# 16lemoing/ccvs

Hardware: AMD Instinct MI355X
Metric: synthesized frames/sec (BAIR 256x256, cond=1, pred=15), whole job (higher is better)
Workload: dtype f32 (convolutions as split-bf16 x3 on bf16 MFMA, fp32 accumulate)

## Files before the change

### ccvs_amd/csrc/gpt.hip

```cpp
#include "common.h"

__global__ __launch_bounds__(256) void gpt_embed_kernel(const int64_t* __restrict__ idx, long idx_sB, const int32_t* __restrict__ pos_off,
                                                        int pos0, const int32_t* __restrict__ pos_dev, int grp_rows, int Tq,
                                                        const float* __restrict__ tok, const float* __restrict__ pos,
                                                        float* __restrict__ x, long total, int C, int vocab) {
    for (long i = (long)blockIdx.x * 256 + threadIdx.x; i < total; i += (long)gridDim.x * 256) {
        const long r = i / C;
        const int c = (int)(i - r * C);
        const long b = r / Tq;
        const int tq = (int)(r - b * Tq);
        long t = idx[b * idx_sB + tq];
        t = t < 0 ? 0 : (t >= vocab ? vocab - 1 : t);
        const long prow = (pos_off ? pos_off[b] : 0) + pos0 + (pos_dev ? pos_dev[grp_rows > 0 ? b / grp_rows : 0] : 0) + tq;
        x[i] = tok[t * C + c] + pos[prow * C + c];
    }
}

extern "C" int ccvs_gpt_embed(const int64_t* idx, int64_t idx_sB, const int32_t* pos_off, int32_t pos0, const int32_t* pos_dev, int32_t Tq,
                              const float* tok_emb, const float* pos_table, float* x, int32_t B, int32_t C, int32_t vocab, void* stream) {
    CCVS_REQUIRE(idx && tok_emb && pos_table && x, "ccvs_gpt_embed: null pointer");
    CCVS_REQUIRE(B > 0 && Tq > 0 && C > 0 && vocab > 0 && (pos0 >= 0 || pos_dev), "ccvs_gpt_embed: empty tensor");
    const long total = (long)B * Tq * C;
    hipLaunchKernelGGL(gpt_embed_kernel, dim3((unsigned)cdiv64(total, 256)), dim3(256), 0, (hipStream_t)stream, idx, (long)idx_sB, pos_off,
                       pos0, pos_dev, 0, Tq, tok_emb, pos_table, x, total, C, vocab);
    CCVS_CHECK_LAUNCH("ccvs_gpt_embed");
    return CCVS_OK;
}

__global__ __launch_bounds__(256) void layernorm_kernel(const float* __restrict__ x, const float* __restrict__ g,
                                                        const float* __restrict__ b, float* __restrict__ y, int rows, int C) {
    const int row = blockIdx.x * 4 + (threadIdx.x >> 6);
    if (row >= rows) return;
    const int lane = threadIdx.x & 63;
    const float* xr = x + (long)row * C;
    float s = 0.f;
    for (int c = lane; c < C; c += 64) s += xr[c];
    const float mean = wave_sum(s) / C;
    float v = 0.f;
    for (int c = lane; c < C; c += 64) { const float d = xr[c] - mean; v += d * d; }
    const float rstd = rsqrtf(wave_sum(v) / C + 1e-5f);
    float* yr = y + (long)row * C;
    for (int c = lane; c < C; c += 64) yr[c] = (xr[c] - mean) * rstd * g[c] + b[c];
}

extern "C" int ccvs_layernorm(const float* x, const float* gamma, const float* beta, float* y, int32_t rows, int32_t C, void* stream) {
    CCVS_REQUIRE(x && gamma && beta && y, "ccvs_layernorm: null pointer");
    CCVS_REQUIRE(rows > 0 && C > 0, "ccvs_layernorm: empty tensor");
    hipLaunchKernelGGL(layernorm_kernel, dim3(cdiv(rows, 4)), dim3(256), 0, (hipStream_t)stream, x, gamma, beta, y, rows, C);
    CCVS_CHECK_LAUNCH("ccvs_layernorm");
    return CCVS_OK;
}

__device__ __forceinline__ float gelu_erf(float v) { return 0.5f * v * (1.f + erff(v * 0.70710678118654752440f)); }

__device__ __forceinline__ void ln_accum(const float4& v, float& sx, float& sxx) {
#pragma clang fp contract(off)
    sx += (v.x + v.y) + (v.z + v.w);
    sxx += (v.x * v.x + v.y * v.y) + (v.z * v.z + v.w * v.w);
}

__device__ __forceinline__ void ln_accum(const f32x4& v, float& sx, float& sxx) {
#pragma clang fp contract(off)
    sx += (v[0] + v[1]) + (v[2] + v[3]);
    sxx += (v[0] * v[0] + v[1] * v[1]) + (v[2] * v[2] + v[3] * v[3]);
}

typedef unsigned int u32x4 __attribute__((ext_vector_type(4)));
template <int AUX = 0>
__device__ __forceinline__ f32x4 buf_load4(__amdgpu_buffer_rsrc_t r, unsigned voff, int soff) {
    const u32x4 v = __builtin_amdgcn_raw_buffer_load_b128(r, voff, soff, AUX);
    return __builtin_bit_cast(f32x4, v);
}

template <bool COH>
__device__ __forceinline__ float ld_act(const float* p) {
    if constexpr (COH) return __hip_atomic_load(p, __ATOMIC_RELAXED, __HIP_MEMORY_SCOPE_AGENT);
    else return *p;
}
template <bool COH>
__device__ __forceinline__ void st_act(float* p, float v) {
    if constexpr (COH) __hip_atomic_store(p, v, __ATOMIC_RELAXED, __HIP_MEMORY_SCOPE_AGENT);
    else *p = v;
}
template <bool OPAQUE>
__device__ __forceinline__ int thread_id() {
    int t = threadIdx.x;
    if constexpr (OPAQUE) asm volatile("" : "+v"(t));
    return t;
}
template <bool COH, typename T>
__device__ __forceinline__ T* gp_(T* p) {
    if constexpr (COH) return (T*)(__attribute__((address_space(1))) T*)p;
    else return p;
}
__device__ __forceinline__ f32x4 ld_act4_sc1(const float* p) {
    const __amdgpu_buffer_rsrc_t r = __builtin_amdgcn_make_buffer_rsrc(const_cast<float*>(p), 0, 16, 0x00020000);
    typedef unsigned int u32x4_ __attribute__((ext_vector_type(4)));
    const u32x4_ v = __builtin_amdgcn_raw_buffer_load_b128(r, 0, 0, 16);
    return __builtin_bit_cast(f32x4, v);
}

struct Gemm16 {
    const float* x; long ldx;
    const float* w; const float* bias; const float* res; float* y; long ldy;
    int M, N, K, epi, ks;
    const float* ln_s; float ln_eps;
    float* kcache; float* vcache; int C, H, D, Tq, Tmax, pos0; const int32_t* pos_dev;
    int seq;
    int grp_rows;
    int kz;
    float* ws_slabs;
    int* ws_count;
};

#define GEMM_U 4
#define GEMM_U_RB 8
#define GEMM_WS_TILES 1024
#define GEMM_KZ_MAX 4
#define GEMM_KZ_MIN_K 2048
#define GEMM_DECODE_MAX_M 256

__device__ __forceinline__ void ln_finish(float a, float b, int K, float eps, float& mean, float& rstd) {
#pragma clang fp contract(off)
    mean = a / K;
    const float var = fmaxf(b / K - mean * mean, 0.f);
    rstd = rsqrtf(var + eps);
}
__device__ __forceinline__ float gemm_epilogue(float v, bool ln, float rstd, float mean, float sn, float bv, int epi, float rv) {
#pragma clang fp contract(off)
    if (ln) v = rstd * (v - mean * sn);
    v += bv;
    if (epi == 1) v = gelu_erf(v);
    if (epi == 2) v += rv;
    return v;
}

#define GEMM_WAVES 4
#define GEMM16_RED_WORDS(NB) (GEMM_WAVES * (NB) * 64 * 4)
#define GEMM16_STAT_WORDS(RB) (GEMM_WAVES * (RB) * 16 * 2)
#define GEMM16_FIN_WORDS(RB) ((RB) * 16 * 2)
template <int RB, int CB, int U, bool COH, typename PT>
__device__ __forceinline__ void gemm16_tile(const float* __restrict__ x_, const float* __restrict__ w_, long ldx_, int K_, int N_, int M_, int ks_,
                                            int kz_, const PT& p, int bx_, int by_, int bz_, float* __restrict__ red, float* __restrict__ stat,
                                            float* __restrict__ fin) {
#define GP(ptr) gp_<COH>(ptr)
    constexpr int NB = RB * CB;
    constexpr int XAUX = COH ? 16 : 0;
    const int tid = thread_id<COH>(), lane = tid & 63, wave = tid >> 6;
    const int li = lane & 15, g = lane >> 4;
    const int m0 = by_ * 16 * RB, ncol0 = bx_ * 16 * CB;
    const int kper = K_ / (ks_ * kz_);
    const int kbase = bz_ * (K_ / kz_);
    const bool active = wave < ks_;
    const unsigned koff = kbase + (active ? wave : 0) * kper + 4 * g;
    unsigned wofs[CB], xofs[RB];
#pragma unroll
    for (int cb = 0; cb < CB; ++cb) {
        const int nrow = min(ncol0 + 16 * cb + li, N_ - 1);
        wofs[cb] = ((unsigned)nrow * (unsigned)K_ + koff) * 4u;
    }
#pragma unroll
    for (int rb = 0; rb < RB; ++rb) {
        const int mrow = min(m0 + 16 * rb + li, M_ - 1);
        xofs[rb] = ((unsigned)mrow * (unsigned)ldx_ + koff) * 4u;
    }
    const __amdgpu_buffer_rsrc_t wr = __builtin_amdgcn_make_buffer_rsrc(const_cast<float*>(w_), 0, N_ * K_ * 4, 0x00020000);
    const __amdgpu_buffer_rsrc_t xr = __builtin_amdgcn_make_buffer_rsrc(const_cast<float*>(x_), 0, (int)(M_ * ldx_ * 4), 0x00020000);
    f32x4 acc[RB][CB];
    float sx[RB], sxx[RB];
#pragma unroll
    for (int rb = 0; rb < RB; ++rb) {
        sx[rb] = 0.f; sxx[rb] = 0.f;
#pragma unroll
        for (int cb = 0; cb < CB; ++cb) acc[rb][cb] = {0.f, 0.f, 0.f, 0.f};
    }
    if (active) {
        int k0 = 0;
        for (; k0 + 16 * U <= kper; k0 += 16 * U) {
            f32x4 wv[CB][U], xv[RB][U];
#pragma unroll
            for (int cb = 0; cb < CB; ++cb)
#pragma unroll
                for (int u = 0; u < U; ++u) wv[cb][u] = buf_load4(wr, wofs[cb], k0 * 4 + 64 * u);
#pragma unroll
            for (int rb = 0; rb < RB; ++rb)
#pragma unroll
                for (int u = 0; u < U; ++u) xv[rb][u] = buf_load4<XAUX>(xr, xofs[rb], k0 * 4 + 64 * u);
            __builtin_amdgcn_sched_barrier(0);
#pragma unroll
            for (int u = 0; u < U; ++u) {
#pragma unroll
                for (int rb = 0; rb < RB; ++rb) {
#pragma unroll
                    for (int cb = 0; cb < CB; ++cb)
#pragma unroll
                        for (int t = 0; t < 4; ++t) acc[rb][cb] = __builtin_amdgcn_mfma_f32_16x16x4f32(xv[rb][u][t], wv[cb][u][t], acc[rb][cb], 0, 0, 0);
                    if (p.ln_s) ln_accum(xv[rb][u], sx[rb], sxx[rb]);
                }
            }
        }
        for (; k0 < kper; k0 += 16) {
            f32x4 w1[CB], x1[RB];
#pragma unroll
            for (int cb = 0; cb < CB; ++cb) w1[cb] = buf_load4(wr, wofs[cb], k0 * 4);
#pragma unroll
            for (int rb = 0; rb < RB; ++rb) x1[rb] = buf_load4<XAUX>(xr, xofs[rb], k0 * 4);
#pragma unroll
            for (int rb = 0; rb < RB; ++rb) {
#pragma unroll
                for (int cb = 0; cb < CB; ++cb)
#pragma unroll
                    for (int t = 0; t < 4; ++t) acc[rb][cb] = __builtin_amdgcn_mfma_f32_16x16x4f32(x1[rb][t], w1[cb][t], acc[rb][cb], 0, 0, 0);
                if (p.ln_s) ln_accum(x1[rb], sx[rb], sxx[rb]);
            }
        }
    }
    if (p.ln_s) {
#pragma unroll
        for (int rb = 0; rb < RB; ++rb) {
            float a = sx[rb], b = sxx[rb];
            a += __shfl_xor(a, 16, 64); a += __shfl_xor(a, 32, 64);
            b += __shfl_xor(b, 16, 64); b += __shfl_xor(b, 32, 64);
            if (g == 0) { stat[((wave * RB + rb) * 16 + li) * 2] = a; stat[((wave * RB + rb) * 16 + li) * 2 + 1] = b; }
        }
    }
#pragma unroll
    for (int rb = 0; rb < RB; ++rb)
#pragma unroll
        for (int cb = 0; cb < CB; ++cb) *reinterpret_cast<f32x4*>(red + ((wave * NB + rb * CB + cb) * 64 + lane) * 4) = acc[rb][cb];
    __syncthreads();
    if (p.ln_s && tid < 16 * RB) {
        const int rb = tid >> 4, r = tid & 15;
        float a = 0.f, b = 0.f;
        for (int w = 0; w < GEMM_WAVES; ++w) { a += stat[((w * RB + rb) * 16 + r) * 2]; b += stat[((w * RB + rb) * 16 + r) * 2 + 1]; }
        float mean, rstd;
        ln_finish(a, b, p.K, p.ln_eps, mean, rstd);
        fin[tid * 2] = mean;
        fin[tid * 2 + 1] = rstd;
    }
    __syncthreads();
#pragma unroll 1
    for (int blk = wave; blk < NB; blk += GEMM_WAVES) {
        const int rb = blk / CB, cb = blk - rb * CB;
        f32x4 a4;
        if constexpr (NB == 1) a4 = acc[0][0];
        else a4 = *reinterpret_cast<const f32x4*>(red + (blk * 64 + lane) * 4);
#pragma unroll
        for (int s = 1; s < GEMM_WAVES; ++s) a4 += *reinterpret_cast<const f32x4*>(red + ((s * NB + blk) * 64 + lane) * 4);
        const int mb0 = m0 + 16 * rb, nb0 = ncol0 + 16 * cb;
        if (mb0 >= p.M || nb0 >= p.N) continue;

        bool finisher = true;
        if (p.kz > 1) {
            const int tile = (mb0 >> 4) * ((p.N + 15) >> 4) + (nb0 >> 4);
            float* slabs = GP(p.ws_slabs) + (long)tile * p.kz * 256;
            float* mine = slabs + (bz_ * 64 + lane) * 4;
#pragma unroll
            for (int c = 0; c < 4; ++c) __hip_atomic_store(mine + c, a4[c], __ATOMIC_RELAXED, __HIP_MEMORY_SCOPE_AGENT);
            asm volatile("s_waitcnt vmcnt(0)" ::: "memory");
            int ticket = 0;
            if (lane == 0) ticket = __hip_atomic_fetch_add(GP(p.ws_count) + tile, 1, __ATOMIC_RELAXED, __HIP_MEMORY_SCOPE_AGENT);
            ticket = __builtin_amdgcn_readfirstlane(ticket);
            finisher = ticket == p.kz - 1;
            if (finisher) {
#pragma unroll
                for (int c = 0; c < 4; ++c) a4[c] = __hip_atomic_load(slabs + lane * 4 + c, __ATOMIC_RELAXED, __HIP_MEMORY_SCOPE_AGENT);
                for (int z = 1; z < p.kz; ++z) {
#pragma unroll
                    for (int c = 0; c < 4; ++c) a4[c] += __hip_atomic_load(slabs + (z * 64 + lane) * 4 + c, __ATOMIC_RELAXED, __HIP_MEMORY_SCOPE_AGENT);
                }
                if (lane == 0) __hip_atomic_store(GP(p.ws_count) + tile, 0, __ATOMIC_RELAXED, __HIP_MEMORY_SCOPE_AGENT);
            }
        }

        const int col = nb0 + li;
        if (finisher && col < p.N) {
            const float bv = p.bias ? GP(p.bias)[col] : 0.f;
            const float sn = p.ln_s ? GP(p.ln_s)[col] : 0.f;
#pragma unroll
            for (int r = 0; r < 4; ++r) {
                const int row = mb0 + 4 * g + r;
                if (row >= p.M) continue;
                const float rv = p.epi == 2 ? ld_act<COH>(GP(p.res) + (long)row * p.ldy + col) : 0.f;
                const float v = gemm_epilogue(a4[r], p.ln_s != nullptr, fin[(rb * 16 + 4 * g + r) * 2 + 1], fin[(rb * 16 + 4 * g + r) * 2], sn, bv, p.epi, rv);
                if (p.kcache && col >= p.C) {
                    const int cc = col - p.C;
                    float* cache = cc >= p.C ? GP(p.vcache) : GP(p.kcache);
                    const int c2 = cc >= p.C ? cc - p.C : cc;
                    const int h = c2 / p.D, d = c2 - h * p.D;
                    const int b = row / p.Tq, t = row - b * p.Tq;
                    const int pos = p.pos0 + (p.pos_dev ? GP(p.pos_dev)[p.grp_rows > 0 ? b / p.grp_rows : 0] : 0);
                    if (pos + t < p.Tmax) st_act<COH>(cache + (((long)b * p.H + h) * p.Tmax + pos + t) * p.D + d, v);
                } else {
                    st_act<COH>(GP(p.y) + (long)row * p.ldy + col, v);
                }
            }
        }
    }
#undef GP
}

template <int RB, int CB, int U>
__global__ __launch_bounds__(64 * GEMM_WAVES) void gemm16_kernel(const float* __restrict__ x_, const float* __restrict__ w_, long ldx_, int K_, int N_,
                                                                int M_, int ks_, int kz_, Gemm16 p) {
    __shared__ __attribute__((aligned(16))) float red[GEMM16_RED_WORDS(RB * CB)];
    __shared__ float stat[GEMM16_STAT_WORDS(RB)];
    __shared__ float fin[GEMM16_FIN_WORDS(RB)];
    gemm16_tile<RB, CB, U, false>(x_, w_, ldx_, K_, N_, M_, ks_, kz_, p, blockIdx.x, blockIdx.y, blockIdx.z, red, stat, fin);
}

template <int RB>
__global__ __launch_bounds__(512) void gemm16_rb_kernel(Gemm16 p) {
    __shared__ __attribute__((aligned(16))) float red[RB * 8 * 64 * 4];
    __shared__ float stat[RB * 8 * 16 * 2];
    __shared__ float fin[RB * 16 * 2];
    const int tid = threadIdx.x, lane = tid & 63, wave = tid >> 6;
    const int li = lane & 15, g = lane >> 4;
    const int m0 = blockIdx.y * 16 * RB, ncol0 = blockIdx.x * 16;
    const int nrow = min(ncol0 + li, p.N - 1);
    const int kper = p.K / p.ks;
    const bool active = wave < p.ks;
    const float* wp = p.w + (long)nrow * p.K + (active ? wave : 0) * kper + 4 * g;
    const float* xp[RB];
#pragma unroll
    for (int rb = 0; rb < RB; ++rb) xp[rb] = p.x + (long)min(m0 + 16 * rb + li, p.M - 1) * p.ldx + (active ? wave : 0) * kper + 4 * g;
    f32x4 acc0[RB], acc1[RB];
    float sx[RB], sxx[RB];
#pragma unroll
    for (int rb = 0; rb < RB; ++rb) { acc0[rb] = {0.f, 0.f, 0.f, 0.f}; acc1[rb] = {0.f, 0.f, 0.f, 0.f}; sx[rb] = 0.f; sxx[rb] = 0.f; }
    if (active) {
        int k0 = 0;
        for (; k0 + 16 * GEMM_U_RB <= kper; k0 += 16 * GEMM_U_RB) {
            float4 wv[GEMM_U_RB];
#pragma unroll
            for (int u = 0; u < GEMM_U_RB; ++u) wv[u] = *reinterpret_cast<const float4*>(wp + k0 + 16 * u);
#pragma unroll
            for (int rb = 0; rb < RB; ++rb) {
                float4 xv[GEMM_U_RB];
#pragma unroll
                for (int u = 0; u < GEMM_U_RB; ++u) xv[u] = *reinterpret_cast<const float4*>(xp[rb] + k0 + 16 * u);
#pragma unroll
                for (int u = 0; u < GEMM_U_RB; ++u) {
                    acc0[rb] = __builtin_amdgcn_mfma_f32_16x16x4f32(xv[u].x, wv[u].x, acc0[rb], 0, 0, 0);
                    acc1[rb] = __builtin_amdgcn_mfma_f32_16x16x4f32(xv[u].y, wv[u].y, acc1[rb], 0, 0, 0);
                    acc0[rb] = __builtin_amdgcn_mfma_f32_16x16x4f32(xv[u].z, wv[u].z, acc0[rb], 0, 0, 0);
                    acc1[rb] = __builtin_amdgcn_mfma_f32_16x16x4f32(xv[u].w, wv[u].w, acc1[rb], 0, 0, 0);
                    if (p.ln_s) ln_accum(xv[u], sx[rb], sxx[rb]);
                }
            }
        }
        for (; k0 < kper; k0 += 16) {
            const float4 w1 = *reinterpret_cast<const float4*>(wp + k0);
#pragma unroll
            for (int rb = 0; rb < RB; ++rb) {
                const float4 x1 = *reinterpret_cast<const float4*>(xp[rb] + k0);
                acc0[rb] = __builtin_amdgcn_mfma_f32_16x16x4f32(x1.x, w1.x, acc0[rb], 0, 0, 0);
                acc1[rb] = __builtin_amdgcn_mfma_f32_16x16x4f32(x1.y, w1.y, acc1[rb], 0, 0, 0);
                acc0[rb] = __builtin_amdgcn_mfma_f32_16x16x4f32(x1.z, w1.z, acc0[rb], 0, 0, 0);
                acc1[rb] = __builtin_amdgcn_mfma_f32_16x16x4f32(x1.w, w1.w, acc1[rb], 0, 0, 0);
                if (p.ln_s) ln_accum(x1, sx[rb], sxx[rb]);
            }
        }
    }
#pragma unroll
    for (int rb = 0; rb < RB; ++rb) {
        const f32x4 acc = acc0[rb] + acc1[rb];
        if (p.ln_s) {
            float a = sx[rb], b = sxx[rb];
            a += __shfl_xor(a, 16, 64); a += __shfl_xor(a, 32, 64);
            b += __shfl_xor(b, 16, 64); b += __shfl_xor(b, 32, 64);
            if (g == 0) { stat[((rb * 8 + wave) * 16 + li) * 2] = a; stat[((rb * 8 + wave) * 16 + li) * 2 + 1] = b; }
        }
        *reinterpret_cast<f32x4*>(red + ((rb * 8 + wave) * 64 + lane) * 4) = acc;
    }
    __syncthreads();
    if (p.ln_s && tid < 16 * RB) {
        const int rb = tid >> 4, r = tid & 15;
        float a = 0.f, b = 0.f;
        for (int w = 0; w < 8; ++w) { a += stat[((rb * 8 + w) * 16 + r) * 2]; b += stat[((rb * 8 + w) * 16 + r) * 2 + 1]; }
        float mean, rstd;
        ln_finish(a, b, p.K, p.ln_eps, mean, rstd);
        fin[tid * 2] = mean;
        fin[tid * 2 + 1] = rstd;
    }
    __syncthreads();
    if (wave >= RB) return;
    const int rb = wave;
    f32x4 acc = *reinterpret_cast<const f32x4*>(red + ((rb * 8) * 64 + lane) * 4);
#pragma unroll
    for (int s2 = 1; s2 < 8; ++s2) acc += *reinterpret_cast<const f32x4*>(red + ((rb * 8 + s2) * 64 + lane) * 4);
    const int col = ncol0 + li;
    if (col >= p.N) return;
    const float bv = p.bias ? p.bias[col] : 0.f;
    const float sn = p.ln_s ? p.ln_s[col] : 0.f;
    int pos0 = p.pos0;
    if (p.kcache && p.pos_dev) pos0 += *p.pos_dev;
#pragma unroll
    for (int r = 0; r < 4; ++r) {
        const int row = m0 + 16 * rb + 4 * g + r;
        if (row >= p.M) continue;
        const float v = gemm_epilogue(acc[r], p.ln_s != nullptr, fin[(rb * 16 + 4 * g + r) * 2 + 1], fin[(rb * 16 + 4 * g + r) * 2], sn, bv, p.epi,
                                      p.epi == 2 ? p.res[(long)row * p.ldy + col] : 0.f);
        if (p.kcache && col >= p.C) {
            const int cc = col - p.C;
            float* cache = cc >= p.C ? p.vcache : p.kcache;
            const int c2 = cc >= p.C ? cc - p.C : cc;
            const int h = c2 / p.D, d = c2 - h * p.D;
            const int b = row / p.Tq, t = row - b * p.Tq;
            if (pos0 + t < p.Tmax) cache[(((long)b * p.H + h) * p.Tmax + pos0 + t) * p.D + d] = v;
        } else {
            p.y[(long)row * p.ldy + col] = v;
        }
    }
}

#define GS_BM 128
#define GS_QS (GS_BM + 1)
typedef __attribute__((address_space(3))) void gs_lds_void;
__global__ __launch_bounds__(256, 4) void gemm_seq_kernel(Gemm16 p, int row_tiles, int col_tiles) {
    __shared__ __attribute__((aligned(16))) f32x4 sm0[2 * 4 * GS_QS];
    __shared__ __attribute__((aligned(16))) f32x4 sm1[2 * 4 * GS_QS];
    __shared__ float fin[GS_BM * 2];
    const int tid = threadIdx.x, lane = tid & 63, wave = tid >> 6;
    int rt, ct;
    {
        const int w = blockIdx.x;
        if (row_tiles % 8 == 0) {
            const int i = w >> 3;
            rt = (w & 7) + 8 * (i / col_tiles);
            ct = i % col_tiles;
        } else {
            rt = w / col_tiles;
            ct = w - rt * col_tiles;
        }
    }
    const int m0 = rt * GS_BM, n0 = ct * GS_BM;
    const __amdgpu_buffer_rsrc_t xr = __builtin_amdgcn_make_buffer_rsrc(const_cast<float*>(p.x), 0, (int)((long)p.M * p.ldx * 4), 0x00020000);
    const __amdgpu_buffer_rsrc_t wrs = __builtin_amdgcn_make_buffer_rsrc(const_cast<float*>(p.w), 0, (int)((long)p.N * p.K * 4), 0x00020000);
    unsigned xoff[2], woff[2];
#pragma unroll
    for (int hf = 0; hf < 2; ++hf) {
        xoff[hf] = (unsigned)((long)min(m0 + 64 * hf + lane, p.M - 1) * p.ldx + 4 * wave) * 4u;
        woff[hf] = (unsigned)((long)min(n0 + 64 * hf + lane, p.N - 1) * p.K + 4 * wave) * 4u;
    }
    const int wr = wave >> 1, wc = wave & 1, l31 = lane & 31, h = lane >> 5;
    f32x16 acc[2][2];
#pragma unroll
    for (int bi = 0; bi < 2; ++bi)
#pragma unroll
        for (int bj = 0; bj < 2; ++bj)
#pragma unroll
            for (int r = 0; r < 16; ++r) acc[bi][bj][r] = 0.f;
    float sx = 0.f, sxx = 0.f;
    const int nst = p.K / 16;
#define GS_DMA(k0, SM)                                                                                             \
    _Pragma("unroll") for (int hf = 0; hf < 2; ++hf) {                                                             \
        __builtin_amdgcn_raw_ptr_buffer_load_lds(xr, (gs_lds_void*)((SM) + wave * GS_QS + 64 * hf), 16, xoff[hf], (k0) * 4, 0, 0);               \
        __builtin_amdgcn_raw_ptr_buffer_load_lds(wrs, (gs_lds_void*)((SM) + 4 * GS_QS + wave * GS_QS + 64 * hf), 16, woff[hf], (k0) * 4, 0, 0);  \
    }
#define GS_STAGE(SM, NEXT_DMA)                                                                                     \
    {                                                                                                              \
        const f32x4* xa = (SM);                                                                                    \
        const f32x4* wb = (SM) + 4 * GS_QS;                                                                        \
        f32x4 a[2][2], b[2][2], t0, t1;                                                                            \
        _Pragma("unroll") for (int s2 = 0; s2 < 2; ++s2) {                                                         \
            const int q = 2 * s2 + h;                                                                              \
            _Pragma("unroll") for (int bi = 0; bi < 2; ++bi) a[s2][bi] = xa[q * GS_QS + 64 * wr + 32 * bi + l31];  \
            _Pragma("unroll") for (int bj = 0; bj < 2; ++bj) b[s2][bj] = wb[q * GS_QS + 64 * wc + 32 * bj + l31];  \
        }                                                                                                          \
        if (p.ln_s) {                                                                                              \
            const int r = tid >> 1, q0 = 2 * (tid & 1);                                                            \
            t0 = xa[q0 * GS_QS + r];                                                                               \
            t1 = xa[(q0 + 1) * GS_QS + r];                                                                         \
        }                                                                                                          \
         \
         \
        NEXT_DMA                                                                                                   \
        _Pragma("unroll") for (int s2 = 0; s2 < 2; ++s2)                                                           \
            _Pragma("unroll") for (int j = 0; j < 4; ++j)                                                          \
                _Pragma("unroll") for (int bi = 0; bi < 2; ++bi)                                                   \
                    _Pragma("unroll") for (int bj = 0; bj < 2; ++bj)                                               \
                        acc[bi][bj] = __builtin_amdgcn_mfma_f32_32x32x2f32(a[s2][bi][j], b[s2][bj][j], acc[bi][bj], 0, 0, 0); \
        if (p.ln_s) {                                                                                              \
            ln_accum(t0, sx, sxx);                                                                                 \
            ln_accum(t1, sx, sxx);                                                                                 \
        }                                                                                                          \
    }
    GS_DMA(0, sm0)
    for (int st = 0; st < nst; st += 2) {
        __syncthreads();
        GS_STAGE(sm0, if (st + 1 < nst) { GS_DMA(16 * (st + 1), sm1) })
        if (st + 1 >= nst) break;
        __syncthreads();
        GS_STAGE(sm1, if (st + 2 < nst) { GS_DMA(16 * (st + 2), sm0) })
    }
#undef GS_DMA
#undef GS_STAGE
    if (p.ln_s) {
        sx += __shfl_xor(sx, 1, 64);
        sxx += __shfl_xor(sxx, 1, 64);
        if (!(tid & 1)) {
            float mean, rstd;
            ln_finish(sx, sxx, p.K, p.ln_eps, mean, rstd);
            fin[(tid >> 1) * 2] = mean;
            fin[(tid >> 1) * 2 + 1] = rstd;
        }
        __syncthreads();
    }
    int pos0 = p.pos0;
    if (p.kcache && p.pos_dev) pos0 += *p.pos_dev;
#pragma unroll
    for (int bj = 0; bj < 2; ++bj) {
        const int col = n0 + 64 * wc + 32 * bj + l31;
        if (col >= p.N) continue;
        const float bv = p.bias ? p.bias[col] : 0.f;
        const float sn = p.ln_s ? p.ln_s[col] : 0.f;
#pragma unroll
        for (int bi = 0; bi < 2; ++bi) {
#pragma unroll
            for (int r = 0; r < 16; ++r) {
                const int lr = 64 * wr + 32 * bi + (r & 3) + 8 * (r >> 2) + 4 * h;
                const int row = m0 + lr;
                if (row >= p.M) continue;
                const float v = gemm_epilogue(acc[bi][bj][r], p.ln_s != nullptr, p.ln_s ? fin[lr * 2 + 1] : 0.f, p.ln_s ? fin[lr * 2] : 0.f, sn, bv,
                                              p.epi, p.epi == 2 ? p.res[(long)row * p.ldy + col] : 0.f);
                if (p.kcache && col >= p.C) {
                    const int cc = col - p.C;
                    float* cache = cc >= p.C ? p.vcache : p.kcache;
                    const int c2 = cc >= p.C ? cc - p.C : cc;
                    const int hh = c2 / p.D, d = c2 - hh * p.D;
                    const int b = row / p.Tq, t = row - b * p.Tq;
                    if (pos0 + t < p.Tmax) cache[(((long)b * p.H + hh) * p.Tmax + pos0 + t) * p.D + d] = v;
                } else {
                    p.y[(long)row * p.ldy + col] = v;
                }
            }
        }
    }
}

static int gemm_kz(const Gemm16& g) {
    const int tiles = cdiv(g.N, 16);
    int kz = 1;
    if (g.ws_slabs && !g.ln_s && tiles * cdiv(GEMM_DECODE_MAX_M, 16) <= GEMM_WS_TILES)
        while (g.K >= GEMM_KZ_MIN_K && kz < GEMM_KZ_MAX && tiles * kz * 2 <= 256 && g.K % (16 * GEMM_WAVES * kz * 2) == 0) kz *= 2;
    return kz;
}

static bool gemm_tile2() {
    static const bool v = getenv_int("CCVS_GEMM_TILE2", 1) != 0;
    return v;
}

enum GemmForm { GEMM_FORM_TILE1, GEMM_FORM_TILE2, GEMM_FORM_RB, GEMM_FORM_SEQ };
static GemmForm gemm16_plan(Gemm16& g) {
    const bool decode_form = !g.seq && g.M <= GEMM_DECODE_MAX_M;
    g.kz = decode_form ? gemm_kz(g) : 1;
    g.ks = decode_form ? GEMM_WAVES : 8;
    while (g.ks > 1 && g.K % (16 * g.ks * g.kz) != 0) g.ks >>= 1;
    if (decode_form) return gemm_tile2() && g.M > 32 && g.N >= 32 ? GEMM_FORM_TILE2 : GEMM_FORM_TILE1;
    static const int seq_dense = getenv_int("CCVS_GEMM_SEQ_DENSE", 1);
    const bool fits = (long)g.M * g.ldx * 4 < (1L << 31) && (long)g.N * g.K * 4 < (1L << 31);
    return g.seq && seq_dense && fits ? GEMM_FORM_SEQ : GEMM_FORM_RB;
}

static bool gemm_ws_holds(const Gemm16& g) { return g.kz == 1 || cdiv(g.N, 16) * cdiv(g.M, 16) <= GEMM_WS_TILES; }

static int launch_gemm16(Gemm16& g, hipStream_t st, const char* name) {
    if (!(g.x && g.w && g.y)) { ccvs_set_error("%s: null pointer", name); return CCVS_ERR_ARG; }
    if (!(g.M > 0 && g.N > 0 && g.K > 0)) { ccvs_set_error("%s: empty tensor", name); return CCVS_ERR_ARG; }
    if (g.K % 16 != 0 || g.ldx % 4 != 0) { ccvs_set_error("%s: K=%d must be a multiple of 16 (ldx %% 4 == 0)", name, g.K); return CCVS_ERR_ARG; }
    if (g.epi < 0 || g.epi > 2 || (g.epi == 2 && !g.res)) { ccvs_set_error("%s: bad epilogue", name); return CCVS_ERR_ARG; }
    const GemmForm form = gemm16_plan(g);
    const bool decode_form = form == GEMM_FORM_TILE1 || form == GEMM_FORM_TILE2;
    if (!gemm_ws_holds(g)) { ccvs_set_error("%s: split-K over %d x %d blocks outgrows the workspace", name, cdiv(g.M, 16), cdiv(g.N, 16)); return CCVS_ERR_ARG; }
    if (decode_form && ((long)g.N * g.K * 4 >= (1L << 31) || (long)g.M * g.ldx * 4 >= (1L << 31))) {
        ccvs_set_error("%s: operand beyond 2^31 bytes (32-bit buffer offsets)", name);
        return CCVS_ERR_ARG;
    }
    if (!decode_form && g.grp_rows > 0) { ccvs_set_error("%s: row groups need M <= %d", name, GEMM_DECODE_MAX_M); return CCVS_ERR_ARG; }
    if (form == GEMM_FORM_SEQ) {
        const int rt = cdiv(g.M, GS_BM), ct = cdiv(g.N, GS_BM);
        hipLaunchKernelGGL(gemm_seq_kernel, dim3(rt * ct), dim3(256), 0, st, g, rt, ct);
    } else if (form == GEMM_FORM_RB)
        hipLaunchKernelGGL((gemm16_rb_kernel<4>), dim3(cdiv(g.N, 16), cdiv(g.M, 64), 1), dim3(512), 0, st, g);
    else {
#define GEMM16_LAUNCH(RBv, CBv, Uv)                                                                                                         \
    hipLaunchKernelGGL((gemm16_kernel<RBv, CBv, Uv>), dim3(cdiv(g.N, 16 * CBv), cdiv(g.M, 16 * RBv), g.kz), dim3(64 * GEMM_WAVES), 0, st, g.x, \
                       g.w, g.ldx, g.K, g.N, g.M, g.ks, g.kz, g)
        if (form == GEMM_FORM_TILE2) GEMM16_LAUNCH(2, 2, 1); else GEMM16_LAUNCH(1, 1, GEMM_U);
#undef GEMM16_LAUNCH
    }
    CCVS_CHECK_LAUNCH(name);
    return CCVS_OK;
}

#define GEMM_WS_SLAB_BYTES ((size_t)GEMM_WS_TILES * GEMM_KZ_MAX * 256 * sizeof(float))
#define GEMM_WS_BAR_OFFSET (GEMM_WS_SLAB_BYTES + (size_t)GEMM_WS_TILES * sizeof(int))
#define GEMM_WS_BAR_BYTES 2048
extern "C" int64_t ccvs_gemm_workspace_bytes(void) { return (int64_t)(GEMM_WS_BAR_OFFSET + GEMM_WS_BAR_BYTES); }

extern "C" int ccvs_gemm_nt(const float* x, int64_t ldx, const float* w, const float* bias, const float* res, float* y, int64_t ldy,
                            int32_t M, int32_t N, int32_t K, int32_t epilogue, void* workspace, void* stream) {
    Gemm16 g = {};
    g.x = x; g.ldx = ldx; g.w = w; g.bias = bias; g.res = res; g.y = y; g.ldy = ldy; g.M = M; g.N = N; g.K = K;
    g.epi = epilogue & 0xff; g.seq = (epilogue & CCVS_GEMM_SEQ) ? 1 : 0;
    if (workspace) {
        g.ws_slabs = (float*)workspace;
        g.ws_count = (int*)((char*)workspace + GEMM_WS_SLAB_BYTES);
    }
    return launch_gemm16(g, (hipStream_t)stream, "ccvs_gemm_nt");
}

extern "C" int ccvs_gemm_ln(const float* x, int64_t ldx, const float* w_gamma, const float* bias_beta, const float* w_rowsum, float eps,
                            float* y, int64_t ldy, int32_t M, int32_t N, int32_t K, int32_t epilogue, void* stream) {
    CCVS_REQUIRE(w_rowsum, "ccvs_gemm_ln: null pointer");
    CCVS_REQUIRE((epilogue & 0xff) == 0 || (epilogue & 0xff) == 1, "ccvs_gemm_ln: bad epilogue");
    Gemm16 g = {};
    g.x = x; g.ldx = ldx; g.w = w_gamma; g.bias = bias_beta; g.y = y; g.ldy = ldy; g.M = M; g.N = N; g.K = K;
    g.epi = epilogue & 0xff; g.seq = (epilogue & CCVS_GEMM_SEQ) ? 1 : 0;
    g.ln_s = w_rowsum; g.ln_eps = eps;
    return launch_gemm16(g, (hipStream_t)stream, "ccvs_gemm_ln");
}

extern "C" int ccvs_gemm_ln_qkv(const float* x, int64_t ldx, const float* w_gamma, const float* bias_beta, const float* w_rowsum, float eps,
                                float* q, float* kcache, float* vcache, int32_t B, int32_t Tq, int32_t C, int32_t H, int32_t pos0,
                                const int32_t* pos_dev, int32_t Tmax, void* stream) {
    CCVS_REQUIRE(w_rowsum && kcache && vcache, "ccvs_gemm_ln_qkv: null pointer");
    CCVS_REQUIRE(B > 0 && Tq > 0 && H > 0 && C % H == 0 && pos0 >= 0 && pos0 + Tq <= Tmax, "ccvs_gemm_ln_qkv: bad shape / positions");
    Gemm16 g = {};
    g.x = x; g.ldx = ldx; g.w = w_gamma; g.bias = bias_beta; g.y = q; g.ldy = C; g.M = B * Tq; g.N = 3 * C; g.K = C; g.epi = 0;
    g.ln_s = w_rowsum; g.ln_eps = eps;
    g.kcache = kcache; g.vcache = vcache; g.C = C; g.H = H; g.D = C / H; g.Tq = Tq; g.Tmax = Tmax; g.pos0 = pos0; g.pos_dev = pos_dev;
    g.seq = Tq > 1 ? 1 : 0;
    return launch_gemm16(g, (hipStream_t)stream, "ccvs_gemm_ln_qkv");
}

__global__ __launch_bounds__(256) void kv_append_kernel(const float* __restrict__ k, const float* __restrict__ v, long sB, long ld,
                                                        float* __restrict__ kc, float* __restrict__ vc, long total, int H, int Tq,
                                                        int pos0, const int32_t* __restrict__ pos_dev, int Tmax, int D) {
    if (pos_dev) pos0 += *pos_dev;
    for (long i = (long)blockIdx.x * 256 + threadIdx.x; i < total; i += (long)gridDim.x * 256) {
        const int d = (int)(i % D);
        long t = i / D;
        const int h = (int)(t % H);
        t /= H;
        const int tq = (int)(t % Tq);
        const long b = t / Tq;
        if (pos0 + tq >= Tmax) continue;
        const long src = b * sB + tq * ld + h * D + d;
        const long dst = ((b * H + h) * Tmax + pos0 + tq) * D + d;
        kc[dst] = k[src];
        vc[dst] = v[src];
    }
}

extern "C" int ccvs_kv_append(const float* k, const float* v, int64_t sB, int64_t ld, float* kcache, float* vcache, int32_t B, int32_t H,
                              int32_t Tq, int32_t pos0, const int32_t* pos_dev, int32_t Tmax, int32_t D, void* stream) {
    CCVS_REQUIRE(k && v && kcache && vcache, "ccvs_kv_append: null pointer");
    CCVS_REQUIRE(B > 0 && H > 0 && Tq > 0 && D > 0 && pos0 >= 0 && pos0 + Tq <= Tmax, "ccvs_kv_append: positions %d..%d exceed cache %d",
                 pos0, pos0 + Tq, Tmax);
    const long total = (long)B * Tq * H * D;
    hipLaunchKernelGGL(kv_append_kernel, dim3((unsigned)cdiv64(total, 256)), dim3(256), 0, (hipStream_t)stream, k, v, (long)sB, (long)ld, kcache,
                       vcache, total, H, Tq, pos0, pos_dev, Tmax, D);
    CCVS_CHECK_LAUNCH("ccvs_kv_append");
    return CCVS_OK;
}

template <int D>
__global__ __launch_bounds__(256) void attention_prefill_kernel(const float* __restrict__ q, long q_sB, long ldq, const float* __restrict__ kc,
                                                                const float* __restrict__ vc, float* __restrict__ out, int H, int Tq, int pos0,
                                                                const int32_t* __restrict__ pos_dev, int Tmax, float scale) {
    constexpr int MT = (D + 31) / 32;
    constexpr int DP = MT * 32;
    constexpr int DK = D / 2;
    constexpr int KS = 33;
    constexpr int F4 = D / 4;
    constexpr int NLD = (32 * F4 + 255) / 256;
    constexpr int TILE_WORDS = D * KS + 32 * DP;
    constexpr int OUT_WORDS = 128 * (D + 1);
    constexpr int SMEM_WORDS = 2 * TILE_WORDS > OUT_WORDS ? 2 * TILE_WORDS : OUT_WORDS;
    __shared__ __attribute__((aligned(16))) float smem[SMEM_WORDS];
    const int tid = threadIdx.x, lane = tid & 63, wave = tid >> 6;
    const int qi = lane & 31, half = lane >> 5;
    const int bh = blockIdx.x, b = bh / H, h = bh - b * H;
    if (pos_dev) pos0 += *pos_dev;
    const int q0 = (gridDim.y - 1 - blockIdx.y) * 128;
    const int qw = q0 + wave * 32;
    const int qidx = qw + qi;
    const int q_last_wg = min(q0 + 127, Tq - 1), q_last_w = min(qw + 31, Tq - 1);
    const int ntiles = (min(pos0 + q_last_wg + 1, Tmax) + 31) >> 5;
    const float* kbase = kc + (long)bh * Tmax * D;
    const float* vbase = vc + (long)bh * Tmax * D;

    float qreg[DK];
    {
        const float* qp = q + (long)b * q_sB + (long)min(qidx, Tq - 1) * ldq + h * D + half;
#pragma unroll
        for (int i = 0; i < DK; ++i) qreg[i] = (qidx < Tq) ? qp[2 * i] * (scale * 1.44269504088896340736f) : 0.f;
    }
    if (MT * 32 > D) {
        for (int e = tid; e < 2 * 32 * (DP - D); e += 256) {
            const int bsel = e / (32 * (DP - D)), r = e - bsel * 32 * (DP - D);
            smem[bsel * TILE_WORDS + D * KS + (r / (DP - D)) * DP + D + r % (DP - D)] = 0.f;
        }
    }

    float4 kreg[NLD], vreg[NLD];
    auto fetch = [&](int kt) {
#pragma unroll
        for (int r = 0; r < NLD; ++r) {
            const int e = min(tid + 256 * r, 32 * F4 - 1);
            const int key = e / F4, d4 = e - key * F4;
            const bool written = kt * 32 + key < pos0 + Tq;
            const long row = min(kt * 32 + key, pos0 + Tq - 1);
            const float4 kv = *reinterpret_cast<const float4*>(kbase + row * D + 4 * d4);
            const float4 vv = *reinterpret_cast<const float4*>(vbase + row * D + 4 * d4);
            kreg[r] = written ? kv : make_float4(0.f, 0.f, 0.f, 0.f);
            vreg[r] = written ? vv : make_float4(0.f, 0.f, 0.f, 0.f);
        }
    };
    auto stash = [&](int buf) {
        float* kt_s = smem + buf * TILE_WORDS;
        float* v_s = kt_s + D * KS;
#pragma unroll
        for (int r = 0; r < NLD; ++r) {
            const int e = tid + 256 * r;
            if (e < 32 * F4) {
                const int key = e / F4, d4 = e - key * F4;
                kt_s[(4 * d4 + 0) * KS + key] = kreg[r].x;
                kt_s[(4 * d4 + 1) * KS + key] = kreg[r].y;
                kt_s[(4 * d4 + 2) * KS + key] = kreg[r].z;
                kt_s[(4 * d4 + 3) * KS + key] = kreg[r].w;
                *reinterpret_cast<float4*>(v_s + key * DP + 4 * d4) = vreg[r];
            }
        }
    };

    f32x16 acc_o[MT];
#pragma unroll
    for (int mt = 0; mt < MT; ++mt)
#pragma unroll
        for (int r = 0; r < 16; ++r) acc_o[mt][r] = 0.f;
    float m_run = -INFINITY, l_run = 0.f;

    fetch(0);
    __syncthreads();
    stash(0);
    __syncthreads();
    for (int kt = 0; kt < ntiles; ++kt) {
        const int buf = kt & 1;
        if (kt + 1 < ntiles) fetch(kt + 1);
        const int key0 = kt * 32;
        if (key0 <= pos0 + q_last_w && qw < Tq) {
            const float* kt_s = smem + buf * TILE_WORDS;
            const float* v_s = kt_s + D * KS;
            f32x16 s;
#pragma unroll
            for (int r = 0; r < 16; ++r) s[r] = 0.f;
#pragma unroll
            for (int i = 0; i < DK; ++i) s = __builtin_amdgcn_mfma_f32_32x32x2f32(kt_s[(2 * i + half) * KS + qi], qreg[i], s, 0, 0, 0);
            const int lim = pos0 + qidx - key0;
            float m_t = -INFINITY;
#pragma unroll
            for (int r = 0; r < 16; ++r) {
                const int kk = 8 * (r >> 2) + 4 * half + (r & 3);
                s[r] = (kk <= lim && qidx < Tq) ? s[r] : -INFINITY;
                m_t = fmaxf(m_t, s[r]);
            }
            m_t = fmaxf(m_t, __shfl_xor(m_t, 32, 64));
            const float m_new = fmaxf(m_run, m_t);
            const float m_use = (m_new == -INFINITY) ? 0.f : m_new;
            const float alpha = __builtin_amdgcn_exp2f(m_run - m_use);
            float l_t = 0.f;
#pragma unroll
            for (int r = 0; r < 16; ++r) {
                s[r] = __builtin_amdgcn_exp2f(s[r] - m_use);
                l_t += s[r];
            }
            l_t += __shfl_xor(l_t, 32, 64);
            l_run = l_run * alpha + l_t;
            m_run = m_new;
            const bool rescale = __any(alpha != 1.f);
#pragma unroll
            for (int mt = 0; mt < MT; ++mt) {
                if (rescale) {
#pragma unroll
                    for (int r = 0; r < 16; ++r) acc_o[mt][r] *= alpha;
                }
#pragma unroll
                for (int j = 0; j < 16; ++j) {
                    const int kk = 8 * (j >> 2) + 4 * half + (j & 3);
                    acc_o[mt] = __builtin_amdgcn_mfma_f32_32x32x2f32(v_s[kk * DP + mt * 32 + qi], s[j], acc_o[mt], 0, 0, 0);
                }
            }
        }
        if (kt + 1 < ntiles) stash(buf ^ 1);
        __syncthreads();
    }
    float* o_s = smem;
    const float inv = l_run > 0.f ? 1.f / l_run : 0.f;
#pragma unroll
    for (int mt = 0; mt < MT; ++mt)
#pragma unroll
        for (int r = 0; r < 16; ++r) {
            const int d = mt * 32 + 8 * (r >> 2) + 4 * half + (r & 3);
            if (d < D) o_s[(wave * 32 + qi) * (D + 1) + d] = acc_o[mt][r] * inv;
        }
    __syncthreads();
    for (int e = tid; e < 128 * D; e += 256) {
        const int ql = e / D, d = e - ql * D;
        if (q0 + ql < Tq) out[((long)b * Tq + q0 + ql) * (H * D) + h * D + d] = o_s[ql * (D + 1) + d];
    }
}

__device__ __forceinline__ f32x4 ld_f4_nt(const float* p) {
    return __builtin_nontemporal_load(reinterpret_cast<const f32x4*>(p));
}

template <int D, bool COH>
__device__ __forceinline__ void attention_decode_item(const float* __restrict__ q, long q_sB, const float* __restrict__ kc,
                                                      const float* __restrict__ vc, float* __restrict__ out, int H, int pos0,
                                                      const int32_t* __restrict__ pos_dev, int grp_rows, int Tmax, float scale, int bh,
                                                      float* smem) {
    constexpr int LPK = D / 4;
    constexpr int KPI = 64 / LPK;
    constexpr int NW = 4;
    constexpr int AU = 4;
    constexpr int BATCH = NW * KPI * AU;
    float* red = smem;
    float* pv = smem + 16;
    float* ps = smem + 16 + NW * 256;
    const int tid = thread_id<COH>(), lane = tid & 63, wave = tid >> 6;
    const int b = bh / H, h = bh - b * H;
    if (pos_dev) {
        if constexpr (COH) pos0 += ((const __attribute__((address_space(4))) int32_t*)pos_dev)[grp_rows > 0 ? b / grp_rows : 0];
        else pos0 += pos_dev[grp_rows > 0 ? b / grp_rows : 0];
    }
    const int L = min(pos0 + 1, Tmax);
    const int kk = lane / LPK, d4 = lane - kk * LPK;
    const float* kbase = kc + (long)bh * Tmax * D + 4 * d4;
    const float* vbase = vc + (long)bh * Tmax * D + 4 * d4;
    const int jw = wave * KPI + kk;
    const int nbatch = (L + BATCH - 1) / BATCH;

    f32x4 k_new = {0.f, 0.f, 0.f, 0.f}, v_new = {0.f, 0.f, 0.f, 0.f};
    if constexpr (COH) {
        k_new = ld_act4_sc1(kbase + (long)(L - 1) * D);
        v_new = ld_act4_sc1(vbase + (long)(L - 1) * D);
    }
#define ATT_LOAD(dst, base, bi, fresh)                                                                                   \
    _Pragma("unroll") for (int u = 0; u < AU; ++u) {                                                                     \
        dst[u] = ld_f4_nt(base + (long)min((bi) * BATCH + jw + u * NW * KPI, L - 1) * D);                                \
        if constexpr (COH) { if ((bi) * BATCH + jw + u * NW * KPI >= L - 1) dst[u] = fresh; }                            \
    }

    float4 qv;
    if constexpr (COH) {
        const f32x4 q4 = ld_act4_sc1(q + (long)b * q_sB + h * D + 4 * d4);
        qv = make_float4(q4[0], q4[1], q4[2], q4[3]);
    } else {
        qv = *reinterpret_cast<const float4*>(q + (long)b * q_sB + h * D + 4 * d4);
    }
    float lmax = -INFINITY;
#pragma unroll 1
    for (int bi = 0; bi < nbatch; ++bi) {
        f32x4 kv[AU];
        ATT_LOAD(kv, kbase, bi, k_new);
#pragma unroll
        for (int u = 0; u < AU; ++u) {
            const int j = bi * BATCH + jw + u * NW * KPI;
            float s = kv[u][0] * qv.x + kv[u][1] * qv.y + kv[u][2] * qv.z + kv[u][3] * qv.w;
#pragma unroll
            for (int o = 1; o < LPK; o <<= 1) s += __shfl_xor(s, o, 64);
            s *= scale;
            if (j < L) {
                if (d4 == 0) ps[j] = s;
                lmax = fmaxf(lmax, s);
            }
        }
    }
    f32x4 vv[AU];
    ATT_LOAD(vv, vbase, 0, v_new);

    lmax = wave_max(lmax);
    if (lane == 0) red[wave] = lmax;
    __syncthreads();
    float gmax = red[0];
#pragma unroll
    for (int w = 1; w < NW; ++w) gmax = fmaxf(gmax, red[w]);
    float lsum = 0.f;
    for (int j = tid; j < L; j += NW * 64) {
        const float e = expf(ps[j] - gmax);
        ps[j] = e;
        lsum += e;
    }
    lsum = wave_sum(lsum);
    __syncthreads();
    if (lane == 0) red[wave] = lsum;
    __syncthreads();
    float tot = red[0];
#pragma unroll
    for (int w = 1; w < NW; ++w) tot += red[w];

    float4 acc = make_float4(0.f, 0.f, 0.f, 0.f);
#pragma unroll 1
    for (int bi = 0; bi < nbatch; ++bi) {
        if (bi > 0) ATT_LOAD(vv, vbase, bi, v_new);
#pragma unroll
        for (int u = 0; u < AU; ++u) {
            const int j = bi * BATCH + jw + u * NW * KPI;
            const float p = (j < L) ? ps[min(j, L - 1)] : 0.f;
            acc.x += p * vv[u][0]; acc.y += p * vv[u][1]; acc.z += p * vv[u][2]; acc.w += p * vv[u][3];
        }
    }
#undef ATT_LOAD
    *reinterpret_cast<float4*>(pv + (wave * 64 + lane) * 4) = acc;
    __syncthreads();
    if (tid < D) {
        const int dd4 = tid >> 2, comp = tid & 3;
        float o = 0.f;
        for (int w = 0; w < NW; ++w)
            for (int s2 = 0; s2 < KPI; ++s2) o += pv[(w * 64 + s2 * LPK + dd4) * 4 + comp];
        st_act<COH>(out + (long)b * (H * D) + h * D + tid, o / tot);
    }
}

template <int D>
__global__ __launch_bounds__(256) void attention_decode_kernel(const float* __restrict__ q, long q_sB, const float* __restrict__ kc,
                                                               const float* __restrict__ vc, float* __restrict__ out, int H, int pos0,
                                                               const int32_t* __restrict__ pos_dev, int grp_rows, int Tmax, float scale) {
    extern __shared__ __attribute__((aligned(16))) float smem[];
    attention_decode_item<D, false>(q, q_sB, kc, vc, out, H, pos0, pos_dev, grp_rows, Tmax, scale, blockIdx.x, smem);
}

static void launch_attention_decode(int D, int n_bh, size_t smem, hipStream_t st, const float* q, long q_sB, const float* kc, const float* vc,
                                    float* out, int H, int pos0, const int32_t* pos_dev, int grp_rows, int Tmax, float scale) {
#define ATT_DECODE_LAUNCH(Dv) \
// ... 65 lines not shown
        __syncthreads();
        for (int j = tid; j < V; j += 256) {
            const unsigned key = fkey(xs[j]);
            if ((key & mask) == prefix) atomicAdd(&hist[(key >> shift) & 255u], 1);
        }
        __syncthreads();
        const int h = hist[tid];
        int s = h;
#pragma unroll
        for (int o = 1; o < 64; o <<= 1) {
            const int t = __shfl_down(s, o, 64);
            if (lane + o < 64) s += t;
        }
        if (lane == 0) wtot[wave] = s;
        __syncthreads();
        for (int w = wave + 1; w < 4; ++w) s += wtot[w];
        if (s >= need && s - h < need) { sel[0] = tid; sel[1] = need - (s - h); }
        __syncthreads();
        prefix |= (unsigned)sel[0] << shift;
        mask |= 255u << shift;
        need = sel[1];
    }
    return prefix;
}

template <bool COH>
__device__ __forceinline__ void sample_topk_row(const float* __restrict__ logits, long ld, const float* __restrict__ noise,
                                                int64_t* __restrict__ out, long out_stride, int V, int top_k, float temperature,
                                                Advance adv, int b, int B_all, float* smem) {
    float* xs = smem;
    float* redf = smem + V;
    int* redj = (int*)(smem + V + 4);
    int* wtot = (int*)(smem + V + 8);
    int* sel = (int*)(smem + V + 12);
    int* hist = (int*)(smem + V + 16);
    const int tid = thread_id<COH>(), lane = tid & 63, wave = tid >> 6;
    const int grp = adv.grp_rows > 0 ? b / adv.grp_rows : 0;
    const int brow = b - grp * (adv.grp_rows > 0 ? adv.grp_rows : 0);
    const int nrows = adv.grp_rows > 0 ? min(adv.grp_rows, B_all - grp * adv.grp_rows) : B_all;
    if (adv.grp_rows > 0) { adv.state += 8 * grp; adv.widx += grp; adv.len += grp; }
    const float* lr = logits + (long)b * ld;
    float lmax = -INFINITY;
    for (int j = tid; j < V; j += 256) {
        const float v = ld_act<COH>(lr + j) / temperature;
        xs[j] = v;
        lmax = fmaxf(lmax, v);
    }
    lmax = wave_max(lmax);
    if (lane == 0) redf[wave] = lmax;
    __syncthreads();
    const float gmax = fmaxf(fmaxf(redf[0], redf[1]), fmaxf(redf[2], redf[3]));

    unsigned thr = 0u;
    if (top_k > 0 && top_k < V) thr = kth_largest_key(xs, V, top_k, hist, wtot, sel, tid);
    float lsum = 0.f;
    for (int j = tid; j < V; j += 256) {
        const float e = (fkey(xs[j]) >= thr) ? expf(xs[j] - gmax) : 0.f;
        xs[j] = e;
        lsum += e;
    }
    lsum = wave_sum(lsum);
    __syncthreads();
    if (lane == 0) redf[wave] = lsum;
    __syncthreads();
    const float tot = ((redf[0] + redf[1]) + redf[2]) + redf[3];
    unsigned k0 = 0u, k1 = 0u, step = 0u, row0 = 0u, call = 0u;
    if (adv.rng == 2) {
        k0 = adv.imm[0]; k1 = adv.imm[1]; row0 = adv.imm[2]; step = adv.imm[3]; call = adv.imm[4];
    } else if (adv.rng) {
        k0 = (unsigned)adv.state[4]; k1 = (unsigned)adv.state[5]; step = (unsigned)adv.state[0];
        call = (unsigned)adv.state[3]; row0 = (unsigned)adv.state[6];
    }
    const float* nrow = noise ? noise + (long)b * V : nullptr;
    if (adv.noise_stream) nrow = adv.noise_stream[grp] + ((long)adv.state[0] * nrows + brow) * V;
    float best = -1.f;
    int bi = 0x7fffffff;
    for (int j = tid; j < V; j += 256) {
        float p = xs[j] / tot;
        if (nrow) p = p / nrow[j];
        else if (adv.rng) {
            const float u = ((float)philox_first((unsigned)j, row0 + (unsigned)brow, step, call, k0, k1) + 0.5f) * 2.3283064365386963e-10f;
            p = p / fmaxf(-logf(u), 1e-30f);
        }
        if (p > best) { best = p; bi = j; }
    }
#pragma unroll
    for (int o = 32; o > 0; o >>= 1) {
        const float ob = __shfl_xor(best, o, 64);
        const int oi = __shfl_xor(bi, o, 64);
        if (ob > best || (ob == best && oi < bi)) { best = ob; bi = oi; }
    }
    __syncthreads();
    if (lane == 0) { redf[wave] = best; redj[wave] = bi; }
    __syncthreads();
    if (tid == 0) {
        for (int w = 1; w < 4; ++w)
            if (redf[w] > best || (redf[w] == best && redj[w] < bi)) { best = redf[w]; bi = redj[w]; }
        out[(long)b * out_stride] = bi;
        if (adv.codes) {
            adv.codes[(long)b * adv.codes_sB + *adv.widx] = bi;
            asm volatile("s_waitcnt vmcnt(0)" ::: "memory");
            __builtin_amdgcn_fence(__ATOMIC_RELEASE, "agent");
            const int ticket = __hip_atomic_fetch_add(adv.state + 2, 1, __ATOMIC_RELAXED, __HIP_MEMORY_SCOPE_AGENT);
            if (ticket == nrows - 1) {
                __builtin_amdgcn_fence(__ATOMIC_ACQUIRE, "agent");
                *adv.widx += 1;
                *adv.len += 1;
                adv.state[0] += 1;
                __hip_atomic_store(adv.state + 2, 0, __ATOMIC_RELAXED, __HIP_MEMORY_SCOPE_AGENT);
            }
        }
    }
}

__global__ __launch_bounds__(256) void sample_topk_kernel(const float* __restrict__ logits, long ld, const float* __restrict__ noise,
                                                          int64_t* __restrict__ out, long out_stride, int V, int top_k, float temperature,
                                                          Advance adv) {
    extern __shared__ __attribute__((aligned(16))) float smem[];
    sample_topk_row<false>(logits, ld, noise, out, out_stride, V, top_k, temperature, adv, blockIdx.x, gridDim.x, smem);
}

#define PICK_SMEM_WORDS(V) ((V) + 16 + 256)
static void pick_allow_big_lds() {
    static bool attr_set = false;
    if (!attr_set) {
        (void)hipFuncSetAttribute((const void*)sample_topk_kernel, hipFuncAttributeMaxDynamicSharedMemorySize, 160 * 1024);
        attr_set = true;
    }
}

extern "C" int ccvs_sample_topk(const float* logits, int64_t ld, const float* noise, int64_t* out, int64_t out_stride, int32_t B, int32_t V,
                                int32_t top_k, float temperature, void* stream) {
    CCVS_REQUIRE(logits && out, "ccvs_sample_topk: null pointer");
    CCVS_REQUIRE(B > 0 && V > 0 && temperature > 0.f, "ccvs_sample_topk: bad arguments");
    const size_t smem = (size_t)PICK_SMEM_WORDS(V) * sizeof(float);
    pick_allow_big_lds();
    CCVS_REQUIRE(smem <= 160 * 1024, "ccvs_sample_topk: vocabulary %d too large", V);
    hipLaunchKernelGGL(sample_topk_kernel, dim3(B), dim3(256), smem, (hipStream_t)stream, logits, (long)ld, noise, out, (long)out_stride, V,
                       top_k, temperature, Advance{});
    CCVS_CHECK_LAUNCH("ccvs_sample_topk");
    return CCVS_OK;
}

extern "C" int ccvs_sample_topk_philox(const float* logits, int64_t ld, int64_t* out, int64_t out_stride, int32_t B, int32_t V, int32_t top_k,
                                       float temperature, uint32_t key0, uint32_t key1, uint32_t row0, uint32_t step, uint32_t call,
                                       void* stream) {
    CCVS_REQUIRE(logits && out, "ccvs_sample_topk_philox: null pointer");
    CCVS_REQUIRE(B > 0 && V > 0 && temperature > 0.f, "ccvs_sample_topk_philox: bad arguments");
    const size_t smem = (size_t)PICK_SMEM_WORDS(V) * sizeof(float);
    pick_allow_big_lds();
    CCVS_REQUIRE(smem <= 160 * 1024, "ccvs_sample_topk_philox: vocabulary %d too large", V);
    Advance adv = {};
    adv.rng = 2;
    adv.imm[0] = key0; adv.imm[1] = key1; adv.imm[2] = row0; adv.imm[3] = step; adv.imm[4] = call;
    hipLaunchKernelGGL(sample_topk_kernel, dim3(B), dim3(256), smem, (hipStream_t)stream, logits, (long)ld, (const float*)nullptr, out,
                       (long)out_stride, V, top_k, temperature, adv);
    CCVS_CHECK_LAUNCH("ccvs_sample_topk_philox");
    return CCVS_OK;
}

__global__ __launch_bounds__(256) void sample_topn_kernel(const float* __restrict__ logits, long ld, const float* __restrict__ noise,
                                                          int64_t* __restrict__ out_idx, float* __restrict__ out_logp, int V, int top_k,
                                                          float temperature, int n) {
    extern __shared__ __attribute__((aligned(16))) float smem[];
    float* xs = smem;
    float* sc = smem + V;
    float* redf = smem + 2 * V;
    int* redj = (int*)(smem + 2 * V + 4);
    int* wtot = (int*)(smem + 2 * V + 8);
    int* sel = (int*)(smem + 2 * V + 12);
    int* hist = (int*)(smem + 2 * V + 16);
    const int tid = threadIdx.x, lane = tid & 63, wave = tid >> 6;
    const int b = blockIdx.x;
    const float* lr = logits + (long)b * ld;
    float lmax = -INFINITY;
    for (int j = tid; j < V; j += 256) {
        const float v = lr[j] / temperature;
        xs[j] = v;
        lmax = fmaxf(lmax, v);
    }
    lmax = wave_max(lmax);
    if (lane == 0) redf[wave] = lmax;
    __syncthreads();
    const float gmax = fmaxf(fmaxf(redf[0], redf[1]), fmaxf(redf[2], redf[3]));
    unsigned thr = 0u;
    if (top_k > 0 && top_k < V) thr = kth_largest_key(xs, V, top_k, hist, wtot, sel, tid);
    float lsum = 0.f;
    for (int j = tid; j < V; j += 256) {
        const float e = (fkey(xs[j]) >= thr) ? expf(xs[j] - gmax) : 0.f;
        xs[j] = e;
        lsum += e;
    }
    lsum = wave_sum(lsum);
    __syncthreads();
    if (lane == 0) redf[wave] = lsum;
    __syncthreads();
    const float tot = ((redf[0] + redf[1]) + redf[2]) + redf[3];
    for (int j = tid; j < V; j += 256) {
        const float p = xs[j] / tot;
        xs[j] = p;
        sc[j] = noise ? p / noise[(long)b * V + j] : p;
    }
    __syncthreads();
    for (int r = 0; r < n; ++r) {
        float best = -1.f;
        int bi = 0x7fffffff;
        for (int j = tid; j < V; j += 256) {
            const float v = sc[j];
            if (v > best) { best = v; bi = j; }
        }
#pragma unroll
        for (int o = 32; o > 0; o >>= 1) {
            const float ob = __shfl_xor(best, o, 64);
            const int oi = __shfl_xor(bi, o, 64);
            if (ob > best || (ob == best && oi < bi)) { best = ob; bi = oi; }
        }
        if (lane == 0) { redf[wave] = best; redj[wave] = bi; }
        __syncthreads();
        if (tid == 0) {
            for (int w = 1; w < 4; ++w)
                if (redf[w] > best || (redf[w] == best && redj[w] < bi)) { best = redf[w]; bi = redj[w]; }
            bi = min(bi, V - 1);
            out_idx[(long)b * n + r] = bi;
            out_logp[(long)b * n + r] = logf(xs[bi]);
            sc[bi] = -2.f;
        }
        __syncthreads();
    }
}

extern "C" int ccvs_sample_topn(const float* logits, int64_t ld, const float* noise, int64_t* out_idx, float* out_logp, int32_t B, int32_t V,
                                int32_t top_k, float temperature, int32_t n, void* stream) {
    CCVS_REQUIRE(logits && out_idx && out_logp, "ccvs_sample_topn: null pointer");
    CCVS_REQUIRE(B > 0 && V > 0 && temperature > 0.f && n >= 1 && n <= V, "ccvs_sample_topn: bad arguments");
    const size_t smem = (size_t)(2 * V + 16 + 256) * sizeof(float);
    CCVS_REQUIRE(smem <= 160 * 1024, "ccvs_sample_topn: vocabulary %d too large", V);
    static bool attr_set = false;
    if (!attr_set) {
        (void)hipFuncSetAttribute((const void*)sample_topn_kernel, hipFuncAttributeMaxDynamicSharedMemorySize, 160 * 1024);
        attr_set = true;
    }
    hipLaunchKernelGGL(sample_topn_kernel, dim3(B), dim3(256), smem, (hipStream_t)stream, logits, (long)ld, noise, out_idx, out_logp, V, top_k,
                       temperature, n);
    CCVS_CHECK_LAUNCH("ccvs_sample_topn");
    return CCVS_OK;
}

#define STEP_SPIN_TICKS 500000000ULL
struct StepBar {
    unsigned shard[8][32];
    unsigned base[32];
    unsigned err[32];
};
static_assert(sizeof(StepBar) <= GEMM_WS_BAR_BYTES, "StepBar outgrew its slot in the workspace");

#define STEP_GEMM 0
#define STEP_ATTENTION 1
struct StepPhase {
    int kind, pad_;
    Gemm16 g;
};

struct StepArgs {
    int B, C, V, vocab, grp_rows, pos_off, n_phases, H;
    const float *tok_emb, *pos_table;
    const int64_t* tok;
    const int32_t* len;
    float *x, *logits;
    StepBar* bar;
    const StepPhase* prog;
    float scale;
    const float* noise;
    int top_k;
    float temperature;
    Advance adv;
};

__device__ __forceinline__ void step_barrier(StepBar* bar, unsigned target, int phase) {
    asm volatile("s_waitcnt vmcnt(0)" ::: "memory");
    __syncthreads();
    if (threadIdx.x < 64) {
        if (threadIdx.x == 0) __hip_atomic_fetch_add(&bar->shard[blockIdx.x & 7][0], 1u, __ATOMIC_RELAXED, __HIP_MEMORY_SCOPE_AGENT);
        const unsigned* sp = &bar->shard[threadIdx.x & 7][0];
        const unsigned long long t0 = __builtin_amdgcn_s_memrealtime();
        for (unsigned spins = 1;; ++spins) {
            unsigned v = __hip_atomic_load(sp, __ATOMIC_RELAXED, __HIP_MEMORY_SCOPE_AGENT);
            v += __shfl_xor(v, 1, 64);
            v += __shfl_xor(v, 2, 64);
            v += __shfl_xor(v, 4, 64);
            if ((int)(v - target) >= 0) break;
            __builtin_amdgcn_s_sleep(2);
            if ((spins & 255u) == 0) {
                const bool late = __builtin_amdgcn_s_memrealtime() - t0 > STEP_SPIN_TICKS;
                if (late || __hip_atomic_load(&bar->err[0], __ATOMIC_RELAXED, __HIP_MEMORY_SCOPE_AGENT) != 0u) {
                    if (late && threadIdx.x == 0) __hip_atomic_store(&bar->err[0], (unsigned)(phase + 1), __ATOMIC_RELAXED, __HIP_MEMORY_SCOPE_AGENT);
                    break;
                }
            }
        }
    }
    __syncthreads();
}

template <int RB, int CB, int U>
__device__ __forceinline__ void step_gemm(const __attribute__((address_space(4))) Gemm16& g, float* smem) {
    float* red = smem;
    float* stat = red + GEMM16_RED_WORDS(RB * CB);
    float* fin = stat + GEMM16_STAT_WORDS(RB);
    const int N = g.N, M = g.M, K = g.K, ks = g.ks, kz = g.kz;
    const long ldx = g.ldx;
    const float* x = gp_<true>(g.x);
    const float* w = gp_<true>(g.w);
    const int gx = (N + 16 * CB - 1) / (16 * CB), gy = (M + 16 * RB - 1) / (16 * RB);
    const int total = gx * gy * kz;
    for (int vb = blockIdx.x; vb < total; vb += gridDim.x) {
        const int bx = vb % gx, r = vb / gx;
        gemm16_tile<RB, CB, U, true>(x, w, ldx, K, N, M, ks, kz, g, bx, r % gy, r / gy, red, stat, fin);
        __syncthreads();
    }
}

#define STEP_GEMM_WORDS(RB, CB) (GEMM16_RED_WORDS((RB) * (CB)) + GEMM16_STAT_WORDS(RB) + GEMM16_FIN_WORDS(RB))

#define STEP_CONST __attribute__((address_space(4)))
#define STEP_GLOBAL __attribute__((address_space(1)))
template <typename T>
__device__ __forceinline__ T* as_global(T* p) {
    return (T*)(STEP_GLOBAL T*)p;
}
template <int D, bool T2>
__global__ __launch_bounds__(256) __attribute__((amdgpu_waves_per_eu(8, 8))) void gpt_step_kernel(const StepArgs* __restrict__ ap_) {
    extern __shared__ __attribute__((aligned(16))) float smem[];
    constexpr int RB = T2 ? 2 : 1, CB = T2 ? 2 : 1, U = T2 ? 1 : GEMM_U;
    const unsigned G = gridDim.x;
    const STEP_CONST StepArgs* ap = (const STEP_CONST StepArgs*)ap_;
    StepBar* bar = as_global(ap->bar);
    const STEP_CONST StepPhase* prog = (const STEP_CONST StepPhase*)ap->prog;
    const int n_phases = ap->n_phases;
    const float att_scale = ap->scale;
    unsigned target = __hip_atomic_load(&bar->base[0], __ATOMIC_RELAXED, __HIP_MEMORY_SCOPE_AGENT);
    {
        const int B = ap->B, C = ap->C, vocab = ap->vocab, grp_rows = ap->grp_rows, pos_off = ap->pos_off;
        const int64_t* tok = as_global(ap->tok);
        const int32_t* len = as_global(ap->len);
        const float* tok_emb = as_global(ap->tok_emb);
        const float* pos_table = as_global(ap->pos_table);
        float* x = as_global(ap->x);
        const long total = (long)B * C;
        for (long i = (long)blockIdx.x * 256 + threadIdx.x; i < total; i += (long)G * 256) {
            const long b = i / C;
            const int c = (int)(i - b * C);
            long t = tok[b];
            t = t < 0 ? 0 : (t >= vocab ? vocab - 1 : t);
            const long prow = pos_off + len[grp_rows > 0 ? b / grp_rows : 0];
            st_act<true>(x + i, tok_emb[t * C + c] + pos_table[prow * C + c]);
        }
    }
    target += G; step_barrier(bar, target, 0);
#pragma unroll 1
    for (int ph = 0; ph < n_phases; ++ph) {
        const STEP_CONST StepPhase* P = prog + ph;
        if (P->kind == STEP_ATTENTION) {
            const STEP_CONST Gemm16& g = P->g;
            const int n_bh = g.M * g.H, H = g.H, Tmax = g.Tmax, grp_rows = g.grp_rows;
            const long q_sB = g.ldx;
            const float* q = as_global(g.x);
            const float* kc = as_global(g.kcache);
            const float* vc = as_global(g.vcache);
            float* att = as_global(g.y);
            const int32_t* len = as_global(g.pos_dev);
            for (int bh = blockIdx.x; bh < n_bh; bh += G) {
                attention_decode_item<D, true>(q, q_sB, kc, vc, att, H, 0, len, grp_rows, Tmax, att_scale, bh, smem);
                __syncthreads();
            }
        } else {
            step_gemm<RB, CB, U>(P->g, smem);
        }
        target += G; step_barrier(bar, target, ph + 1);
    }
    if (blockIdx.x == 0 && threadIdx.x == 0) __hip_atomic_store(&bar->base[0], target, __ATOMIC_RELAXED, __HIP_MEMORY_SCOPE_AGENT);
    {
        const int B = ap->B, V = ap->V;
        Advance adv;
        adv.codes = as_global(ap->adv.codes); adv.codes_sB = ap->adv.codes_sB; adv.widx = as_global(ap->adv.widx); adv.len = as_global(ap->adv.len);
        adv.rng = ap->adv.rng;
#pragma unroll
        for (int i = 0; i < 5; ++i) adv.imm[i] = 0u;
        adv.state = as_global(ap->adv.state); adv.grp_rows = ap->adv.grp_rows; adv.noise_stream = as_global(ap->adv.noise_stream);
        for (int b = blockIdx.x; b < B; b += G) {
            sample_topk_row<true>(as_global(ap->logits), (long)V, as_global(ap->noise), const_cast<int64_t*>(as_global(ap->tok)), 1L, V, ap->top_k,
                                  ap->temperature, adv, b, B, smem);
            __syncthreads();
        }
    }
}

extern "C" int ccvs_gpt_decode_status(const void* workspace, void* stream) {
    CCVS_REQUIRE(workspace, "ccvs_gpt_decode_status: null pointer");
    unsigned err = 0;
    const StepBar* bar = (const StepBar*)((const char*)workspace + GEMM_WS_BAR_OFFSET);
    hipError_t e = hipMemcpyAsync(&err, &bar->err[0], sizeof(err), hipMemcpyDeviceToHost, (hipStream_t)stream);
    if (e == hipSuccess) e = hipStreamSynchronize((hipStream_t)stream);
    if (e != hipSuccess) { ccvs_set_error("ccvs_gpt_decode_status: %s", hipGetErrorString(e)); return CCVS_ERR_LAUNCH; }
    if (err) {
        (void)hipMemsetAsync((void*)bar, 0, sizeof(StepBar), (hipStream_t)stream);
        (void)hipStreamSynchronize((hipStream_t)stream);
        ccvs_set_error("ccvs_gpt_decode_status: a grid barrier of the persistent decode step gave up (phase %u): the tokens of the steps since the last check are invalid", err - 1);
        return CCVS_ERR_LAUNCH;
    }
    return CCVS_OK;
}

#define STEP_HEAD_BYTES 512
static_assert(sizeof(StepArgs) <= STEP_HEAD_BYTES, "StepArgs outgrew the head of the program buffer");
extern "C" int64_t ccvs_gpt_program_bytes(int32_t n_layer) { return (int64_t)STEP_HEAD_BYTES + (int64_t)(5 * (n_layer > 0 ? n_layer : 0) + 1) * sizeof(StepPhase); }

static int step_check(const ccvs_gpt_decode* d, const char* who) {
    if (!(d->workspace && d->program)) { ccvs_set_error("%s: the persistent step needs `workspace` (ccvs_gemm_workspace_bytes, zeroed once) and `program` (ccvs_gpt_program_bytes)", who); return CCVS_ERR_ARG; }
    if (d->B > GEMM_DECODE_MAX_M) { ccvs_set_error("%s: the persistent step takes at most %d rows", who, GEMM_DECODE_MAX_M); return CCVS_ERR_ARG; }
    if (!gemm_tile2()) { ccvs_set_error("%s: the persistent step is built for the default tile (CCVS_GEMM_TILE2=1)", who); return CCVS_ERR_ARG; }
    if (!(d->C >= 32 && d->F >= 32 && d->V >= 32 && d->C % 16 == 0 && d->F % 16 == 0)) { ccvs_set_error("%s: the persistent step needs >= 32 output columns per GEMM and K %% 16 == 0", who); return CCVS_ERR_ARG; }
    if (!((long)d->V * d->C * 4 < (1L << 31) && (long)d->F * d->C * 4 < (1L << 31) && (long)d->B * d->F * 4 < (1L << 31))) { ccvs_set_error("%s: operand beyond 2^31 bytes (32-bit buffer offsets)", who); return CCVS_ERR_ARG; }
    return CCVS_OK;
}

static int step_grp_rows(const ccvs_gpt_decode* d) { return d->groups > 1 ? d->B / d->groups : 0; }

static Advance step_advance(const ccvs_gpt_decode* d, int grp_rows) {
    Advance adv = {};
    adv.codes = d->codes; adv.codes_sB = (long)d->codes_sB; adv.widx = d->widx; adv.len = d->len;
    adv.rng = (d->rng && !d->noise && !d->noise_stream) ? 1 : 0; adv.state = d->state; adv.grp_rows = grp_rows;
    adv.noise_stream = d->noise ? nullptr : d->noise_stream;
    return adv;
}

static Gemm16 step_head_gemm(const ccvs_gpt_decode* d) {
    Gemm16 g = {};
    g.x = d->x; g.ldx = d->C; g.w = d->head_w; g.bias = d->head_b; g.y = d->logits; g.ldy = d->V; g.M = d->B; g.N = d->V; g.K = d->C;
    g.ln_s = d->head_s; g.ln_eps = d->ln_eps;
    return g;
}

static bool step_tile2(const ccvs_gpt_decode* d) {
    Gemm16 g = step_head_gemm(d);
    return gemm16_plan(g) == GEMM_FORM_TILE2;
}

template <typename Visit>
static int step_phases(const ccvs_gpt_decode* d, const char* who, Visit visit) {
    const int D = d->C / d->H, grp_rows = step_grp_rows(d);
    float* ws_slabs = (float*)d->workspace;
    int* ws_count = d->workspace ? (int*)((char*)d->workspace + GEMM_WS_SLAB_BYTES) : nullptr;
    int rc;
    for (int l = 0; l < d->n_layer; ++l) {
        const ccvs_gpt_layer& L = d->layers[l];
        CCVS_REQUIRE(L.qkv_w && L.qkv_b && L.qkv_s && L.proj_w && L.proj_b && L.fc_w && L.fc_b && L.fc_s && L.fc2_w && L.fc2_b && L.kcache && L.vcache,
                     "%s: null pointer in layer %d", who, l);
        Gemm16 g = {};
        g.x = d->x; g.ldx = d->C; g.w = L.qkv_w; g.bias = L.qkv_b; g.y = d->q; g.ldy = d->C; g.M = d->B; g.N = 3 * d->C; g.K = d->C;
        g.ln_s = L.qkv_s; g.ln_eps = d->ln_eps;
        g.kcache = L.kcache; g.vcache = L.vcache; g.C = d->C; g.H = d->H; g.D = D; g.Tq = 1; g.Tmax = d->Tmax; g.pos0 = 0; g.pos_dev = d->len; g.grp_rows = grp_rows;
        if ((rc = visit(STEP_GEMM, g, "ccvs_gpt_decode_step(qkv)")) != CCVS_OK) return rc;
        g = Gemm16{};
        g.x = d->q; g.ldx = d->C; g.y = d->att; g.kcache = L.kcache; g.vcache = L.vcache; g.H = d->H; g.M = d->B; g.Tmax = d->Tmax;
        g.pos_dev = d->len; g.grp_rows = grp_rows;
        if ((rc = visit(STEP_ATTENTION, g, "ccvs_gpt_decode_step(attention)")) != CCVS_OK) return rc;
        g = Gemm16{};
        g.x = d->att; g.ldx = d->C; g.w = L.proj_w; g.bias = L.proj_b; g.res = d->x; g.y = d->x; g.ldy = d->C; g.M = d->B; g.N = d->C; g.K = d->C; g.epi = 2;
        g.ws_slabs = ws_slabs; g.ws_count = ws_count;
        if ((rc = visit(STEP_GEMM, g, "ccvs_gpt_decode_step(proj)")) != CCVS_OK) return rc;
        g = Gemm16{};
        g.x = d->x; g.ldx = d->C; g.w = L.fc_w; g.bias = L.fc_b; g.y = d->h; g.ldy = d->F; g.M = d->B; g.N = d->F; g.K = d->C; g.epi = 1;
        g.ln_s = L.fc_s; g.ln_eps = d->ln_eps;
        if ((rc = visit(STEP_GEMM, g, "ccvs_gpt_decode_step(fc)")) != CCVS_OK) return rc;
        g = Gemm16{};
        g.x = d->h; g.ldx = d->F; g.w = L.fc2_w; g.bias = L.fc2_b; g.res = d->x; g.y = d->x; g.ldy = d->C; g.M = d->B; g.N = d->C; g.K = d->F; g.epi = 2;
        g.ws_slabs = ws_slabs; g.ws_count = ws_count;
        if ((rc = visit(STEP_GEMM, g, "ccvs_gpt_decode_step(fc2)")) != CCVS_OK) return rc;
    }
    Gemm16 g = step_head_gemm(d);
    return visit(STEP_GEMM, g, "ccvs_gpt_decode_step(head)");
}

extern "C" int ccvs_gpt_decode_prepare(const ccvs_gpt_decode* d, void* stream) {
    CCVS_REQUIRE(d && d->layers && d->n_layer > 0 && d->C > 0 && d->H > 0 && d->C % d->H == 0, "ccvs_gpt_decode_prepare: bad descriptor");
    int rc = step_check(d, "ccvs_gpt_decode_prepare");
    if (rc != CCVS_OK) return rc;
    const int grp_rows = step_grp_rows(d), n_ph = 5 * d->n_layer + 1;
    const size_t bytes = (size_t)ccvs_gpt_program_bytes(d->n_layer);
    char* host = (char*)calloc(1, bytes);
    CCVS_REQUIRE(host, "ccvs_gpt_decode_prepare: out of host memory");
    StepPhase* prog = (StepPhase*)(host + STEP_HEAD_BYTES);
    {
        StepArgs& a = *(StepArgs*)host;
        a.B = d->B; a.C = d->C; a.V = d->V; a.vocab = d->vocab; a.grp_rows = grp_rows; a.pos_off = d->pos_off; a.n_phases = n_ph; a.H = d->H;
        a.tok_emb = d->tok_emb; a.pos_table = d->pos_table; a.tok = d->tok; a.len = d->len; a.x = d->x; a.logits = d->logits;
        a.bar = (StepBar*)((char*)d->workspace + GEMM_WS_BAR_OFFSET);
        a.prog = (const StepPhase*)((const char*)d->program + STEP_HEAD_BYTES);
        a.scale = 1.0f / sqrtf((float)(d->C / d->H));
        a.noise = d->noise; a.top_k = d->top_k; a.temperature = d->temperature;
        a.adv = step_advance(d, grp_rows);
    }
    const GemmForm tile = step_tile2(d) ? GEMM_FORM_TILE2 : GEMM_FORM_TILE1;
    int n = 0;
    rc = step_phases(d, "ccvs_gpt_decode_prepare", [&](int kind, Gemm16& g, const char* name) -> int {
        if (n == n_ph || (kind == STEP_GEMM && (gemm16_plan(g) != tile || !gemm_ws_holds(g)))) { ccvs_set_error("ccvs_gpt_decode_prepare: %s does not fit the persistent step's table", name); return CCVS_ERR_ARG; }
        prog[n].kind = kind;
        prog[n++].g = g;
        return CCVS_OK;
    });
    if (rc == CCVS_OK && n != n_ph) { ccvs_set_error("ccvs_gpt_decode_prepare: %d phases, the table holds %d", n, n_ph); rc = CCVS_ERR_ARG; }
    if (rc != CCVS_OK) { free(host); return rc; }
    hipError_t e = hipMemcpyAsync(d->program, host, bytes, hipMemcpyHostToDevice, (hipStream_t)stream);
    if (e == hipSuccess) e = hipStreamSynchronize((hipStream_t)stream);
    free(host);
    if (e != hipSuccess) { ccvs_set_error("ccvs_gpt_decode_prepare: %s", hipGetErrorString(e)); return CCVS_ERR_LAUNCH; }
    return CCVS_OK;
}

static int launch_step_persistent(const ccvs_gpt_decode* d, int D, hipStream_t st) {
    static int n_cu = 0;
    if (!n_cu) {
        int dev = 0;
        hipDeviceProp_t prop;
        if (hipGetDevice(&dev) != hipSuccess || hipGetDeviceProperties(&prop, dev) != hipSuccess) { ccvs_set_error("ccvs_gpt_decode_step: no device properties"); return CCVS_ERR_LAUNCH; }
        n_cu = prop.multiProcessorCount;
    }
    const StepArgs* a = (const StepArgs*)d->program;
    const bool t2 = step_tile2(d);
    size_t words = t2 ? STEP_GEMM_WORDS(2, 2) : STEP_GEMM_WORDS(1, 1);
    const size_t w_att = 16 + 4 * 256 + (size_t)d->Tmax, w_pick = PICK_SMEM_WORDS(d->V);
    if (w_att > words) words = w_att;
    if (w_pick > words) words = w_pick;
    const size_t smem = words * sizeof(float);
#define STEP_LAUNCH(Dv, T2v)                                                                                                          \
    do {                                                                                                                              \
        static bool attr_set = false;                                                                                                 \
        if (!attr_set) {                                                                                                              \
            (void)hipFuncSetAttribute((const void*)gpt_step_kernel<Dv, T2v>, hipFuncAttributeMaxDynamicSharedMemorySize, 160 * 1024); \
            attr_set = true;                                                                                                          \
        }                                                                                                                             \
        hipLaunchKernelGGL((gpt_step_kernel<Dv, T2v>), dim3(n_cu), dim3(256), smem, st, a);                                           \
    } while (0)
    if (D == 64) { if (t2) STEP_LAUNCH(64, true); else STEP_LAUNCH(64, false); }
    else if (D == 32) { if (t2) STEP_LAUNCH(32, true); else STEP_LAUNCH(32, false); }
    else { if (t2) STEP_LAUNCH(16, true); else STEP_LAUNCH(16, false); }
#undef STEP_LAUNCH
    CCVS_CHECK_LAUNCH("ccvs_gpt_decode_step(persistent)");
    return CCVS_OK;
}

extern "C" int ccvs_gpt_decode_step(const ccvs_gpt_decode* d, void* stream) {
    CCVS_REQUIRE(d && d->layers && d->tok_emb && d->pos_table && d->head_w && d->head_b && d->head_s, "ccvs_gpt_decode_step: null pointer");
    CCVS_REQUIRE(d->tok && d->codes && d->widx && d->len && d->x && d->q && d->att && d->h && d->logits && d->state,
                 "ccvs_gpt_decode_step: null state pointer");
    CCVS_REQUIRE(d->B > 0 && d->C > 0 && d->H > 0 && d->C % d->H == 0 && d->F > 0 && d->n_layer > 0 && d->Tmax > 0 && d->vocab > 0 && d->V > 0,
                 "ccvs_gpt_decode_step: bad shape");
    const int D = d->C / d->H;
    CCVS_REQUIRE(D == 64 || D == 32 || D == 16, "ccvs_gpt_decode_step: head dim %d unsupported (16, 32, 64)", D);
    CCVS_REQUIRE(d->temperature > 0.f, "ccvs_gpt_decode_step: bad temperature");
    CCVS_REQUIRE(d->groups >= 0 && (d->groups <= 1 || d->B % d->groups == 0), "ccvs_gpt_decode_step: %d rows do not split into %d groups", d->B, d->groups);
    CCVS_REQUIRE(d->groups <= 1 || d->B <= GEMM_DECODE_MAX_M, "ccvs_gpt_decode_step: at most %d rows per grouped step", GEMM_DECODE_MAX_M);
    const int grp_rows = step_grp_rows(d);
    const size_t smem_att = (size_t)(16 + 4 * 256 + d->Tmax) * sizeof(float);
    const size_t smem_pick = (size_t)PICK_SMEM_WORDS(d->V) * sizeof(float);
    CCVS_REQUIRE(smem_att <= 64 * 1024, "ccvs_gpt_decode_step: sequence too long for the LDS score buffer");
    CCVS_REQUIRE(smem_pick <= 160 * 1024, "ccvs_gpt_decode_step: vocabulary %d too large", d->V);
    hipStream_t st = (hipStream_t)stream;
    if (d->persistent) {
        int rc_ = step_check(d, "ccvs_gpt_decode_step");
        if (rc_ != CCVS_OK) return rc_;
        return launch_step_persistent(d, D, st);
    }
    pick_allow_big_lds();

    {
        const long total = (long)d->B * d->C;
        hipLaunchKernelGGL(gpt_embed_kernel, dim3((unsigned)cdiv64(total, 256)), dim3(256), 0, st, d->tok, 1L, (const int32_t*)nullptr, d->pos_off,
                           (const int32_t*)d->len, grp_rows, 1, d->tok_emb, d->pos_table, d->x, total, d->C, d->vocab);
        CCVS_CHECK_LAUNCH("ccvs_gpt_decode_step(embed)");
    }
    const float scale = 1.0f / sqrtf((float)D);
    const int rc = step_phases(d, "ccvs_gpt_decode_step", [&](int kind, Gemm16& g, const char* name) -> int {
        if (kind == STEP_GEMM) return launch_gemm16(g, st, name);
        launch_attention_decode(D, g.M * g.H, smem_att, st, g.x, g.ldx, g.kcache, g.vcache, g.y, g.H, 0, g.pos_dev, g.grp_rows, g.Tmax, scale);
        CCVS_CHECK_LAUNCH(name);
        return CCVS_OK;
    });
    if (rc != CCVS_OK) return rc;
    hipLaunchKernelGGL(sample_topk_kernel, dim3(d->B), dim3(256), smem_pick, st, d->logits, (long)d->V, d->noise, d->tok, 1L, d->V,
                       d->top_k, d->temperature, step_advance(d, grp_rows));
    CCVS_CHECK_LAUNCH("ccvs_gpt_decode_step(pick)");
    return CCVS_OK;
}
```

### ccvs_amd/lib.py

```python
import ctypes as C
import os

_HERE = os.path.dirname(os.path.abspath(__file__))
LIB_PATH = os.environ.get("CCVS_LIB") or os.path.join(_HERE, "csrc", "libccvs_hip.so")

EXPORTS = [
    "ccvs_last_error", "ccvs_abi_version", "ccvs_conv2d", "ccvs_conv2d_bf16x3", "ccvs_conv_fetch_bytes_per_lane", "ccvs_conv_persistent_tiles", "ccvs_upfirdn2d", "ccvs_dwconvT4x4s2",
    "ccvs_correlation7x7", "ccvs_backwarp", "ccvs_backwarp_ctx", "ccvs_backwarp_p8_ctx", "ccvs_backwarp_proj_ctx", "ccvs_warp_fuse_blend", "ccvs_warp_fuse_blend_ctx", "ccvs_tap_shift_add", "ccvs_vq_argmin", "ccvs_embed_gather", "ccvs_l2_normalize_channels",
    "ccvs_gpt_embed", "ccvs_layernorm", "ccvs_gemm_workspace_bytes", "ccvs_gemm_nt", "ccvs_gemm_ln", "ccvs_gemm_ln_qkv", "ccvs_attention", "ccvs_kv_append", "ccvs_sample_topk", "ccvs_sample_topk_philox", "ccvs_sample_topn",
    "ccvs_gpt_decode_step", "ccvs_gpt_decode_status", "ccvs_gpt_program_bytes", "ccvs_gpt_decode_prepare", "ccvs_pack_u8", "ccvs_pack_u8_norm", "ccvs_stream_cu_limit", "ccvs_psnr", "ccvs_ssim_workspace_bytes", "ccvs_ssim", "ccvs_resize_bilinear",
    "ccvs_deform_conv3x3_ctx", "ccvs_gconvT4x4s2", "ccvs_flow_mask_toff", "ccvs_gaussian_blur", "ccvs_to_rgb", "ccvs_channel_head", "ccvs_mse",
    "ccvs_token_nll", "ccvs_mean_f32", "ccvs_conv_last_launch",
]
EVAL_EXPORTS = ["ccvs_l1_workspace_bytes", "ccvs_l1_mean", "ccvs_vq_stats_workspace_bytes", "ccvs_vq_stats", "ccvs_code_perplexity"]
INPUT_EXPORTS = ["ccvs_ingest_u8"]


class ConvDesc(C.Structure):
    _fields_ = [
        ("N", C.c_int32), ("Cin", C.c_int32), ("Hin", C.c_int32), ("Win", C.c_int32),
        ("in_sN", C.c_int64), ("in_sC", C.c_int64),
        ("Cout", C.c_int32), ("CoutPad", C.c_int32), ("Hout", C.c_int32), ("Wout", C.c_int32),
        ("out_sN", C.c_int64), ("out_sC", C.c_int64), ("res_sN", C.c_int64), ("res_sC", C.c_int64),
        ("kh", C.c_int32), ("kw", C.c_int32), ("stride", C.c_int32), ("pad", C.c_int32), ("transposed", C.c_int32),
        ("act", C.c_int32), ("accumulate", C.c_int32), ("out_scale", C.c_float),
        ("pre", C.c_void_p), ("pre_sN", C.c_int64), ("pre_sC", C.c_int64), ("pre_div", C.c_int32),
        ("in_p8", C.c_int32), ("out_p8", C.c_int32), ("cu_limit", C.c_int32),
        ("w_ktail", C.c_void_p),
    ]


MAX_CTX = 16


class CtxList(C.Structure):
    _fields_ = [("k", C.c_int32), ("p", C.c_void_p * MAX_CTX), ("sN", C.c_int64 * MAX_CTX)]


class GptLayer(C.Structure):
    _fields_ = [(n, C.c_void_p) for n in ("qkv_w", "qkv_b", "qkv_s", "proj_w", "proj_b", "fc_w", "fc_b", "fc_s", "fc2_w", "fc2_b",
                                          "kcache", "vcache")]


class GptDecode(C.Structure):
    _fields_ = [
        ("B", C.c_int32), ("C", C.c_int32), ("H", C.c_int32), ("F", C.c_int32), ("n_layer", C.c_int32), ("Tmax", C.c_int32),
        ("vocab", C.c_int32), ("V", C.c_int32), ("ln_eps", C.c_float),
        ("layers", C.POINTER(GptLayer)),
        ("tok_emb", C.c_void_p), ("pos_table", C.c_void_p), ("pos_off", C.c_int32),
        ("head_w", C.c_void_p), ("head_b", C.c_void_p), ("head_s", C.c_void_p),
        ("tok", C.c_void_p), ("codes", C.c_void_p), ("codes_sB", C.c_int64),
        ("widx", C.c_void_p), ("len", C.c_void_p),
        ("x", C.c_void_p), ("q", C.c_void_p), ("att", C.c_void_p), ("h", C.c_void_p), ("logits", C.c_void_p),
        ("noise", C.c_void_p), ("rng", C.c_int32), ("top_k", C.c_int32), ("temperature", C.c_float),
        ("workspace", C.c_void_p), ("state", C.c_void_p), ("groups", C.c_int32),
        ("noise_stream", C.c_void_p),
        ("persistent", C.c_int32), ("program", C.c_void_p),
    ]


class CcvsError(RuntimeError):
    pass


_lib = None


def load():
    global _lib
    if _lib is not None:
        return _lib
    if not os.path.exists(LIB_PATH):
        raise CcvsError(f"{LIB_PATH} not found: the HIP kernel library is not built "
                        f"(run `make -C {os.path.dirname(LIB_PATH)}`); there is no CPU fallback")
    lib = C.CDLL(LIB_PATH)
    vp, i32, i64, f32 = C.c_void_p, C.c_int32, C.c_int64, C.c_float
    lib.ccvs_last_error.restype = C.c_char_p
    lib.ccvs_last_error.argtypes = []
    lib.ccvs_abi_version.restype = C.c_int
    lib.ccvs_gemm_workspace_bytes.restype = C.c_int64
    lib.ccvs_gemm_workspace_bytes.argtypes = []
    lib.ccvs_ssim_workspace_bytes.restype = C.c_int64
    lib.ccvs_ssim_workspace_bytes.argtypes = [C.c_int64, C.c_int32, C.c_int32]
    lib.ccvs_l1_workspace_bytes.restype = C.c_int64
    lib.ccvs_l1_workspace_bytes.argtypes = [C.c_int64]
    lib.ccvs_vq_stats_workspace_bytes.restype = C.c_int64
    lib.ccvs_vq_stats_workspace_bytes.argtypes = [C.c_int64, C.c_int32, C.c_int32]
    lib.ccvs_gpt_program_bytes.restype = C.c_int64
    lib.ccvs_gpt_program_bytes.argtypes = [C.c_int32]
    lib.ccvs_conv_fetch_bytes_per_lane.restype = C.c_int
    lib.ccvs_conv_fetch_bytes_per_lane.argtypes = [C.c_char_p]
    lib.ccvs_conv_persistent_tiles.restype = C.c_int
    lib.ccvs_conv_persistent_tiles.argtypes = [C.c_int32]
    lib.ccvs_conv_last_launch.restype = C.c_char_p
    lib.ccvs_conv_last_launch.argtypes = []
    sigs = {
        "ccvs_conv2d": [vp, vp, vp, vp, vp, C.POINTER(ConvDesc), vp],
        "ccvs_conv2d_bf16x3": [vp, vp, vp, vp, vp, C.POINTER(ConvDesc), vp],
        "ccvs_upfirdn2d": [vp, vp, vp, i64, i32, i32, i32, i32, i32, i32, f32, i32, f32, vp],
        "ccvs_dwconvT4x4s2": [vp, i64, vp, vp, i64, i32, i32, i32, i32, vp],
        "ccvs_correlation7x7": [vp, vp, vp, i32, i32, i32, i32, i32, i32, i32, vp],
        "ccvs_backwarp": [vp, i64, i64, vp, i64, f32, vp, i64, i64, i32, i32, i32, i32, vp],
        "ccvs_warp_fuse_blend": [vp, i64, i64, vp, vp, i64, vp, i64, f32, i32, i32, i32, i32, i32, vp],
        "ccvs_backwarp_ctx": [C.POINTER(CtxList), i64, vp, i64, f32, vp, i64, i64, i32, i32, i32, i32, vp],
        "ccvs_backwarp_p8_ctx": [C.POINTER(CtxList), i64, vp, i64, f32, vp, i32, i32, i32, i32, vp],
        "ccvs_backwarp_proj_ctx": [C.POINTER(CtxList), i64, vp, i64, f32, vp, vp, vp, i32, i32, i32, i32, i32, i32, i32, vp],
        "ccvs_warp_fuse_blend_ctx": [vp, i64, i64, C.POINTER(CtxList), vp, i64, vp, i64, f32, i32, i32, i32, i32, vp],
        "ccvs_tap_shift_add": [vp, vp, vp, i64, i32, i32, i32, i32, i32, i32, vp],
        "ccvs_vq_argmin": [vp, vp, vp, vp, i32, i32, i32, i32, vp],
        "ccvs_embed_gather": [vp, vp, vp, i32, i32, i32, i32, vp],
        "ccvs_l2_normalize_channels": [vp, i32, i32, i64, vp],
        "ccvs_gpt_embed": [vp, i64, vp, i32, vp, i32, vp, vp, vp, i32, i32, i32, vp],
        "ccvs_layernorm": [vp, vp, vp, vp, i32, i32, vp],
        "ccvs_gemm_nt": [vp, i64, vp, vp, vp, vp, i64, i32, i32, i32, i32, vp, vp],
        "ccvs_gemm_ln": [vp, i64, vp, vp, vp, f32, vp, i64, i32, i32, i32, i32, vp],
        "ccvs_gemm_ln_qkv": [vp, i64, vp, vp, vp, f32, vp, vp, vp, i32, i32, i32, i32, i32, vp, i32, vp],
        "ccvs_attention": [vp, i64, i64, vp, vp, vp, i32, i32, i32, i32, vp, i32, i32, vp],
        "ccvs_kv_append": [vp, vp, i64, i64, vp, vp, i32, i32, i32, i32, vp, i32, i32, vp],
        "ccvs_sample_topk": [vp, i64, vp, vp, i64, i32, i32, i32, f32, vp],
        "ccvs_sample_topk_philox": [vp, i64, vp, i64, i32, i32, i32, f32, C.c_uint32, C.c_uint32, C.c_uint32, C.c_uint32, C.c_uint32, vp],
        "ccvs_sample_topn": [vp, i64, vp, vp, vp, i32, i32, i32, f32, i32, vp],
        "ccvs_gpt_decode_step": [C.POINTER(GptDecode), vp],
        "ccvs_gpt_decode_status": [vp, vp],
        "ccvs_gpt_decode_prepare": [C.POINTER(GptDecode), vp],
        "ccvs_pack_u8": [vp, vp, i64, i32, i32, f32, f32, vp],
        "ccvs_pack_u8_norm": [vp, vp, i64, i32, i32, C.POINTER(C.c_float), C.POINTER(C.c_float), vp],
        "ccvs_stream_cu_limit": [vp, i32],
        "ccvs_psnr": [vp, vp, vp, i64, i64, f32, vp],
        "ccvs_ssim": [vp, vp, vp, vp, i64, i32, i32, C.c_double, vp],
        "ccvs_resize_bilinear": [vp, vp, i64, i32, i32, i32, i32, vp],
        "ccvs_deform_conv3x3_ctx": [C.POINTER(CtxList), i64, vp, i64, f32, vp, i32, i32, vp, vp, i64, vp, i64, i64, vp, i64, i64, i32, i32,
                                    i32, i32, i32, vp],
        "ccvs_gconvT4x4s2": [vp, i64, vp, vp, i64, i64, i32, i32, i32, i32, i32, vp],
        "ccvs_flow_mask_toff": [vp, i64, i64, vp, i64, vp, i64, i64, i32, i32, i32, i32, i32, vp],
        "ccvs_gaussian_blur": [vp, i64, i64, vp, i32, i32, i32, i32, i32, C.POINTER(C.c_float), vp],
        "ccvs_to_rgb": [vp, i64, vp, vp, vp, vp, vp, i32, i32, i32, i32, vp],
        "ccvs_channel_head": [vp, i64, vp, f32, vp, vp, i32, i32, i32, i32, i32, i32, vp],
        "ccvs_mse": [vp, vp, vp, i64, vp],
        "ccvs_token_nll": [vp, i64, vp, vp, i64, i32, vp, vp],
        "ccvs_mean_f32": [vp, i64, vp, vp],
        "ccvs_l1_mean": [vp, vp, vp, vp, i64, vp],
        "ccvs_vq_stats": [vp, vp, vp, vp, vp, vp, vp, i64, i32, i32, i32, vp],
        "ccvs_code_perplexity": [vp, i32, i64, vp, vp],
        "ccvs_ingest_u8": [vp, i64, i32, i32, i32, i32, i32, i32, i32, vp, vp, i32, vp, vp, i32, i32, i32, vp, vp, i64, i64, vp, vp],
    }
    for name, argtypes in sigs.items():
        fn = getattr(lib, name)
        fn.restype = C.c_int
        fn.argtypes = argtypes
    _lib = lib
    return lib


def check(rc, name):
    if rc != 0:
        raise CcvsError(f"{name} failed ({rc}): {load().ccvs_last_error().decode()}")
```

### ccvs_amd/models/skip_vid_generator/models/mingpt.py

```python
import torch
import torch.nn as nn

from ccvs_amd import ops


class GPTConfig:
    embd_pdrop = 0.1
    resid_pdrop = 0.1
    attn_pdrop = 0.1

    def __init__(self, block_size, **kwargs):
        self.block_size = block_size
        for k, v in kwargs.items():
            setattr(self, k, v)


class CausalSelfAttention(nn.Module):

    def __init__(self, config):
        super().__init__()
        assert config.n_embd % config.n_head == 0
        self.key = nn.Linear(config.n_embd, config.n_embd)
        self.query = nn.Linear(config.n_embd, config.n_embd)
        self.value = nn.Linear(config.n_embd, config.n_embd)
        self.attn_drop = nn.Dropout(config.attn_pdrop)
        self.resid_drop = nn.Dropout(config.resid_pdrop)
        self.proj = nn.Linear(config.n_embd, config.n_embd)
        self.n_head = config.n_head
        self._qkv = None

    def qkv_packed(self):
        ws = (self.query.weight, self.key.weight, self.value.weight)
        key = tuple((w.data_ptr(), w._version) for w in ws) + (ws[0].device,)
        if self._qkv is None or self._qkv[0] != key:
            w = torch.cat([w.detach() for w in ws], dim=0).contiguous()
            b = torch.cat([self.query.bias.detach(), self.key.bias.detach(), self.value.bias.detach()]).contiguous()
            self._qkv = (key, w, b)
        return self._qkv[1], self._qkv[2]


class NoiseInjection(nn.Module):

    def __init__(self, use_noise):
        super().__init__()
        if use_noise:
            raise NotImplementedError("resid_noise is a training-time option")

    def forward(self, x):
        return x


class Block(nn.Module):

    def __init__(self, config):
        super().__init__()
        self.ln1 = nn.LayerNorm(config.n_embd)
        self.ln2 = nn.LayerNorm(config.n_embd)
        self.attn = CausalSelfAttention(config)
        self.mlp = nn.Sequential(
            nn.Linear(config.n_embd, 4 * config.n_embd),
            NoiseInjection(config.resid_noise),
            nn.GELU(),
            nn.Linear(4 * config.n_embd, config.n_embd),
            nn.Dropout(config.resid_pdrop),
        )
        self._folded = None

    def folded(self):
        src = (self.ln1.weight, self.ln1.bias, self.attn.query.weight, self.attn.key.weight, self.attn.value.weight,
               self.attn.query.bias, self.attn.key.bias, self.attn.value.bias, self.ln2.weight, self.ln2.bias,
               self.mlp[0].weight, self.mlp[0].bias)
        key = tuple((t.data_ptr(), t._version) for t in src) + (src[0].device,)
        if self._folded is None or self._folded[0] != key:
            wqkv, bqkv = self.attn.qkv_packed()
            qkv = ops.pack_ln_linear(wqkv, bqkv, self.ln1.weight, self.ln1.bias)
            fc = ops.pack_ln_linear(self.mlp[0].weight, self.mlp[0].bias, self.ln2.weight, self.ln2.bias)
            self._folded = (key, qkv, fc)
        return self._folded[1], self._folded[2]


class GPT(nn.Module):

    def __init__(self, vocab_size, block_size, num_blocks, n_layer=12, n_head=8, n_embd=256, embd_pdrop=0., resid_pdrop=0.,
                 attn_pdrop=0., n_unmasked=0, resid_noise=False, emb_mode=None, shape=None, state_vocab_size=0, state_size=0,
                 use_start_token=False, num_lbl=0, use_lbl=False, state_front=False):
        super().__init__()
        if n_unmasked:
            raise NotImplementedError("unmasked prefixes are not on the MI355X path (SURVEY 8f)")
        config = GPTConfig(block_size=block_size, vocab_size=vocab_size, embd_pdrop=embd_pdrop, resid_pdrop=resid_pdrop,
                           attn_pdrop=attn_pdrop, n_layer=n_layer, n_head=n_head, n_embd=n_embd, n_unmasked=n_unmasked,
                           resid_noise=resid_noise, shape=shape, emb_mode=emb_mode, state_vocab_size=state_vocab_size,
                           state_size=state_size, use_start_token=use_start_token, num_blocks=num_blocks, num_lbl=num_lbl,
                           use_lbl=use_lbl, state_front=state_front)
        self.tok_emb = nn.Embedding(config.vocab_size, config.n_embd)
        if config.state_vocab_size > 0:
            self.state_tok_emb = nn.Embedding(config.state_vocab_size, config.n_embd)
        if config.use_start_token:
            self.start_tok_emb = nn.Parameter(torch.randn(1, config.n_embd))
        if config.use_lbl:
            self.lbl_emb = nn.Embedding(config.num_lbl, config.n_embd)
        height, width = config.shape
        if config.emb_mode is not None:
            if config.emb_mode == "spatio-temporal":
                self.h_emb = nn.Parameter(torch.zeros(1, height, config.n_embd))
                self.w_emb = nn.Parameter(torch.zeros(1, width, config.n_embd))
                self.t_emb = nn.Parameter(torch.zeros(1, config.num_blocks, config.n_embd))
            elif config.emb_mode == "temporal":
                self.s_emb = nn.Parameter(torch.zeros(1, height * width, config.n_embd))
                self.t_emb = nn.Parameter(torch.zeros(1, config.num_blocks, config.n_embd))
            else:
                raise ValueError
        else:
            self.pos_emb = nn.Parameter(torch.zeros(1, config.num_blocks * height * width, config.n_embd))
        if config.state_size > 0:
            if config.emb_mode is not None:
                self.state_s_emb = nn.Parameter(torch.zeros(1, config.state_size, config.n_embd))
            else:
                self.state_pos_emb = nn.Parameter(torch.zeros(1, config.num_blocks * config.state_size, config.n_embd))
        self.drop = nn.Dropout(config.embd_pdrop)
        self.blocks = nn.Sequential(*[Block(config) for _ in range(config.n_layer)])
        self.ln_f = nn.LayerNorm(config.n_embd)
        self.head = nn.Linear(config.n_embd, max(config.vocab_size, config.state_vocab_size), bias=False)
        self.block_size = config.block_size + (1 if config.use_start_token else 0) + (1 if config.use_lbl else 0)
        self.apply(self._init_weights)
        self.config = config
        self._cache = None
        self._caches = {}
        self.noise_key = None
        self.row_offset = 0
        self.noise_call = 0
        self.warm_only = False
        self.progress = None
        self.noise_streams = None
        import os
        self.persistent_step = os.environ.get("CCVS_DECODE_PERSISTENT", "0") == "1"

    @property
    def _graphs(self):
        return self._cache["graphs"]

    def n_groups(self):
        return len(self.noise_key) if isinstance(self.noise_key, list) else 1

    def drop_engine_state(self):
        self._cache, self._caches = None, {}

    def _philox_words(self):
        if self.noise_key is None:
            k = torch.randint(0, 2**32, (2,), dtype=torch.int64).tolist()
            return [(int(k[0]), int(k[1]), int(self.row_offset), 0)]
        call = self.noise_call
        self.noise_call += 1
        if isinstance(self.noise_key, list):
            assert isinstance(self.row_offset, list) and len(self.row_offset) == len(self.noise_key)
            return [(int(k[0]) & 0xffffffff, int(k[1]) & 0xffffffff, int(r), call) for k, r in zip(self.noise_key, self.row_offset)]
        return [(int(self.noise_key[0]) & 0xffffffff, int(self.noise_key[1]) & 0xffffffff, int(self.row_offset), call)]

    def _set_decode_state(self, words):
        c = self._cache
        st = torch.zeros(c["G"], 8, dtype=torch.int64)
        if words is not None:
            assert len(words) == c["G"], (len(words), c["G"])
            for g, (k0, k1, row0, call) in enumerate(words):
                st[g, 3], st[g, 4], st[g, 5], st[g, 6] = call, k0, k1, row0
        st = torch.where(st >= 2**31, st - 2**32, st).to(torch.int32)
        c["state"].copy_(st, non_blocking=True)

    def _pick(self, logits, sampler, noise, out, words, step):
        if words is None:
            return ops.sample_topk(logits, sampler["top_k"], sampler["temperature"], noise=noise, out=out)
        b = logits.shape[0]
        n = len(words)
        assert b % n == 0
        per = b // n
        if out is None:
            out = torch.empty(b, dtype=torch.int64, device=logits.device)
        for g, (k0, k1, row0, call) in enumerate(words):
            ops.sample_topk(logits[g * per:(g + 1) * per], sampler["top_k"], sampler["temperature"], out=out[g * per:(g + 1) * per],
                            philox=(k0, k1, row0, step[0], call | step[1]))
        return out

    def get_block_size(self):
        return self.block_size

    def _init_weights(self, module):
        if isinstance(module, (nn.Linear, nn.Embedding)):
            module.weight.data.normal_(mean=0.0, std=0.02)
            if isinstance(module, nn.Linear) and module.bias is not None:
                module.bias.data.zero_()
        elif isinstance(module, nn.LayerNorm):
            module.bias.data.zero_()
            module.weight.data.fill_(1.0)

    @torch.no_grad()
    def get_pos_emb(self, t, delta_length=None):
        if t == 0:
            return 0
        cfg = self.config
        height, width = cfg.shape
        size = height * width
        dev = self.tok_emb.weight.device
        if delta_length is None or 0 in delta_length.size():
            delta_length = torch.zeros(1, dtype=torch.long)
        deltas = [int(d) for d in delta_length.view(-1).tolist()]
        n = len(deltas)
        if cfg.emb_mode is None:
            return torch.stack([self.pos_emb[0, d * size: d * size + t] for d in deltas]).to(dev)
        length = t // size + (1 if t % size != 0 else 0)
        t_emb = torch.stack([self.t_emb[0, d: d + length] for d in deltas])
        if cfg.emb_mode == "temporal":
            pos = self.s_emb.view(1, 1, size, -1) + t_emb.view(n, length, 1, -1)
        else:
            pos = self.h_emb.view(1, 1, height, 1, -1) + self.w_emb.view(1, 1, 1, width, -1)
            pos = pos + t_emb.view(n, length, 1, 1, -1)
        return pos.reshape(n, length * size, -1)[:, :t]

    @torch.no_grad()
    def get_state_pos_emb(self, t):
        cfg = self.config
        size = cfg.state_size
        if cfg.emb_mode is not None:
            length = t // size + (1 if t % size != 0 else 0)
            pos = self.state_s_emb.view(1, 1, size, -1) + self.t_emb[:, :length].view(1, length, 1, -1)
            return pos.reshape(1, length * size, -1)[:, :t]
        return self.state_pos_emb[:, :t]

    def stream_kinds(self, n_code, n_state):
        cfg = self.config
        size, ss = cfg.shape[0] * cfg.shape[1], cfg.state_size
        n_state = min(n_state, cfg.num_blocks * ss)
        if n_state == 0:
            return [(0, i) for i in range(n_code)]
        if cfg.state_front:
            return [(1, i) for i in range(n_state)] + [(0, i) for i in range(n_code)]
        length = n_code // size
        if length == 0:
            return [(1, i) for i in range(min(ss, n_state))]
        assert n_state >= length * ss, "ancillary stream shorter than the frames it annotates (the reference's view() fails too)"
        seq = []
        for f in range(length):
            seq += [(1, f * ss + i) for i in range(ss)] + [(0, f * size + i) for i in range(size)]
        seq += [(1, i) for i in range(length * ss, min((length + 1) * ss, n_state))]
        seq += [(0, i) for i in range(length * size, n_code)]
        return seq

    def _token_table(self):
        if self.config.state_vocab_size <= 0:
            return self.tok_emb.weight
        src = (self.tok_emb.weight, self.state_tok_emb.weight)
        key = tuple((t.data_ptr(), t._version) for t in src) + (src[0].device,)
        tt = getattr(self, "_tok_table", None)
        if tt is None or tt[0] != key:
            tt = self._tok_table = (key, torch.cat([t.detach() for t in src], dim=0).contiguous())
        return tt[1]

    def _stream_rows(self, code, state_code):
        kinds = self.stream_kinds(code.shape[1], 0 if state_code is None else state_code.shape[1])
        dev = code.device
        kind = torch.tensor([k for k, _ in kinds], dtype=torch.bool, device=dev)
        idx = torch.tensor([i for _, i in kinds], dtype=torch.long, device=dev)
        frame_rows = code[:, idx.clamp(max=max(code.shape[1] - 1, 0))] if code.shape[1] else torch.zeros(code.shape[0], len(kinds), dtype=torch.long, device=dev)
        if state_code is None or state_code.shape[1] == 0:
            return frame_rows.contiguous()
        state_rows = state_code[:, idx.clamp(max=state_code.shape[1] - 1)] + self.config.vocab_size
        return torch.where(kind.view(1, -1), state_rows, frame_rows).contiguous()

    def _stream_pos_table(self, n_rows, n_state_front=0):
        cfg = self.config
        size, ss = cfg.shape[0] * cfg.shape[1], cfg.state_size
        if cfg.state_front:
            parts = [self.get_state_pos_emb(n_state_front)[0]] if n_state_front else []
            if n_rows - n_state_front > 0:
                parts.append(self.get_pos_emb(n_rows - n_state_front)[0])
            return torch.cat(parts, dim=0)
        tot = size + ss
        nf = (n_rows + tot - 1) // tot
        assert nf <= cfg.num_blocks, "Cannot forward, model block size is exhausted."
        fp = self.get_pos_emb(nf * size)[0].view(nf, size, -1)
        sp = self.get_state_pos_emb(nf * ss)[0].view(nf, ss, -1)
        return torch.cat([sp, fp], dim=1).reshape(nf * tot, -1)[:n_rows]

    @torch.no_grad()
    def begin(self, batch, max_len, stream=False, n_state_front=0):
        cfg = self.config
        if not stream:
            assert max_len <= self.block_size, "Cannot forward, model block size is exhausted."
        dev = self.tok_emb.weight.device
        d = cfg.n_embd // cfg.n_head
        groups = self.n_groups()
        assert batch % groups == 0, f"{batch} rows do not split into {groups} row groups"
        c = self._caches.get(batch)
        if c is None or c["T"] < max_len or c["dev"] != dev or c["G"] != groups:
            if c is None and len(self._caches) >= 8:
                self._caches.pop(next(iter(self._caches)))
            C, V = cfg.n_embd, self.head.weight.shape[0]
            f32 = dict(dtype=torch.float32, device=dev)
            kc = [torch.empty(batch, cfg.n_head, max_len, d, **f32) for _ in range(cfg.n_layer)]
            vc = [torch.empty(batch, cfg.n_head, max_len, d, **f32) for _ in range(cfg.n_layer)]
            c = self._caches[batch] = {
                "B": batch, "G": groups, "T": max_len, "dev": dev, "k": kc, "v": vc,
                "len_dev": torch.zeros(groups, dtype=torch.int32, device=dev),
                "widx": torch.zeros(groups, dtype=torch.int32, device=dev),
                "tok": torch.zeros(batch, 1, dtype=torch.int64, device=dev),
                "codes": torch.zeros(batch, max_len, dtype=torch.int64, device=dev),
                "x": torch.empty(batch, C, **f32), "q": torch.empty(batch, C, **f32), "att": torch.empty(batch, C, **f32),
                "h": torch.empty(batch, 4 * C, **f32), "logits": torch.empty(batch, V, **f32), "noise": torch.empty(batch, V, **f32),
                "state": torch.zeros(groups, 8, dtype=torch.int32, device=dev),
                "noise_ptrs": torch.zeros(groups, dtype=torch.int64, device=dev),
                "noise_keep": None,
                "desc": None, "graphs": {},
            }
        self._cache = c
        c["len"] = 0
        c["stream"] = bool(stream)
        if stream:
            tot = cfg.shape[0] * cfg.shape[1] + cfg.state_size
            table = self._stream_pos_table(c["T"] if cfg.state_front else min(c["T"], cfg.num_blocks * tot), n_state_front)
        else:
            table = self.get_pos_emb(min(c["T"], cfg.block_size))[0]
        if "pos_table" in c and c["pos_table"].shape == table.shape:
            c["pos_table"].copy_(table)
        else:
            c["pos_table"] = table.contiguous().clone()
            c["desc"], c["graphs"] = None, {}
        c["frame_pos0"] = 0
        return c

    def _layers(self, x, b, tq, pos_dev=None):
        c = self._cache
        pos0 = 0 if pos_dev is not None else c["len"]
        C = self.config.n_embd
        seq = ops.GEMM_SEQ if tq > 1 else 0
        for i, blk in enumerate(self.blocks):
            qkv_w, fc_w = blk.folded()
            q = ops.gemm_ln_qkv(x, *qkv_w, c["k"][i], c["v"][i], b, tq, pos0, pos_dev, eps=blk.ln1.eps).view(b, tq, C)
            att = ops.attention(q, c["k"][i], c["v"][i], pos0, pos_dev)
            ops.gemm_nt(att.view(b * tq, C), blk.attn.proj.weight, blk.attn.proj.bias, ops.EPI_RESIDUAL | seq, residual=x, out=x)
            h = ops.gemm_ln(x, *fc_w, eps=blk.ln2.eps, epilogue=ops.EPI_GELU | seq)
            ops.gemm_nt(h, blk.mlp[3].weight, blk.mlp[3].bias, ops.EPI_RESIDUAL | seq, residual=x, out=x)
        if pos_dev is None:
            c["len"] = pos0 + tq
        return x

    def _head_packed(self):
        src = (self.ln_f.weight, self.ln_f.bias, self.head.weight)
        key = tuple((t.data_ptr(), t._version) for t in src) + (src[0].device,)
        hf = getattr(self, "_head_folded", None)
        if hf is None or hf[0] != key:
            hf = self._head_folded = (key, ops.pack_ln_linear(self.head.weight, None, self.ln_f.weight, self.ln_f.bias))
        return hf

    def _head(self, x):
        return ops.gemm_ln(x, *self._head_packed()[1], eps=self.ln_f.eps)

    def n_prefix(self):
        return (1 if self.config.use_lbl else 0) + (1 if self.config.use_start_token else 0)

    def _prefix_emb(self, b, lbl_idx):
        rows = []
        if self.config.use_lbl:
            assert lbl_idx is not None and 0 not in lbl_idx.size(), "label tokens (--x_cat) need data['vid_lbl']"
            rows.append(self.lbl_emb.weight.detach()[lbl_idx.to(self.lbl_emb.weight.device).view(-1)].view(b, 1, -1))
        if self.config.use_start_token:
            rows.append(self.start_tok_emb.detach().view(1, 1, -1).expand(b, 1, -1))
        return torch.cat(rows, dim=1) if rows else None

    @torch.no_grad()
    def prefill(self, idx, cond_idx=None, delta_length_cond=None, all_logits=False, lbl_idx=None):
        c = self._cache
        b, t = idx.shape
        C = self.config.n_embd
        use_cond = cond_idx is not None and 0 not in cond_idx.size()
        parts = []
        prefix = self._prefix_emb(b, lbl_idx)
        n_pre = 0 if prefix is None else prefix.shape[1]
        if prefix is not None:
            parts.append(prefix.float())
        if use_cond:
            t_cond = cond_idx.shape[1]
            cond_tab = self.get_pos_emb(t_cond, delta_length_cond)
            if cond_tab.shape[0] == 1 and b > 1:
                cond_tab = cond_tab.expand(b, -1, -1)
            table = torch.cat([c["pos_table"], cond_tab.reshape(-1, C)], dim=0).contiguous()
            off = (c["pos_table"].shape[0] + torch.arange(b, dtype=torch.int32) * t_cond).to(idx.device)
            parts.append(ops.gpt_embed(cond_idx.contiguous(), self._token_table(), table, 0, off).view(b, t_cond, C))
        else:
            t_cond = 0
        if t > 0:
            parts.append(ops.gpt_embed(idx.contiguous(), self._token_table(), c["pos_table"], 0).view(b, t, C))
        assert parts, "nothing to run: no frame token, no conditioning prefix, no start / label token"
        x = parts[0] if len(parts) == 1 else torch.cat(parts, dim=1)
        tq = n_pre + t_cond + t
        assert c["len"] == 0 and tq <= c["T"], "Cannot forward, model block size is exhausted."
        x = self._layers(x.reshape(b * tq, C).contiguous(), b, tq)
        c["frame_pos0"] = n_pre + t_cond
        if all_logits:
            xs = x.view(b, tq, C)[:, t_cond:].reshape(b * (tq - t_cond), C)
            return self._head(xs).view(b, tq - t_cond, -1)
        return self._head(x.view(b, tq, C)[:, -1].contiguous())

    @torch.no_grad()
    def step(self, tok):
        c = self._cache
        b = tok.shape[0]
        frame_pos = c["len"] - c["frame_pos0"]
        assert c["len"] < c["T"], "Cannot forward, model block size is exhausted."
        x = ops.gpt_embed(tok, self._token_table(), c["pos_table"], frame_pos)
        x = self._layers(x, b, 1)
        return self._head(x)

    @torch.no_grad()
    def reorder_cache(self, rows):
        c = self._cache
        n = c["len"]
        for cache in c["k"] + c["v"]:
            cache[:, :, :n] = cache[rows, :, :n]

    @torch.no_grad()
    def extend(self, rows):
        c = self._cache
        b, tq = rows.shape
        C = self.config.n_embd
        assert c["len"] + tq <= c["T"], "Cannot forward, model block size is exhausted."
        x = ops.gpt_embed(rows.contiguous(), self._token_table(), c["pos_table"], c["len"] - c["frame_pos0"])
        x = self._layers(x.view(b * tq, C), b, tq)
        return self._head(x.view(b, tq, C)[:, -1].contiguous())

    def _decode_desc(self, sampler):
        c = self._cache
        cfg = self.config
        folded = [blk.folded() for blk in self.blocks]
        head_key, (hw, hb, hs) = self._head_packed()
        device_rng = sampler["sample"] and sampler["noise"] == "device"
        host_stream = bool(sampler["sample"] and not device_rng and sampler.get("stream"))
        key = (tuple(blk._folded[0] for blk in self.blocks), head_key, sampler["sample"], sampler["top_k"],
               sampler["temperature"], device_rng, host_stream, c["frame_pos0"], bool(self.persistent_step))
        if c["desc"] is None or c["desc"][0] != key:
            layers = []
            for i, blk in enumerate(self.blocks):
                (qw, qb, qs), (fw, fb, fs) = folded[i]
                layers.append(dict(qkv_w=qw, qkv_b=qb, qkv_s=qs, proj_w=blk.attn.proj.weight, proj_b=blk.attn.proj.bias,
                                   fc_w=fw, fc_b=fb, fc_s=fs, fc2_w=blk.mlp[3].weight, fc2_b=blk.mlp[3].bias,
                                   kcache=c["k"][i], vcache=c["v"][i]))
            desc = ops.GptDecodeStep(
                layers, B=c["B"], groups=c["G"], C=cfg.n_embd, H=cfg.n_head, Tmax=c["T"], ln_eps=self.ln_f.eps,
                tok_emb=self._token_table(), pos_table=c["pos_table"], pos_off=-c["frame_pos0"], head=(hw, hb, hs),
                tok=c["tok"], codes=c["codes"], widx=c["widx"], length=c["len_dev"],
                x=c["x"], q=c["q"], att=c["att"], h=c["h"], logits=c["logits"],
                noise=c["noise"] if (sampler["sample"] and not device_rng and not host_stream) else None, rng=device_rng,
                noise_stream=c["noise_ptrs"] if host_stream else None,
                top_k=sampler["top_k"], temperature=sampler["temperature"], state=c["state"], persistent=self.persistent_step)
            c["desc"] = (key, desc)
            c["graphs"] = {}
        return c["desc"][1]

    def check_steps(self):
        for c in self._caches.values():
            if c.get("desc") is not None and c["desc"][1].persistent:
                c["desc"][1].status()
                return

    def _emit(self, logits, sampler, noise, col, words=None, step=None):
        c = self._cache
        self._pick(logits, sampler, noise, c["tok"].view(-1), words, step)
        c["codes"][:, col] = c["tok"][:, 0]
        c["widx"].fill_(col + 1)

    def _decode_body(self, sampler, noise=None, trace=None):
        c = self._cache
        desc = self._decode_desc(sampler)
        if sampler["sample"] and sampler["noise"] != "device" and not sampler.get("stream"):
            c["noise"].copy_(noise, non_blocking=True)
        desc.launch()
        if trace is not None:
            trace.append(c["logits"].clone())

    GRAPH_STEPS = 8

    def _replay_steps(self, sampler, key, n, known=None):
        k = self.GRAPH_STEPS
        if self.warm_only:
            self._decode_graph(sampler, key + (k,), steps=k)
            self._decode_graph(sampler, key)
            return
        report = self.progress if known is not None else None
        codes = self._cache["codes"]
        if n >= 2 * k:
            long_graph = self._decode_graph(sampler, key + (k,), steps=k)
            for _ in range(n // k):
                long_graph.replay()
                if report is not None:
                    known += k
                    report(known, codes)
            n -= (n // k) * k
        if n:
            graph = self._decode_graph(sampler, key)
            for _ in range(n):
                graph.replay()
                if report is not None:
                    known += 1
                    report(known, codes)

    def _decode_graph(self, sampler, key, steps=1):
        c = self._cache
        self._decode_desc(sampler)
        graph = self._graphs.get(key)
        if graph is None:
            state = {k: c[k].clone() for k in ("len_dev", "widx", "tok", "codes", "state")}
            warm = torch.cuda.Stream()
            warm.wait_stream(torch.cuda.current_stream())
            with torch.cuda.stream(warm):
                self._decode_body(sampler)
            torch.cuda.current_stream().wait_stream(warm)
            for k, v in state.items():
                c[k].copy_(v)
            graph = torch.cuda.CUDAGraph()
            with torch.cuda.graph(graph, capture_error_mode="thread_local"):
                for _ in range(steps):
                    self._decode_body(sampler)
            for k, v in state.items():
                c[k].copy_(v)
            self._graphs[key] = graph
        return graph

    @torch.no_grad()
    def _generate_stream(self, code, state_code, add_len, cond_idx, delta_length_cond, sampler, state_sampler, host_noise, trace,
                         use_graph):
        cfg = self.config
        if cfg.state_front:
            return self._generate_state_front(code, state_code, add_len, cond_idx, delta_length_cond, sampler, state_sampler, host_noise, trace)
        size, ss = cfg.shape[0] * cfg.shape[1], cfg.state_size
        tot = size + ss
        b, t0 = code.shape
        ns0 = state_code.shape[1]
        cap = cfg.num_blocks * ss
        if t0 < size:
            raise NotImplementedError("less than one whole frame of tokens with an ancillary stream (the reference drops them)")
        n_cond = cond_idx.shape[1] if cond_idx is not None else 0
        slen = lambda nc, nst: len(self.stream_kinds(nc, nst))
        plan, single = [], []
        nc, nst = t0, ns0
        for i in range(add_len):
            fed = slen(nc, nst)
            is_state = fed % tot < ss
            plan.append(1 if is_state else 0)
            single.append(i > 0 and plan[i - 1] == 0 and not is_state and fed - prev_fed == 1)
            prev_fed = fed
            if is_state:
                nst += 1
            else:
                nc += 1
        assert n_cond + nc <= self.block_size, "Cannot forward, model block size is exhausted."
        max_len = n_cond + slen(nc, nst)
        c = self.begin(b, max_len, stream=True)
        dev = code.device
        frame_codes = c["codes"]
        frame_codes[:, :t0] = code
        state_buf = torch.zeros(b, max(nst, ns0), dtype=torch.int64, device=dev)
        state_buf[:, :ns0] = state_code
        n_code, n_state = t0, ns0
        device_noise = sampler["sample"] and sampler["noise"] == "device"
        eager = trace is not None or (sampler["sample"] and not device_noise) or not use_graph
        if self.warm_only and eager:
            out = torch.zeros(b, nc, dtype=torch.int64, device=dev)
            out[:, :t0] = code
            return out, state_buf[:, :nst].clone()
        words = self._philox_words() if device_noise else None
        self._set_decode_state(words)

        def rows_of(lo, hi):
            kinds = self.stream_kinds(n_code, n_state)[lo:hi]
            cols = [frame_codes[:, i:i + 1] if k == 0 else state_buf[:, i:i + 1] + cfg.vocab_size for k, i in kinds]
            return torch.cat(cols, dim=1)

        def draw(kind, width, pick):
            smp = state_sampler if kind else sampler
            if not smp["sample"]:
                return None, None, None
            if device_noise:
                return None, words, (pick, 0x80000000)
            return host_noise(b, width).to(dev, non_blocking=True), None, None

        logits = self.prefill(self._stream_rows(code, state_code), cond_idx, delta_length_cond)
        fed = slen(n_code, n_state)
        i = 0
        while i < add_len:
            if single[i] and not eager:
                run = 1
                while i + run < add_len and single[i + run]:
                    run += 1
                c["len_dev"].fill_(c["len"])
                c["widx"].fill_(n_code)
                self._replay_steps(sampler, (sampler["sample"], sampler["top_k"], sampler["temperature"], n_cond, b, "stream"), run)
                c["len"] += run
                n_code += run
                fed += run
                i += run
                logits = None
                continue
            if logits is None:
                new_fed = slen(n_code, n_state)
                logits = self.extend(rows_of(fed, new_fed))
                fed = new_fed
            if plan[i]:
                lg = logits[:, :state_sampler["vocab"]].contiguous()
                if trace is not None:
                    trace.append(lg.clone())
                nz, wd, stp = draw(1, lg.shape[1], i)
                tok = self._pick(lg, state_sampler, nz, None, wd, stp)
                state_buf[:, n_state] = tok
                n_state += 1
            else:
                if trace is not None:
                    trace.append(logits.clone())
                nz, wd, stp = draw(0, logits.shape[1], i)
                self._pick(logits, sampler, nz, c["tok"].view(-1), wd, stp)
                frame_codes[:, n_code] = c["tok"][:, 0]
                n_code += 1
            i += 1
            logits = None
            if i < add_len and not (single[i] and not eager):
                new_fed = slen(n_code, n_state)
                logits = self.extend(rows_of(fed, new_fed))
                fed = new_fed
        return frame_codes[:, :n_code].clone(), state_buf[:, :n_state].clone()

    @torch.no_grad()
    def _generate_state_front(self, code, state_code, add_len, cond_idx, delta_length_cond, sampler, state_sampler, host_noise, trace):
        cfg = self.config
        size, ss = cfg.shape[0] * cfg.shape[1], cfg.state_size
        tot, cap = size + ss, cfg.num_blocks * ss
        b = code.shape[0]
        dev = code.device
        n_cond = cond_idx.shape[1] if cond_idx is not None else 0
        device_noise = sampler["noise"] == "device"
        words = self._philox_words() if device_noise and (sampler["sample"] or state_sampler["sample"]) else None
        state_code = state_code.to(dev)
        for i in range(add_len):
            st = state_code[:, :cap]
            assert n_cond + code.shape[1] <= self.block_size, "Cannot forward, model block size is exhausted."
            rows = self._stream_rows(code, st)
            self.begin(b, n_cond + rows.shape[1], stream=True, n_state_front=st.shape[1])
            logits = self.prefill(rows, cond_idx, delta_length_cond)
            is_state = rows.shape[1] % tot < ss
            smp = state_sampler if is_state else sampler
            lg = logits[:, :state_sampler["vocab"]].contiguous() if is_state else logits
            if trace is not None:
                trace.append(lg.clone())
            nz, wd, stp = None, None, None
            if smp["sample"]:
                if device_noise:
                    wd, stp = words, (i, 0x80000000)
                else:
                    nz = host_noise(b, lg.shape[1]).to(dev, non_blocking=True)
            tok = self._pick(lg, smp, nz, None, wd, stp).view(b, 1).to(torch.int64)
            if is_state:
                state_code = torch.cat((state_code, tok), dim=1)
            else:
                code = torch.cat((code, tok), dim=1)
        return code, state_code

    @torch.no_grad()
    def generate(self, code, add_len, cond_idx=None, delta_length_cond=None, sample=False, top_k=None, temperature=1.0,
                 noise="device", host_noise=None, trace=None, use_graph=True, state_code=None, state_sampler=None, lbl_idx=None):
        b, t0 = code.shape
        use_cond = cond_idx is not None and 0 not in cond_idx.size()
        n_cond = cond_idx.shape[1] if use_cond else 0
        sampler = {"sample": bool(sample), "top_k": top_k, "temperature": float(temperature), "noise": noise}
        n_pre = self.n_prefix()
        if state_code is not None and 0 not in state_code.size():
            if n_pre:
                raise NotImplementedError("label / start tokens together with an ancillary token stream")
            return self._generate_stream(code, state_code, add_len, cond_idx if use_cond else None,
                                         delta_length_cond if use_cond else None, sampler, state_sampler, host_noise, trace, use_graph)
        eager = trace is not None or not use_graph or add_len < 3
        host = bool(sample) and noise != "device"
        if host and eager and self.noise_streams is not None:
            streams, self.noise_streams = self.noise_streams, None
            blocks = iter(range(add_len))

            def host_noise(nb, nv):
                i = next(blocks)
                return streams[0][i] if len(streams) == 1 else torch.cat([s_[i] for s_ in streams], dim=0)
        if host and not eager and self.noise_streams is None:
            import os
            if 4.0 * add_len * b * self.head.weight.shape[0] / 2 ** 20 > float(os.environ.get("CCVS_NOISE_STREAM_MAX_MB", "1024")):
                eager = True
        sampler["stream"] = host and not eager
        max_len = n_pre + n_cond + t0 + add_len
        if self.persistent_step and not self.warm_only:
            self.check_steps()
        c = self.begin(b, max_len)

        device_rng = sample and noise == "device"
        words = self._philox_words() if device_rng else None
        logits = self.prefill(code, cond_idx if use_cond else None, delta_length_cond if use_cond else None, lbl_idx=lbl_idx)
        if trace is not None:
            trace.append(logits.clone())
        c["codes"][:, :t0] = code
        c["len_dev"].fill_(n_pre + n_cond + t0)
        self._set_decode_state(words)
        if device_rng:
            self._emit(logits, sampler, None, t0, words=words, step=(0xffffffff, 0))
        elif sampler["stream"]:
            self._emit(logits, sampler, self._stage_noise_streams(b, add_len, logits.shape[1], host_noise), t0)
        else:
            self._emit(logits, sampler, host_noise(b, logits.shape[1]).to(logits.device, non_blocking=True) if sample else None, t0)

        if not eager:
            if self.progress is not None:
                self.progress(t0 + 1, c["codes"])
            self._replay_steps(sampler, (bool(sample), top_k, float(temperature), n_pre + n_cond, b), add_len - 1, known=t0 + 1)
        else:
            for _ in range(add_len - 1):
                nz = None
                if host:
                    nz = host_noise(b, self.head.weight.shape[0]).to(code.device, non_blocking=True)
                self._decode_body(sampler, noise=nz, trace=trace)
        c["len"] = n_pre + n_cond + t0 + add_len - 1
        return c["codes"][:, :t0 + add_len].clone()

    def _stage_noise_streams(self, b, add_len, v, host_noise):
        c = self._cache
        dev = c["noise_ptrs"].device
        groups = c["G"]
        rows = b // groups
        streams, self.noise_streams = self.noise_streams, None
        if self.warm_only:
            streams = [torch.ones(2, rows, v, dtype=torch.float32, device=dev)] * groups
        elif streams is None:
            assert groups == 1, "host-drawn sampling noise of stacked batches is pre-drawn per batch (GPT.noise_streams)"
            buf = torch.empty(add_len, b, v, dtype=torch.float32, pin_memory=True)
            for i in range(add_len):
                buf[i].copy_(host_noise(b, v))
            streams = [buf.to(dev, non_blocking=True)]
        assert len(streams) == groups, (len(streams), groups)
        cur = torch.cuda.current_stream()
        for s_ in streams:
            assert s_.is_cuda and s_.dtype == torch.float32 and s_.is_contiguous() and tuple(s_.shape[1:]) == (rows, v) and s_.shape[0] >= min(add_len, 2), s_.shape
            s_.record_stream(cur)
        ptrs = torch.tensor([s_.data_ptr() + 4 * rows * v for s_ in streams], dtype=torch.int64)
        c["noise_ptrs"].copy_(ptrs, non_blocking=True)
        c["noise_keep"] = streams
        return streams[0][0] if groups == 1 else torch.cat([s_[0] for s_ in streams], dim=0)

    @torch.no_grad()
    def forward(self, idx, cond_idx=torch.tensor([]), state_idx=torch.tensor([]), lbl_idx=torch.tensor([]), delta_length_cond=None):
        t_cond = cond_idx.shape[1] if 0 not in cond_idx.size() else 0
        n_pre = self.n_prefix()
        assert t_cond + n_pre + idx.shape[1] <= self.block_size, "Cannot forward, model block size is exhausted."
        if 0 not in state_idx.size():
            if n_pre:
                raise NotImplementedError("label / start tokens together with an ancillary token stream")
            state_idx = state_idx[:, :self.config.num_blocks * self.config.state_size].to(idx.device)
# ... 6 lines not shown
```

### ccvs_amd/ops.py

```python
import ctypes as C
import math

import torch

from . import lib as _lib

ACT_NONE, ACT_LRELU = 0, 1
EPI_NONE, EPI_GELU, EPI_RESIDUAL = 0, 1, 2
GEMM_SEQ = 0x100


class KernelTimer:

    def __init__(self):
        self.records = []
        self._open = None

    def begin(self, name, flops=0.0, nbytes=0.0, side=0.0, tag=None):
        e0 = torch.cuda.Event(enable_timing=True)
        e0.record()
        self._open = (name, flops, e0, nbytes, side, tag)

    def end(self):
        e1 = torch.cuda.Event(enable_timing=True)
# ... 303 lines not shown
        out = torch.empty(n, 49, ho, wo, dtype=torch.float32, device=second.device)
    assert out.shape == (n, 49, ho, wo) and out.is_contiguous() and out.dtype == torch.float32
    L = _lib.load()
    _lib.check(L.ccvs_correlation7x7(_p(first), _p(second), _p(out), n, c, h, w, stride, first_div, 1 if lrelu else 0, _stream()),
               "ccvs_correlation7x7")
    return out


def _ctx_list(ctxs):
    assert 1 <= len(ctxs) <= _lib.MAX_CTX
    cl = _lib.CtxList()
    cl.k = len(ctxs)
    keep = []
    n, c, h, w = ctxs[0].shape
    for j, t in enumerate(ctxs):
        _need_gpu(t)
        assert t.shape == (n, c, h, w) and t.dtype == torch.float32
        if not (t.stride(3) == 1 and t.stride(2) == w and t.stride(1) == h * w):
            t = t.contiguous()
        keep.append(t)
        cl.p[j] = t.data_ptr()
        cl.sN[j] = t.stride(0)
    return cl, keep


def backwarp(x, flow, flow_mult=1.0, out=None):
    _need_gpu(flow, out)
    if not _planes_dense(flow):
        flow = flow.contiguous()
    L = _lib.load()
    if isinstance(x, (list, tuple)):
        cl, keep = _ctx_list(x)
        nf, c, h, w = keep[0].shape
        n = nf * cl.k
        assert flow.shape == (n, 2, h, w)
        if out is None:
            out = torch.empty(n, c, h, w, dtype=torch.float32, device=flow.device)
        assert _rows_dense(out)
        _lib.check(L.ccvs_backwarp_ctx(C.byref(cl), h * w, _p(flow), flow.stride(0), flow_mult, _p(out), out.stride(0), out.stride(1),
                                       n, c, h, w, _stream()), "ccvs_backwarp_ctx")
        return out
    _need_gpu(x)
    x = _as_rows_dense(x)
    n, c, h, w = x.shape
    assert flow.shape == (n, 2, h, w)
    if out is None:
        out = torch.empty(n, c, h, w, dtype=torch.float32, device=x.device)
    assert _rows_dense(out)
    _lib.check(L.ccvs_backwarp(_p(x), x.stride(0), x.stride(1), _p(flow), flow.stride(0), flow_mult, _p(out), out.stride(0),
                               out.stride(1), n, c, h, w, _stream()), "ccvs_backwarp")
    return out


def pack_proj_weight(weight):
    cout, cin = weight.shape[:2]
    pads = [p_ for p_ in (16, 24, 48, 96) if p_ >= cout]
    if not pads:
        return None
    w = (weight.detach().float().view(cout, cin) * (1 / math.sqrt(cin))).t()
    out = torch.zeros(cin, pads[0], dtype=torch.float32, device=weight.device)
    out[:, :cout] = w
    return out.contiguous(), pads[0]


def backwarp_p8(ctxs, flow_occ, flow_mult, out=None):
    _need_gpu(flow_occ, out)
    if not _planes_dense(flow_occ):
        flow_occ = flow_occ.contiguous()
    cl, keep = _ctx_list(ctxs)
    nf, c, h, w = keep[0].shape
    n = nf * cl.k
    assert flow_occ.shape == (n, 3, h, w) and c % 8 == 0 and w % 4 == 0
    if out is None:
        out = torch.empty(n * (c + 8) * h * w, dtype=torch.float32, device=flow_occ.device)
    assert out.shape == (n * (c + 8) * h * w,) and out.is_contiguous() and out.dtype == torch.float32
    L = _lib.load()
    _lib.check(L.ccvs_backwarp_p8_ctx(C.byref(cl), h * w, _p(flow_occ), flow_occ.stride(0), flow_mult, _p(out), n, c, h, w, _stream()),
               "ccvs_backwarp_p8_ctx")
    return P8Act(out, n, c + 8, h, w)


def backwarp_proj(ctxs, flow, flow_mult, w_t, cout_pad, bias, cout, act=True, out=None):
    _need_gpu(flow, w_t, bias, out)
    if not _planes_dense(flow):
        flow = flow.contiguous()
    cl, keep = _ctx_list(ctxs)
    nf, c, h, w = keep[0].shape
    n = nf * cl.k
    assert flow.shape == (n, 2, h, w) and w_t.shape == (c, cout_pad)
    if out is None:
        out = torch.empty(n, cout, h, w, dtype=torch.float32, device=flow.device)
    assert out.shape == (n, cout, h, w) and out.is_contiguous() and out.dtype == torch.float32
    L = _lib.load()
    _lib.check(L.ccvs_backwarp_proj_ctx(C.byref(cl), h * w, _p(flow), flow.stride(0), flow_mult, _p(w_t), _p(bias), _p(out), n, c, cout, cout_pad,
                                        h, w, ACT_LRELU if act else ACT_NONE, _stream()), "ccvs_backwarp_proj_ctx")
    return out


def warp_fuse_blend(dec, ctx, flows, occs, flow_mult, k):
    _need_gpu(dec, flows, occs)
    assert _rows_dense(dec)
    flows = flows if _planes_dense(flows) else flows.contiguous()
    occs = occs if _planes_dense(occs) else occs.contiguous()
    n, c, h, w = dec.shape
    assert flows.shape == (n * k, 2, h, w) and occs.shape == (n * k, 1, h, w)
    L = _lib.load()
    if isinstance(ctx, (list, tuple)):
        cl, keep = _ctx_list(ctx)
        assert cl.k == k and keep[0].shape == (n, c, h, w)
        _lib.check(L.ccvs_warp_fuse_blend_ctx(_p(dec), dec.stride(0), dec.stride(1), C.byref(cl), _p(flows), flows.stride(0), _p(occs),
                                              occs.stride(0), flow_mult, n, c, h, w, _stream()), "ccvs_warp_fuse_blend_ctx")
        return dec
    _need_gpu(ctx)
    ctx = ctx.contiguous()
    assert ctx.shape == (n * k, c, h, w)
    _lib.check(L.ccvs_warp_fuse_blend(_p(dec), dec.stride(0), dec.stride(1), _p(ctx), _p(flows), flows.stride(0), _p(occs),
                                      occs.stride(0), flow_mult, n, k, c, h, w, _stream()), "ccvs_warp_fuse_blend")
    return dec


def pack_deform_weight(weight, precision=None):
    return pack_conv_weight(weight, precision, scale=1.0)


def deform_conv3x3(ctxs, flow, flow_mult, w_packed, bias, occ=None, toff=None, act=False):
    _need_gpu(flow, w_packed.data, bias, occ, toff)
    if not _planes_dense(flow):
        flow = flow.contiguous()
    if occ is not None and not _planes_dense(occ):
        occ = occ.contiguous()
    if toff is not None:
        toff = _as_rows_dense(toff)
    cl, keep = _ctx_list(ctxs)
    nf, c, h, w = keep[0].shape
    n = nf * cl.k
    assert flow.shape == (n, 2, h, w) and w_packed.k == 3 and w_packed.kw == 3 and w_packed.cin == c and w_packed.cout == c
    assert occ is None or occ.shape == (n, 1, h, w)
    assert toff is None or toff.shape == (n, c, h, w)
    out = torch.empty(n, c, h, w, dtype=torch.float32, device=flow.device)
    prec = {"f32": 0, "bf16x3": 1}[w_packed.kind]
    prof = KERNEL_TIMER
    if prof is not None:
        prof.begin("deform_" + w_packed.kind, flops=2.0 * n * c * c * 9 * h * w, nbytes=4.0 * (2 * n * c * h * w + 2 * n * h * w),
                   side=4.0 * 9 * c * c, tag=(n, c, h, w))
    L = _lib.load()
    _lib.check(L.ccvs_deform_conv3x3_ctx(C.byref(cl), h * w, _p(flow), flow.stride(0), float(flow_mult), _p(w_packed.data), w_packed.cout_pad,
                                         prec, _p(bias), _p(occ), occ.stride(0) if occ is not None else 0, _p(toff),
                                         toff.stride(0) if toff is not None else 0, toff.stride(1) if toff is not None else 0, _p(out),
                                         out.stride(0), out.stride(1), n, c, h, w, ACT_LRELU if act else ACT_NONE, _stream()),
               "ccvs_deform_conv3x3_ctx")
    if prof is not None:
        prof.end()
    return out


def gconvT4x4s2(x, w, out=None):
    _need_gpu(x, w, out)
    if not _planes_dense(x):
        x = x.contiguous()
    n, g, h, ww = x.shape
    assert w.shape[0] == g and w.shape[2:] == (4, 4)
    mult = w.shape[1]
    if out is None:
        out = torch.empty(n, g * mult, 2 * h, 2 * ww, dtype=torch.float32, device=x.device)
    assert out.shape == (n, g * mult, 2 * h, 2 * ww) and _rows_dense(out)
    L = _lib.load()
    _lib.check(L.ccvs_gconvT4x4s2(_p(x), x.stride(0), _p(w.detach().contiguous()), _p(out), out.stride(0), out.stride(1), n, g, mult, h, ww,
                                  _stream()), "ccvs_gconvT4x4s2")
    return out


def flow_mask_toff_(x, occ=None, toff=None, act=False):
    _need_gpu(x, occ, toff)
    assert _rows_dense(x)
    n, c, h, w = x.shape
    if occ is not None:
        occ = occ if _planes_dense(occ) else occ.contiguous()
        assert occ.shape == (n, 1, h, w)
    if toff is not None:
        toff = _as_rows_dense(toff)
        assert toff.shape == (n, c, h, w)
    L = _lib.load()
    _lib.check(L.ccvs_flow_mask_toff(_p(x), x.stride(0), x.stride(1), _p(occ), occ.stride(0) if occ is not None else 0, _p(toff),
                                     toff.stride(0) if toff is not None else 0, toff.stride(1) if toff is not None else 0, n, c, h, w,
                                     ACT_LRELU if act else ACT_NONE, _stream()), "ccvs_flow_mask_toff")
    return x


def vq_argmin(z, codebook_t, e_sq):
    _need_gpu(z, codebook_t, e_sq)
    z = z.contiguous()
    n, c = z.shape[:2]
    hw = z.shape[2] * z.shape[3]
    idx = torch.empty(n * hw, dtype=torch.int64, device=z.device)
    L = _lib.load()
    _lib.check(L.ccvs_vq_argmin(_p(z), _p(codebook_t), _p(e_sq), _p(idx), n, c, hw, codebook_t.shape[1], _stream()), "ccvs_vq_argmin")
    return idx


def embed_gather(code, codebook, n, hw):
    _need_gpu(code, codebook)
    code = code.contiguous()
    n_e, c = codebook.shape
    z = torch.empty(n, c, hw, dtype=torch.float32, device=codebook.device)
    L = _lib.load()
    _lib.check(L.ccvs_embed_gather(_p(code), _p(codebook), _p(z), n, c, hw, n_e, _stream()), "ccvs_embed_gather")
    return z


def l2_normalize_channels_(x):
    _need_gpu(x)
    assert x.is_contiguous() and x.dtype == torch.float32 and x.dim() == 4
    n, c, h, w = x.shape
    L = _lib.load()
    _lib.check(L.ccvs_l2_normalize_channels(_p(x), n, c, h * w, _stream()), "ccvs_l2_normalize_channels")
    return x


def gpt_embed(idx, tok_emb, pos_table, pos0=0, pos_off=None, pos_dev=None):
    _need_gpu(idx, pos_off, tok_emb, pos_table, pos_dev)
    b, tq = idx.shape
    assert idx.stride(1) == 1 or tq == 1
    c = tok_emb.shape[1]
    x = torch.empty(b * tq, c, dtype=torch.float32, device=tok_emb.device)
    L = _lib.load()
    _lib.check(L.ccvs_gpt_embed(_p(idx), idx.stride(0), _p(pos_off), pos0, _p(pos_dev), tq, _p(tok_emb), _p(pos_table), _p(x), b, c,
                                tok_emb.shape[0], _stream()), "ccvs_gpt_embed")
    return x


def layernorm(x, gamma, beta, out=None):
    _need_gpu(x, gamma, beta)
    rows, c = x.shape
    assert x.is_contiguous()
    if out is None:
        out = torch.empty_like(x)
    L = _lib.load()
    _lib.check(L.ccvs_layernorm(_p(x), _p(gamma), _p(beta), _p(out), rows, c, _stream()), "ccvs_layernorm")
    return out


def gemm_nt(x, w, bias=None, epilogue=EPI_NONE, residual=None, out=None):
    _need_gpu(x, w, bias, residual, out)
    m, k = x.shape
    n = w.shape[0]
    assert x.stride(1) == 1 and w.is_contiguous() and w.shape[1] == k
    if out is None:
        out = torch.empty(m, n, dtype=torch.float32, device=x.device)
    assert out.stride(1) == 1
    if residual is not None:
        assert residual.stride(1) == 1 and residual.stride(0) == out.stride(0)
    L = _lib.load()
    _lib.check(L.ccvs_gemm_nt(_p(x), x.stride(0), _p(w), _p(bias), _p(residual), _p(out), out.stride(0), m, n, k, epilogue,
                              _p(_gemm_workspace(x.device)), _stream()), "ccvs_gemm_nt")
    return out


_GEMM_WS = {}


def _gemm_workspace(device):
    key = (device, torch.cuda.current_stream().cuda_stream)
    ws = _GEMM_WS.get(key)
    if ws is None:
        ws = _GEMM_WS[key] = torch.zeros(int(_lib.load().ccvs_gemm_workspace_bytes()), dtype=torch.uint8, device=device)
    return ws


def pack_ln_linear(weight, bias, gamma, beta):
    w = weight.detach().float()
    wg = (w * gamma.detach().float().view(1, -1)).contiguous()
    b = bias.detach().float() if bias is not None else torch.zeros(w.shape[0], device=w.device)
    bb = (b + w.double().matmul(beta.detach().double()).float()).contiguous()
    s = wg.double().sum(dim=1).float().contiguous()
    return wg, bb, s


def gemm_ln(x, wg, bb, s, eps=1e-5, epilogue=EPI_NONE, out=None):
    _need_gpu(x, wg, bb, s, out)
    m, k = x.shape
    n = wg.shape[0]
    assert x.stride(1) == 1 and wg.is_contiguous() and wg.shape[1] == k
    if out is None:
        out = torch.empty(m, n, dtype=torch.float32, device=x.device)
    L = _lib.load()
    _lib.check(L.ccvs_gemm_ln(_p(x), x.stride(0), _p(wg), _p(bb), _p(s), eps, _p(out), out.stride(0), m, n, k, epilogue, _stream()),
               "ccvs_gemm_ln")
    return out


def gemm_ln_qkv(x, wg, bb, s, kcache, vcache, b, tq, pos0, pos_dev=None, eps=1e-5, out=None):
    _need_gpu(x, wg, bb, s, kcache, vcache, pos_dev, out)
    c = x.shape[1]
    _, h, tmax, d = kcache.shape
    assert x.shape[0] == b * tq and x.stride(1) == 1 and wg.shape == (3 * c, c) and h * d == c
    q = out if out is not None else torch.empty(b * tq, c, dtype=torch.float32, device=x.device)
    assert q.shape == (b * tq, c) and q.dtype == torch.float32 and q.is_contiguous()
    L = _lib.load()
    _lib.check(L.ccvs_gemm_ln_qkv(_p(x), x.stride(0), _p(wg), _p(bb), _p(s), eps, _p(q), _p(kcache), _p(vcache), b, tq, c, h, pos0,
                                  _p(pos_dev), tmax, _stream()), "ccvs_gemm_ln_qkv")
    return q


def kv_append(k, v, kcache, vcache, pos0, pos_dev=None):
    b, tq, hd = k.shape
    _, h, tmax, d = kcache.shape
    assert k.stride(2) == 1 and v.stride() == k.stride()
    L = _lib.load()
    _lib.check(L.ccvs_kv_append(_p(k), _p(v), k.stride(0), k.stride(1), _p(kcache), _p(vcache), b, h, tq, pos0, _p(pos_dev), tmax, d,
                                _stream()), "ccvs_kv_append")


def attention(q, kcache, vcache, pos0, pos_dev=None):
    b, tq, hd = q.shape
    _, h, tmax, d = kcache.shape
    assert q.stride(2) == 1
    out = torch.empty(b, tq, hd, dtype=torch.float32, device=q.device)
    L = _lib.load()
    _lib.check(L.ccvs_attention(_p(q), q.stride(0), q.stride(1), _p(kcache), _p(vcache), _p(out), b, h, tq, pos0, _p(pos_dev), tmax, d,
                                _stream()), "ccvs_attention")
    return out


def sample_topk(logits, top_k, temperature, noise=None, out=None, philox=None):
    _need_gpu(logits, noise, out)
    b, v = logits.shape
    assert logits.stride(1) == 1
    if out is None:
        out = torch.empty(b, dtype=torch.int64, device=logits.device)
    if philox is not None:
        assert noise is None
        k0, k1, row0, step, call = (int(t) & 0xffffffff for t in philox)
        L = _lib.load()
        _lib.check(L.ccvs_sample_topk_philox(_p(logits), logits.stride(0), _p(out), out.stride(0), b, v, 0 if top_k is None else int(top_k),
                                             float(temperature), k0, k1, row0, step, call, _stream()), "ccvs_sample_topk_philox")
        return out
    if noise is not None:
        assert noise.shape == (b, v) and noise.is_contiguous()
    L = _lib.load()
    _lib.check(L.ccvs_sample_topk(_p(logits), logits.stride(0), _p(noise), _p(out), out.stride(0), b, v,
                                  0 if top_k is None else int(top_k), float(temperature), _stream()), "ccvs_sample_topk")
    return out


def sample_topn(logits, top_k, temperature, n, noise=None):
    _need_gpu(logits, noise)
    b, v = logits.shape
    assert logits.stride(1) == 1 and 1 <= n <= v
    if noise is not None:
        assert noise.shape == (b, v) and noise.is_contiguous()
    idx = torch.empty(b, n, dtype=torch.int64, device=logits.device)
    logp = torch.empty(b, n, dtype=torch.float32, device=logits.device)
    L = _lib.load()
    _lib.check(L.ccvs_sample_topn(_p(logits), logits.stride(0), _p(noise), _p(idx), _p(logp), b, v, 0 if top_k is None else int(top_k),
                                  float(temperature), int(n), _stream()), "ccvs_sample_topn")
    return idx, logp


class GptDecodeStep:

    def __init__(self, layers, B, C, H, Tmax, ln_eps, tok_emb, pos_table, pos_off, head, tok, codes, widx, length,
                 x, q, att, h, logits, noise, top_k, temperature, state, rng=False, groups=1, noise_stream=None, persistent=False):
        hw, hb, hs = head
        keep = [tok_emb, pos_table, hw, hb, hs, tok, codes, widx, length, x, q, att, h, logits, noise, state, noise_stream]
        for t in keep:
            if t is not None:
                _need_gpu(t)
        f32 = [tok_emb, pos_table, hw, hb, hs, x, q, att, h, logits] + ([noise] if noise is not None else [])
        assert all(t.dtype == torch.float32 and t.is_contiguous() for t in f32)
        assert tok.dtype == torch.int64 and tok.numel() == B and tok.is_contiguous() and codes.dtype == torch.int64 and codes.stride(1) == 1
        assert widx.dtype == torch.int32 and length.dtype == torch.int32 and state.dtype == torch.int32
        assert groups >= 1 and B % groups == 0 and widx.numel() == groups and length.numel() == groups and state.numel() == 8 * groups
        assert widx.is_contiguous() and length.is_contiguous() and state.is_contiguous()
        if noise_stream is not None:
            assert noise is None and noise_stream.dtype == torch.int64 and noise_stream.numel() == groups and noise_stream.is_contiguous()
        arr = (_lib.GptLayer * len(layers))()
        for i, lay in enumerate(layers):
            for name, t in lay.items():
                t = t.detach()
                _need_gpu(t)
                assert t.dtype == torch.float32 and t.is_contiguous(), name
                keep.append(t)
                setattr(arr[i], name, _p(t))
        F = layers[0]["fc_w"].shape[0]
        assert x.shape == (B, C) and h.shape == (B, F) and logits.shape == (B, hw.shape[0])
        self.ws = _gemm_workspace(x.device)
        d = _lib.GptDecode()
        d.B, d.C, d.H, d.F, d.n_layer, d.Tmax, d.vocab, d.V = B, C, H, F, len(layers), Tmax, tok_emb.shape[0], hw.shape[0]
        d.ln_eps = ln_eps
        d.layers = arr
        d.tok_emb, d.pos_table, d.pos_off = _p(tok_emb.detach()), _p(pos_table), int(pos_off)
        d.head_w, d.head_b, d.head_s = _p(hw), _p(hb), _p(hs)
        d.tok, d.codes, d.codes_sB = _p(tok), _p(codes), codes.stride(0)
        d.widx, d.len = _p(widx), _p(length)
        d.x, d.q, d.att, d.h, d.logits = _p(x), _p(q), _p(att), _p(h), _p(logits)
        d.noise = _p(noise)
        d.rng = 1 if (rng and noise is None and noise_stream is None) else 0
        d.noise_stream = _p(noise_stream)
        d.top_k, d.temperature = 0 if top_k is None else int(top_k), float(temperature)
        d.workspace, d.state = _p(self.ws), _p(state)
        d.groups = groups
        self.desc, self._arr, self._keep = d, arr, keep
        self.persistent = bool(persistent)
        if self.persistent:
            L = _lib.load()
            self.program = torch.empty(int(L.ccvs_gpt_program_bytes(len(layers))), dtype=torch.uint8, device=x.device)
            d.persistent, d.program = 1, _p(self.program)
            import ctypes
            _lib.check(L.ccvs_gpt_decode_prepare(ctypes.byref(d), _stream()), "ccvs_gpt_decode_prepare")

    def launch(self):
        L = _lib.load()
        _lib.check(L.ccvs_gpt_decode_step(C.byref(self.desc), _stream()), "ccvs_gpt_decode_step")

    def status(self):
        if self.persistent:
            L = _lib.load()
            _lib.check(L.ccvs_gpt_decode_status(_p(self.ws), _stream()), "ccvs_gpt_decode_status")


def stream_cu_limit(stream, cu_limit):
    L = _lib.load()
    _lib.check(L.ccvs_stream_cu_limit(C.c_void_p(stream.cuda_stream), int(cu_limit)), "ccvs_stream_cu_limit")


def pack_u8_norm(vid, std, mean, out=None):
    _need_gpu(vid, out)
    vid = vid.contiguous()
    lead = vid.shape[:-3]
    h, w = vid.shape[-2:]
    n = int(math.prod(lead)) if len(lead) else 1
    if out is None:
        out = torch.empty(*lead, h, w, 3, dtype=torch.uint8, device=vid.device)
    assert out.shape == (*lead, h, w, 3) and out.is_contiguous() and out.dtype == torch.uint8
    s3, m3 = (C.c_float * 3)(*[float(v) for v in std]), (C.c_float * 3)(*[float(v) for v in mean])
    L = _lib.load()
    _lib.check(L.ccvs_pack_u8_norm(_p(vid), _p(out), n, h, w, s3, m3, _stream()), "ccvs_pack_u8_norm")
    return out


def psnr(x, y, data_range=1.0):
    _need_gpu(x, y)
    assert x.shape == y.shape and x.dim() == 4 and x.dtype == y.dtype == torch.float32, (x.shape, y.shape)
    x, y = x.contiguous(), y.contiguous()
    out = torch.empty(x.shape[0], dtype=torch.float32, device=x.device)
    _lib.check(_lib.load().ccvs_psnr(_p(x), _p(y), _p(out), x.shape[0], x[0].numel(), float(data_range), _stream()), "ccvs_psnr")
    return out


def mse(a, b):
    _need_gpu(a, b)
    assert a.shape == b.shape and a.dtype == b.dtype == torch.float32 and a.numel() > 0, (a.shape, b.shape)
    a, b = a.contiguous(), b.contiguous()
    out = torch.empty((), dtype=torch.float32, device=a.device)
    _lib.check(_lib.load().ccvs_mse(_p(a), _p(b), _p(out), a.numel(), _stream()), "ccvs_mse")
    return out


def token_nll(logits2d, target, rows=None, ncols=None):
    _need_gpu(logits2d, target, rows)
    assert logits2d.dim() == 2 and logits2d.dtype == torch.float32 and logits2d.stride(1) == 1, (logits2d.shape, logits2d.stride())
    ncols = logits2d.shape[1] if ncols is None else int(ncols)
    assert 0 < ncols <= logits2d.shape[1], (ncols, logits2d.shape)
    target = target.reshape(-1).to(torch.int64).contiguous()
    n_rows = target.numel()
    if rows is not None:
        assert rows.dtype == torch.int32 and rows.dim() == 1 and rows.is_contiguous() and rows.numel() == n_rows, (rows.shape, n_rows)
    else:
        assert n_rows == logits2d.shape[0], (n_rows, logits2d.shape)
    out = torch.empty(n_rows, dtype=torch.float32, device=logits2d.device)
    _lib.check(_lib.load().ccvs_token_nll(_p(logits2d), logits2d.stride(0), _p(rows), _p(target), n_rows, ncols, _p(out), _stream()),
               "ccvs_token_nll")
    return out


def mean_f32(x):
    _need_gpu(x)
    assert x.dtype == torch.float32 and x.numel() > 0, (x.dtype, x.shape)
    x = x.contiguous()
    out = torch.empty((), dtype=torch.float32, device=x.device)
    _lib.check(_lib.load().ccvs_mean_f32(_p(x), x.numel(), _p(out), _stream()), "ccvs_mean_f32")
    return out


def l1_mean(a, b):
    _need_gpu(a, b)
    assert a.shape == b.shape and a.dtype == b.dtype == torch.float32 and a.numel() > 0, (a.shape, b.shape)
    a, b = a.contiguous(), b.contiguous()
    L = _lib.load()
    out = torch.empty((), dtype=torch.float32, device=a.device)
    ws = torch.empty(int(L.ccvs_l1_workspace_bytes(a.numel())), dtype=torch.uint8, device=a.device)
    _lib.check(L.ccvs_l1_mean(_p(a), _p(b), _p(out), _p(ws), a.numel(), _stream()), "ccvs_l1_mean")
    return out


def vq_stats(z_nchw, idx, codebook, row_scale=None):
    _need_gpu(z_nchw, idx, codebook, row_scale)
    assert z_nchw.dim() == 4 and z_nchw.dtype == torch.float32 and z_nchw.numel() > 0, (z_nchw.shape, z_nchw.dtype)
    assert codebook.dim() == 2 and codebook.dtype == torch.float32 and codebook.shape[1] == z_nchw.shape[1], (codebook.shape, z_nchw.shape)
    z, codebook = z_nchw.contiguous(), codebook.contiguous()
    n, c = z.shape[:2]
    hw = z.shape[2] * z.shape[3]
    n_e = codebook.shape[0]
    idx = idx.reshape(-1).to(torch.int64).contiguous()
    assert idx.numel() == n * hw, (idx.shape, z.shape)
    if row_scale is not None:
        assert row_scale.dtype == torch.float32 and row_scale.shape == (n_e,) and row_scale.is_contiguous(), (row_scale.shape, n_e)
    L = _lib.load()
    mean_sq = torch.empty((), dtype=torch.float32, device=z.device)
    counts = torch.empty(n_e, dtype=torch.int32, device=z.device)
    ws = torch.empty(int(L.ccvs_vq_stats_workspace_bytes(n, c, hw)), dtype=torch.uint8, device=z.device)
    _lib.check(L.ccvs_vq_stats(_p(z), _p(idx), _p(codebook), _p(row_scale), _p(mean_sq), _p(counts), _p(ws), n, c, hw, n_e, _stream()),
               "ccvs_vq_stats")
    return mean_sq, counts


def code_perplexity(counts, total):
    _need_gpu(counts)
    assert counts.dim() == 1 and counts.dtype == torch.int32 and counts.numel() > 0 and int(total) > 0, (counts.shape, counts.dtype, total)
    counts = counts.contiguous()
    out = torch.empty((), dtype=torch.float32, device=counts.device)
    _lib.check(_lib.load().ccvs_code_perplexity(_p(counts), counts.numel(), int(total), _p(out), _stream()), "ccvs_code_perplexity")
    return out


def ssim_planes(x, y, data_range=2.0):
    _need_gpu(x, y)
    assert x.shape == y.shape and x.dim() >= 2 and x.dtype == y.dtype == torch.float32, (x.shape, y.shape)
    x, y = x.contiguous(), y.contiguous()
    h, w = x.shape[-2:]
    planes = x.numel() // (h * w)
    out = torch.empty(planes, dtype=torch.float64, device=x.device)
    L = _lib.load()
    step = 65535
    ws = torch.empty(int(L.ccvs_ssim_workspace_bytes(min(planes, step), h, w)), dtype=torch.uint8, device=x.device)
    xf, yf = x.view(planes, h, w), y.view(planes, h, w)
    for p0 in range(0, planes, step):
        n = min(step, planes - p0)
        _lib.check(L.ccvs_ssim(_p(xf[p0:]), _p(yf[p0:]), _p(out[p0:]), _p(ws), n, h, w, float(data_range), _stream()), "ccvs_ssim")
    return out.view(x.shape[:-2])


def resize_bilinear(x, size):
    _need_gpu(x)
    assert x.dtype == torch.float32 and x.dim() >= 2
    x = x.contiguous()
    h, w = x.shape[-2:]
    oh, ow = int(size[0]), int(size[1])
    out = torch.empty(*x.shape[:-2], oh, ow, dtype=torch.float32, device=x.device)
    _lib.check(_lib.load().ccvs_resize_bilinear(_p(x), _p(out), x.numel() // (h * w), h, w, oh, ow, _stream()), "ccvs_resize_bilinear")
    return out


def pack_u8(vid, lo=-1.0, hi=1.0, out=None):
    _need_gpu(vid, out)
    vid = vid.contiguous()
    lead = vid.shape[:-3]
    h, w = vid.shape[-2:]
    n = int(math.prod(lead)) if len(lead) else 1
    if out is None:
        out = torch.empty(*lead, h, w, 3, dtype=torch.uint8, device=vid.device)
    assert out.shape == (*lead, h, w, 3) and out.is_contiguous() and out.dtype == torch.uint8
    L = _lib.load()
    _lib.check(L.ccvs_pack_u8(_p(vid), _p(out), n, h, w, lo, hi, _stream()), "ccvs_pack_u8")
    return out


_RESAMPLE_TABLES = {}
_NORM_TABLES = {}


def resample_tables(in_size, out_size, device=None):
    in_size, out_size = int(in_size), int(out_size)
    assert in_size > 0 and out_size > 0, (in_size, out_size)
    device = torch.device("cpu" if device is None else device)
    key = (in_size, out_size, str(device))
    if key in _RESAMPLE_TABLES:
        return _RESAMPLE_TABLES[key]
    f64 = torch.float64
    scale = in_size / out_size
    filterscale = max(scale, 1.0)
    support = 1.0 * filterscale
    ksize = int(math.ceil(support)) * 2 + 1
    center = (torch.arange(out_size, dtype=f64) + 0.5) * scale
    xmin = torch.trunc(center - support + 0.5).clamp_(min=0)
    xmax = torch.trunc(center + support + 0.5).clamp_(max=in_size) - xmin
    ss = 1.0 / filterscale
    w = torch.zeros(out_size, ksize, dtype=f64)
    ww = torch.zeros(out_size, dtype=f64)
    for x in range(ksize):
        v = (1.0 - ((x + xmin - center + 0.5) * ss).abs()).clamp_(min=0)
        v = torch.where(x < xmax, v, torch.zeros_like(v))
        w[:, x] = v
        ww += v
    w = torch.where((ww != 0)[:, None], w / ww[:, None], w)
    coef = torch.trunc(w * float(1 << 22) + 0.5).to(torch.int32)
    bounds = torch.stack([xmin, xmax], dim=1).to(torch.int32)
    _RESAMPLE_TABLES[key] = (coef.contiguous().to(device), bounds.contiguous().to(device))
    return _RESAMPLE_TABLES[key]


def norm_table(mean, std, device):
    mean, std = tuple(float(m) for m in mean), tuple(float(s) for s in std)
    assert len(mean) == 3 and len(std) == 3, (mean, std)
    key = (mean, std, str(torch.device(device)))
    if key not in _NORM_TABLES:
        v = torch.arange(256, dtype=torch.uint8).to(torch.float32).div(255)[None].repeat(3, 1)
        v = v.sub_(torch.tensor(mean, dtype=torch.float32)[:, None]).div_(torch.tensor(std, dtype=torch.float32)[:, None])
        _NORM_TABLES[key] = v.contiguous().to(device)
    return _NORM_TABLES[key]


def ingest_u8(frames, box=None, size=None, out=None, mean=None, std=None, as_u8=False):
    _need_gpu(frames, out)
    assert frames.dtype == torch.uint8 and frames.dim() in (3, 4) and frames.shape[-1] == 3, (frames.dtype, frames.shape)
    if frames.dim() == 3:
        frames = frames[None]
    n, hs, ws = frames.shape[:3]
    if frames.stride()[1:] != (3 * ws, 3, 1) or (n > 1 and frames.stride(0) < hs * ws * 3):
        frames = frames.contiguous()
    top, left, hc, wc = (0, 0, hs, ws) if box is None else (int(v) for v in box)
    ho, wo = (hc, wc) if size is None else (int(size[0]), int(size[1]))
    if not (0 <= top and 0 <= left and hc > 0 and wc > 0 and top + hc <= hs and left + wc <= ws):
        raise ValueError(f"ingest_u8: crop box {(top, left, hc, wc)} leaves the {hs} x {ws} frame")
    dev = frames.device
    hcoef, hbounds = resample_tables(wc, wo, dev) if wo != wc else (None, None)
    vcoef, vbounds = resample_tables(hc, ho, dev) if ho != hc else (None, None)
    lut = None
    if as_u8:
        assert mean is None and std is None, "as_u8: the uint8 form is not normalised"
        if out is None:
            out = torch.empty(n, ho, wo, 3, dtype=torch.uint8, device=dev)
        assert out.dtype == torch.uint8 and out.shape == (n, ho, wo, 3) and out.is_contiguous(), (out.dtype, out.shape, out.stride())
        s_n = s_c = 0
    else:
        lut = norm_table((0.5, 0.5, 0.5) if mean is None else mean, (0.5, 0.5, 0.5) if std is None else std, dev)
        if out is None:
            out = torch.empty(n, 3, ho, wo, dtype=torch.float32, device=dev)
        assert out.dtype == torch.float32 and out.shape == (n, 3, ho, wo) and _rows_dense(out), (out.dtype, out.shape, out.stride())
        s_n, s_c = out.stride(0), out.stride(1)
        assert s_c >= ho * wo and (n == 1 or s_n >= 2 * s_c + ho * wo), out.stride()
    _lib.check(_lib.load().ccvs_ingest_u8(_p(frames), frames.stride(0) if n > 1 else hs * ws * 3, n, hs, ws, top, left, hc, wc,
                                          _p(hcoef), _p(hbounds), hcoef.shape[1] if hcoef is not None else 0,
                                          _p(vcoef), _p(vbounds), vcoef.shape[1] if vcoef is not None else 0, ho, wo,
                                          _p(out) if as_u8 else None, None if as_u8 else _p(out), s_n, s_c, _p(lut), _stream()),
               "ccvs_ingest_u8")
    return out
```

### include/ccvs_hip.h

```cpp
#ifndef CCVS_HIP_H
#define CCVS_HIP_H

#include <stdint.h>

#ifdef __cplusplus
extern "C" {
#endif

#define CCVS_OK 0
#define CCVS_ERR_ARG (-1)
#define CCVS_ERR_LAUNCH (-2)

#define CCVS_ACT_NONE 0
#define CCVS_ACT_LRELU 1

const char* ccvs_last_error(void);
int ccvs_abi_version(void);

typedef struct ccvs_conv_desc {
    int32_t N, Cin, Hin, Win;
    int64_t in_sN, in_sC;
    int32_t Cout, CoutPad, Hout, Wout;
    int64_t out_sN, out_sC;
    int64_t res_sN, res_sC;
    int32_t kh, kw, stride, pad, transposed;
    int32_t act, accumulate;
    float out_scale;
    const float* pre;
    int64_t pre_sN, pre_sC;
    int32_t pre_div;
    int32_t in_p8, out_p8;
    int32_t cu_limit;
    const void* w_ktail;
} ccvs_conv_desc;

int ccvs_conv2d(const float* x, const float* w_packed, const float* bias, const float* residual, float* y,
                const ccvs_conv_desc* d, void* stream);

int ccvs_conv2d_bf16x3(const float* x, const void* w_split, const float* bias, const float* residual, float* y,
                       const ccvs_conv_desc* d, void* stream);

int ccvs_conv_fetch_bytes_per_lane(const char* kernel_name);

int ccvs_conv_persistent_tiles(int32_t mode);

const char* ccvs_conv_last_launch(void);

int ccvs_upfirdn2d(const float* x, float* y, const float* residual, int64_t NC, int32_t H, int32_t W, int32_t up,
                   int32_t down, int32_t pad0, int32_t pad1, float gain, int32_t act, float out_scale, void* stream);

int ccvs_dwconvT4x4s2(const float* x, int64_t x_sN, const float* w, float* y, int64_t y_sN, int32_t N, int32_t C, int32_t H,
                      int32_t W, void* stream);

int ccvs_gaussian_blur(const float* x, int64_t x_sN, int64_t x_sC, float* y, int32_t N, int32_t C, int32_t H, int32_t W, int32_t k,
                       const float* weights, void* stream);

int ccvs_to_rgb(const float* x, int64_t x_sN, const float* w, const float* b_conv, const float* bias, const float* skip, float* y,
                int32_t N, int32_t C, int32_t H, int32_t W, void* stream);

int ccvs_channel_head(const float* x, int64_t x_sN, const float* w, float scale, const float* bias, float* y, int32_t N, int32_t C,
                      int32_t H, int32_t W, int32_t act, int32_t tanh_out, void* stream);

int ccvs_correlation7x7(const float* first, const float* second, float* out, int32_t N, int32_t C, int32_t H, int32_t W,
                        int32_t stride, int32_t first_div, int32_t lrelu, void* stream);

int ccvs_backwarp(const float* x, int64_t x_sN, int64_t x_sC, const float* flow, int64_t flow_sN, float flow_mult, float* y,
                  int64_t y_sN, int64_t y_sC, int32_t N, int32_t C, int32_t H, int32_t W, void* stream);

#define CCVS_MAX_CTX 16
typedef struct ccvs_ctx_list {
    int32_t k;
    const float* p[CCVS_MAX_CTX];
    int64_t sN[CCVS_MAX_CTX];
} ccvs_ctx_list;
int ccvs_backwarp_ctx(const ccvs_ctx_list* ctx, int64_t x_sC, const float* flow, int64_t flow_sN, float flow_mult, float* y,
                      int64_t y_sN, int64_t y_sC, int32_t N, int32_t C, int32_t H, int32_t W, void* stream);
int ccvs_warp_fuse_blend_ctx(float* dec, int64_t dec_sN, int64_t dec_sC, const ccvs_ctx_list* ctx, const float* flows,
                             int64_t flows_sN, const float* occs, int64_t occs_sN, float flow_mult, int32_t N, int32_t C,
                             int32_t H, int32_t W, void* stream);

int ccvs_backwarp_p8_ctx(const ccvs_ctx_list* ctx, int64_t x_sC, const float* flow_occ, int64_t fo_sN, float flow_mult, void* y_p8,
                         int32_t N, int32_t C, int32_t H, int32_t W, void* stream);

int ccvs_backwarp_proj_ctx(const ccvs_ctx_list* ctx, int64_t x_sC, const float* flow, int64_t flow_sN, float flow_mult,
                           const float* w_t, const float* bias, float* y, int32_t N, int32_t Cin, int32_t Cout, int32_t CoutPad,
                           int32_t H, int32_t W, int32_t act, void* stream);

int ccvs_warp_fuse_blend(float* dec, int64_t dec_sN, int64_t dec_sC, const float* ctx, const float* flows, int64_t flows_sN,
                         const float* occs, int64_t occs_sN, float flow_mult, int32_t N, int32_t k, int32_t C, int32_t H,
                         int32_t W, void* stream);

int ccvs_tap_shift_add(const float* t, const float* bias, float* y, int64_t y_sN, int32_t N, int32_t k, int32_t H, int32_t W,
                       int32_t accumulate, int32_t vertical, void* stream);

int ccvs_vq_argmin(const float* z, const float* codebook_t, const float* e_sq, int64_t* idx, int32_t N, int32_t C, int32_t HW,
                   int32_t n_e, void* stream);

int ccvs_embed_gather(const int64_t* code, const float* codebook, float* z, int32_t N, int32_t C, int32_t HW, int32_t n_e,
                      void* stream);

int ccvs_l2_normalize_channels(float* x, int32_t N, int32_t C, int64_t HW, void* stream);

int ccvs_gpt_embed(const int64_t* idx, int64_t idx_sB, const int32_t* pos_off, int32_t pos0, const int32_t* pos_dev, int32_t Tq,
                   const float* tok_emb, const float* pos_table, float* x, int32_t B, int32_t C, int32_t vocab, void* stream);

int ccvs_layernorm(const float* x, const float* gamma, const float* beta, float* y, int32_t rows, int32_t C, void* stream);

#define CCVS_GEMM_SEQ 0x100
int64_t ccvs_gemm_workspace_bytes(void);
int ccvs_gemm_nt(const float* x, int64_t ldx, const float* w, const float* bias, const float* res, float* y, int64_t ldy,
                 int32_t M, int32_t N, int32_t K, int32_t epilogue, void* workspace, void* stream);

int ccvs_gemm_ln(const float* x, int64_t ldx, const float* w_gamma, const float* bias_beta, const float* w_rowsum, float eps,
                 float* y, int64_t ldy, int32_t M, int32_t N, int32_t K, int32_t epilogue, void* stream);

int ccvs_gemm_ln_qkv(const float* x, int64_t ldx, const float* w_gamma, const float* bias_beta, const float* w_rowsum, float eps,
                     float* q, float* kcache, float* vcache, int32_t B, int32_t Tq, int32_t C, int32_t H, int32_t pos0,
                     const int32_t* pos_dev, int32_t Tmax, void* stream);

int ccvs_attention(const float* q, int64_t q_sB, int64_t ldq, const float* kcache, const float* vcache, float* out, int32_t B,
                   int32_t H, int32_t Tq, int32_t pos0, const int32_t* pos_dev, int32_t Tmax, int32_t D, void* stream);

int ccvs_kv_append(const float* k, const float* v, int64_t sB, int64_t ld, float* kcache, float* vcache, int32_t B, int32_t H,
                   int32_t Tq, int32_t pos0, const int32_t* pos_dev, int32_t Tmax, int32_t D, void* stream);

int ccvs_sample_topk(const float* logits, int64_t ld, const float* noise, int64_t* out, int64_t out_stride, int32_t B, int32_t V,
                     int32_t top_k, float temperature, void* stream);
int ccvs_sample_topk_philox(const float* logits, int64_t ld, int64_t* out, int64_t out_stride, int32_t B, int32_t V, int32_t top_k,
                            float temperature, uint32_t key0, uint32_t key1, uint32_t row0, uint32_t step, uint32_t call, void* stream);

int ccvs_sample_topn(const float* logits, int64_t ld, const float* noise, int64_t* out_idx, float* out_logp, int32_t B, int32_t V,
                     int32_t top_k, float temperature, int32_t n, void* stream);

typedef struct ccvs_gpt_layer {
    const float *qkv_w, *qkv_b, *qkv_s;
    const float *proj_w, *proj_b;
    const float *fc_w, *fc_b, *fc_s;
    const float *fc2_w, *fc2_b;
    float *kcache, *vcache;
} ccvs_gpt_layer;

typedef struct ccvs_gpt_decode {
    int32_t B, C, H, F, n_layer, Tmax, vocab, V;
    float ln_eps;
    const ccvs_gpt_layer* layers;
    const float *tok_emb, *pos_table;
    int32_t pos_off;
    const float *head_w, *head_b, *head_s;
    int64_t* tok;
    int64_t* codes; int64_t codes_sB;
    int32_t *widx, *len;
    float *x, *q, *att, *h, *logits;
    const float* noise;
    int32_t rng;
    int32_t top_k; float temperature;
    void* workspace;
    int32_t* state;
    int32_t groups;
    const float* const* noise_stream;
    int32_t persistent;
    void* program;
} ccvs_gpt_decode;
int ccvs_gpt_decode_step(const ccvs_gpt_decode* d, void* stream);
int ccvs_gpt_decode_status(const void* workspace, void* stream);
int64_t ccvs_gpt_program_bytes(int32_t n_layer);
int ccvs_gpt_decode_prepare(const ccvs_gpt_decode* d, void* stream);

int ccvs_stream_cu_limit(void* stream, int32_t cu_limit);

int ccvs_deform_conv3x3_ctx(const ccvs_ctx_list* ctx, int64_t x_sC, const float* flow, int64_t flow_sN, float flow_mult,
                            const void* w, int32_t CoutPad, int32_t precision, const float* bias, const float* occ, int64_t occ_sN,
                            const float* toff, int64_t toff_sN, int64_t toff_sC, float* y, int64_t y_sN, int64_t y_sC, int32_t N,
                            int32_t C, int32_t H, int32_t W, int32_t act, void* stream);
int ccvs_gconvT4x4s2(const float* x, int64_t x_sN, const float* w, float* y, int64_t y_sN, int64_t y_sC, int32_t N, int32_t G,
                     int32_t mult, int32_t H, int32_t W, void* stream);
int ccvs_flow_mask_toff(float* x, int64_t x_sN, int64_t x_sC, const float* occ, int64_t occ_sN, const float* toff, int64_t toff_sN,
                        int64_t toff_sC, int32_t N, int32_t C, int32_t H, int32_t W, int32_t act, void* stream);

int ccvs_pack_u8(const float* vid, uint8_t* out, int64_t N, int32_t H, int32_t W, float lo, float hi, void* stream);
int ccvs_pack_u8_norm(const float* vid, uint8_t* out, int64_t N, int32_t H, int32_t W, const float* std3, const float* mean3,
                      void* stream);

int ccvs_psnr(const float* x, const float* y, float* out, int64_t N, int64_t per_image, float data_range, void* stream);
int ccvs_mse(const float* a, const float* b, float* out, int64_t n, void* stream);
int ccvs_token_nll(const float* logits, int64_t ld, const int32_t* rows, const int64_t* target, int64_t n_rows, int32_t ncols, float* nll,
                   void* stream);
int ccvs_mean_f32(const float* x, int64_t n, float* out, void* stream);
int64_t ccvs_ssim_workspace_bytes(int64_t planes, int32_t H, int32_t W);
int ccvs_ssim(const float* x, const float* y, double* out, void* workspace, int64_t planes, int32_t H, int32_t W, double data_range,
              void* stream);
int ccvs_resize_bilinear(const float* x, float* out, int64_t planes, int32_t H, int32_t W, int32_t OH, int32_t OW, void* stream);

#include "ccvs_hip_eval.h"
#include "ccvs_hip_input.h"

#ifdef __cplusplus
}
#endif
#endif
```

Before: 204.7.

## Pre-tile GPT decode weights into MFMA fragment order for coalesced loads

Adds a tiled weight layout in which each 16x16 block of a 16-deep K slice is stored contiguously in MFMA fragment order. The decode GEMMs (qkv, proj, fc, fc2, head), in both the graph-captured and persistent step kernels, then read weights with one contiguous 16-byte load per lane instead of 16 strided rows. This targets poor coalescing of weight reads, which dominate memory-bound small-M decode. In exchange it keeps an extra copy of every weight, adds a re-tiling cache keyed on the weight versions, and requires each K slice to be a whole number of 16-deep batches.

```diff
diff --git a/ccvs_amd/csrc/gpt.hip b/ccvs_amd/csrc/gpt.hip
--- a/ccvs_amd/csrc/gpt.hip
+++ b/ccvs_amd/csrc/gpt.hip
@@ -111,6 +111,7 @@
     int kz;
     float* ws_slabs;
     int* ws_count;
+    int wt;
 };
 
 #define GEMM_U 4
@@ -139,15 +140,15 @@
 #define GEMM16_RED_WORDS(NB) (GEMM_WAVES * (NB) * 64 * 4)
 #define GEMM16_STAT_WORDS(RB) (GEMM_WAVES * (RB) * 16 * 2)
 #define GEMM16_FIN_WORDS(RB) ((RB) * 16 * 2)
-template <int RB, int CB, int U, bool COH, typename PT>
+template <int RB, int CB, int U, bool COH, bool WT, typename PT>
 __device__ __forceinline__ void gemm16_tile(const float* __restrict__ x_, const float* __restrict__ w_, long ldx_, int K_, int N_, int M_, int ks_,
                                             int kz_, const PT& p, int bx_, int by_, int bz_, float* __restrict__ red, float* __restrict__ stat,
                                             float* __restrict__ fin) {
 #define GP(ptr) gp_<COH>(ptr)
     constexpr int NB = RB * CB;
     constexpr int XAUX = COH ? 16 : 0;
-    const int tid = thread_id<COH>(), lane = tid & 63, wave = tid >> 6;
-    const int li = lane & 15, g = lane >> 4;
+    int tid = thread_id<COH>(), lane = tid & 63, wave = tid >> 6;
+    int li = lane & 15, g = lane >> 4;
     const int m0 = by_ * 16 * RB, ncol0 = bx_ * 16 * CB;
     const int kper = K_ / (ks_ * kz_);
     const int kbase = bz_ * (K_ / kz_);
@@ -156,15 +157,21 @@
     unsigned wofs[CB], xofs[RB];
 #pragma unroll
     for (int cb = 0; cb < CB; ++cb) {
-        const int nrow = min(ncol0 + 16 * cb + li, N_ - 1);
-        wofs[cb] = ((unsigned)nrow * (unsigned)K_ + koff) * 4u;
+        if constexpr (WT) {
+            const int ct = min(bx_ * CB + cb, ((N_ + 15) >> 4) - 1);
+            wofs[cb] = (((unsigned)ct * (unsigned)(K_ >> 4) + ((koff - 4 * g) >> 4)) * 256u + 4u * lane) * 4u;
+        } else {
+            const int nrow = min(ncol0 + 16 * cb + li, N_ - 1);
+            wofs[cb] = ((unsigned)nrow * (unsigned)K_ + koff) * 4u;
+        }
     }
 #pragma unroll
     for (int rb = 0; rb < RB; ++rb) {
         const int mrow = min(m0 + 16 * rb + li, M_ - 1);
         xofs[rb] = ((unsigned)mrow * (unsigned)ldx_ + koff) * 4u;
     }
-    const __amdgpu_buffer_rsrc_t wr = __builtin_amdgcn_make_buffer_rsrc(const_cast<float*>(w_), 0, N_ * K_ * 4, 0x00020000);
+    const __amdgpu_buffer_rsrc_t wr = __builtin_amdgcn_make_buffer_rsrc(const_cast<float*>(w_), 0, (WT ? (N_ + 15) & ~15 : N_) * K_ * 4, 0x00020000);
+    constexpr int WSTEP = WT ? 1024 : 64;
     const __amdgpu_buffer_rsrc_t xr = __builtin_amdgcn_make_buffer_rsrc(const_cast<float*>(x_), 0, (int)(M_ * ldx_ * 4), 0x00020000);
     f32x4 acc[RB][CB];
     float sx[RB], sxx[RB];
@@ -181,7 +188,7 @@
 #pragma unroll
             for (int cb = 0; cb < CB; ++cb)
 #pragma unroll
-                for (int u = 0; u < U; ++u) wv[cb][u] = buf_load4(wr, wofs[cb], k0 * 4 + 64 * u);
+                for (int u = 0; u < U; ++u) wv[cb][u] = buf_load4(wr, wofs[cb], k0 * (WSTEP / 16) + WSTEP * u);
 #pragma unroll
             for (int rb = 0; rb < RB; ++rb)
 #pragma unroll
@@ -202,7 +209,7 @@
         for (; k0 < kper; k0 += 16) {
             f32x4 w1[CB], x1[RB];
 #pragma unroll
-            for (int cb = 0; cb < CB; ++cb) w1[cb] = buf_load4(wr, wofs[cb], k0 * 4);
+            for (int cb = 0; cb < CB; ++cb) w1[cb] = buf_load4(wr, wofs[cb], k0 * (WSTEP / 16));
 #pragma unroll
             for (int rb = 0; rb < RB; ++rb) x1[rb] = buf_load4<XAUX>(xr, xofs[rb], k0 * 4);
 #pragma unroll
@@ -214,6 +221,11 @@
                 if (p.ln_s) ln_accum(x1[rb], sx[rb], sxx[rb]);
             }
         }
+    }
+    if constexpr (WT) {
+        asm volatile("" : "+v"(tid));
+        if constexpr (!COH) __builtin_assume(tid >= 0 && tid < 64 * GEMM_WAVES);
+        lane = tid & 63; wave = tid >> 6; li = lane & 15; g = lane >> 4;
     }
     if (p.ln_s) {
 #pragma unroll
@@ -300,13 +312,13 @@
 #undef GP
 }
 
-template <int RB, int CB, int U>
+template <int RB, int CB, int U, bool WT>
 __global__ __launch_bounds__(64 * GEMM_WAVES) void gemm16_kernel(const float* __restrict__ x_, const float* __restrict__ w_, long ldx_, int K_, int N_,
                                                                 int M_, int ks_, int kz_, Gemm16 p) {
     __shared__ __attribute__((aligned(16))) float red[GEMM16_RED_WORDS(RB * CB)];
     __shared__ float stat[GEMM16_STAT_WORDS(RB)];
     __shared__ float fin[GEMM16_FIN_WORDS(RB)];
-    gemm16_tile<RB, CB, U, false>(x_, w_, ldx_, K_, N_, M_, ks_, kz_, p, blockIdx.x, blockIdx.y, blockIdx.z, red, stat, fin);
+    gemm16_tile<RB, CB, U, false, WT>(x_, w_, ldx_, K_, N_, M_, ks_, kz_, p, blockIdx.x, blockIdx.y, blockIdx.z, red, stat, fin);
 }
 
 template <int RB>
@@ -566,6 +578,10 @@
 
 static bool gemm_ws_holds(const Gemm16& g) { return g.kz == 1 || cdiv(g.N, 16) * cdiv(g.M, 16) <= GEMM_WS_TILES; }
 
+static bool gemm_wt_holds(const Gemm16& g) {
+    return !g.wt || ((long)cdiv(g.N, 16) * 16 * g.K * 4 < (1L << 31) && g.K % (g.ks * g.kz) == 0 && (g.K / (g.ks * g.kz)) % 16 == 0);
+}
+
 static int launch_gemm16(Gemm16& g, hipStream_t st, const char* name) {
     if (!(g.x && g.w && g.y)) { ccvs_set_error("%s: null pointer", name); return CCVS_ERR_ARG; }
     if (!(g.M > 0 && g.N > 0 && g.K > 0)) { ccvs_set_error("%s: empty tensor", name); return CCVS_ERR_ARG; }
@@ -578,6 +594,11 @@
         ccvs_set_error("%s: operand beyond 2^31 bytes (32-bit buffer offsets)", name);
         return CCVS_ERR_ARG;
     }
+    if (g.wt && !decode_form) { ccvs_set_error("%s: tiled weights are read by the decode forms only (single position, M <= %d)", name, GEMM_DECODE_MAX_M); return CCVS_ERR_ARG; }
+    if (!gemm_wt_holds(g)) {
+        ccvs_set_error("%s: tiled weights need K slices of whole 16-deep batches and fewer than 2^31 bytes", name);
+        return CCVS_ERR_ARG;
+    }
     if (!decode_form && g.grp_rows > 0) { ccvs_set_error("%s: row groups need M <= %d", name, GEMM_DECODE_MAX_M); return CCVS_ERR_ARG; }
     if (form == GEMM_FORM_SEQ) {
         const int rt = cdiv(g.M, GS_BM), ct = cdiv(g.N, GS_BM);
@@ -585,10 +606,11 @@
     } else if (form == GEMM_FORM_RB)
         hipLaunchKernelGGL((gemm16_rb_kernel<4>), dim3(cdiv(g.N, 16), cdiv(g.M, 64), 1), dim3(512), 0, st, g);
     else {
-#define GEMM16_LAUNCH(RBv, CBv, Uv)                                                                                                         \
-    hipLaunchKernelGGL((gemm16_kernel<RBv, CBv, Uv>), dim3(cdiv(g.N, 16 * CBv), cdiv(g.M, 16 * RBv), g.kz), dim3(64 * GEMM_WAVES), 0, st, g.x, \
+#define GEMM16_LAUNCH(RBv, CBv, Uv, WTv)                                                                                                         \
+    hipLaunchKernelGGL((gemm16_kernel<RBv, CBv, Uv, WTv>), dim3(cdiv(g.N, 16 * CBv), cdiv(g.M, 16 * RBv), g.kz), dim3(64 * GEMM_WAVES), 0, st, g.x, \
                        g.w, g.ldx, g.K, g.N, g.M, g.ks, g.kz, g)
-        if (form == GEMM_FORM_TILE2) GEMM16_LAUNCH(2, 2, 1); else GEMM16_LAUNCH(1, 1, GEMM_U);
+        if (form == GEMM_FORM_TILE2) { if (g.wt) GEMM16_LAUNCH(2, 2, 1, true); else GEMM16_LAUNCH(2, 2, 1, false); }
+        else { if (g.wt) GEMM16_LAUNCH(1, 1, GEMM_U, true); else GEMM16_LAUNCH(1, 1, GEMM_U, false); }
 #undef GEMM16_LAUNCH
     }
     CCVS_CHECK_LAUNCH(name);
@@ -634,6 +656,28 @@
     g.kcache = kcache; g.vcache = vcache; g.C = C; g.H = H; g.D = C / H; g.Tq = Tq; g.Tmax = Tmax; g.pos0 = pos0; g.pos_dev = pos_dev;
     g.seq = Tq > 1 ? 1 : 0;
     return launch_gemm16(g, (hipStream_t)stream, "ccvs_gemm_ln_qkv");
+}
+
+extern "C" int32_t ccvs_gemm_tiled_max_rows(void) { return GEMM_DECODE_MAX_M; }
+
+extern "C" int ccvs_gemm_tiled(const float* x, int64_t ldx, const float* w_tiled, const float* bias, const float* res, const float* w_rowsum,
+                               float eps, float* y, int64_t ldy, int32_t M, int32_t N, int32_t K, int32_t epilogue, float* kcache, float* vcache,
+                               int32_t H, int32_t pos0, const int32_t* pos_dev, int32_t Tmax, void* workspace, void* stream) {
+    CCVS_REQUIRE((epilogue & ~0xff) == 0 && M <= GEMM_DECODE_MAX_M, "ccvs_gemm_tiled: a single-position call of at most %d rows", GEMM_DECODE_MAX_M);
+    CCVS_REQUIRE(!w_rowsum || epilogue == 0 || epilogue == 1, "ccvs_gemm_tiled: bad epilogue");
+    CCVS_REQUIRE((kcache != nullptr) == (vcache != nullptr), "ccvs_gemm_tiled: one cache without the other");
+    Gemm16 g = {};
+    g.x = x; g.ldx = ldx; g.w = w_tiled; g.bias = bias; g.res = res; g.y = y; g.ldy = ldy; g.M = M; g.N = N; g.K = K; g.epi = epilogue; g.wt = 1;
+    g.ln_s = w_rowsum; g.ln_eps = eps;
+    if (kcache) {
+        CCVS_REQUIRE(w_rowsum && epilogue == 0 && N == 3 * K && ldy == K && H > 0 && K % H == 0 && pos0 >= 0 && pos0 < Tmax, "ccvs_gemm_tiled: bad QKV shape / position");
+        g.kcache = kcache; g.vcache = vcache; g.C = K; g.H = H; g.D = K / H; g.Tq = 1; g.Tmax = Tmax; g.pos0 = pos0; g.pos_dev = pos_dev;
+    }
+    if (workspace) {
+        g.ws_slabs = (float*)workspace;
+        g.ws_count = (int*)((char*)workspace + GEMM_WS_SLAB_BYTES);
+    }
+    return launch_gemm16(g, (hipStream_t)stream, "ccvs_gemm_tiled");
 }
 
 __global__ __launch_bounds__(256) void kv_append_kernel(const float* __restrict__ k, const float* __restrict__ v, long sB, long ld,
@@ -1305,7 +1349,7 @@
     __syncthreads();
 }
 
-template <int RB, int CB, int U>
+template <int RB, int CB, int U, bool WT>
 __device__ __forceinline__ void step_gemm(const __attribute__((address_space(4))) Gemm16& g, float* smem) {
     float* red = smem;
     float* stat = red + GEMM16_RED_WORDS(RB * CB);
@@ -1318,7 +1362,7 @@
     const int total = gx * gy * kz;
     for (int vb = blockIdx.x; vb < total; vb += gridDim.x) {
         const int bx = vb % gx, r = vb / gx;
-        gemm16_tile<RB, CB, U, true>(x, w, ldx, K, N, M, ks, kz, g, bx, r % gy, r / gy, red, stat, fin);
+        gemm16_tile<RB, CB, U, true, WT>(x, w, ldx, K, N, M, ks, kz, g, bx, r % gy, r / gy, red, stat, fin);
         __syncthreads();
     }
 }
@@ -1331,7 +1375,7 @@
 __device__ __forceinline__ T* as_global(T* p) {
     return (T*)(STEP_GLOBAL T*)p;
 }
-template <int D, bool T2>
+template <int D, bool T2, bool WT>
 __global__ __launch_bounds__(256) __attribute__((amdgpu_waves_per_eu(8, 8))) void gpt_step_kernel(const StepArgs* __restrict__ ap_) {
     extern __shared__ __attribute__((aligned(16))) float smem[];
     constexpr int RB = T2 ? 2 : 1, CB = T2 ? 2 : 1, U = T2 ? 1 : GEMM_U;
@@ -1377,7 +1421,7 @@
                 __syncthreads();
             }
         } else {
-            step_gemm<RB, CB, U>(P->g, smem);
+            step_gemm<RB, CB, U, WT>(P->g, smem);
         }
         target += G; step_barrier(bar, target, ph + 1);
     }
@@ -1440,7 +1484,7 @@
 static Gemm16 step_head_gemm(const ccvs_gpt_decode* d) {
     Gemm16 g = {};
     g.x = d->x; g.ldx = d->C; g.w = d->head_w; g.bias = d->head_b; g.y = d->logits; g.ldy = d->V; g.M = d->B; g.N = d->V; g.K = d->C;
-    g.ln_s = d->head_s; g.ln_eps = d->ln_eps;
+    g.ln_s = d->head_s; g.ln_eps = d->ln_eps; g.wt = d->w_tiled ? 1 : 0;
     return g;
 }
 
@@ -1451,7 +1495,7 @@
 
 template <typename Visit>
 static int step_phases(const ccvs_gpt_decode* d, const char* who, Visit visit) {
-    const int D = d->C / d->H, grp_rows = step_grp_rows(d);
+    const int D = d->C / d->H, grp_rows = step_grp_rows(d), wt = d->w_tiled ? 1 : 0;
     float* ws_slabs = (float*)d->workspace;
     int* ws_count = d->workspace ? (int*)((char*)d->workspace + GEMM_WS_SLAB_BYTES) : nullptr;
     int rc;
@@ -1463,6 +1507,7 @@
         g.x = d->x; g.ldx = d->C; g.w = L.qkv_w; g.bias = L.qkv_b; g.y = d->q; g.ldy = d->C; g.M = d->B; g.N = 3 * d->C; g.K = d->C;
         g.ln_s = L.qkv_s; g.ln_eps = d->ln_eps;
         g.kcache = L.kcache; g.vcache = L.vcache; g.C = d->C; g.H = d->H; g.D = D; g.Tq = 1; g.Tmax = d->Tmax; g.pos0 = 0; g.pos_dev = d->len; g.grp_rows = grp_rows;
+        g.wt = wt;
         if ((rc = visit(STEP_GEMM, g, "ccvs_gpt_decode_step(qkv)")) != CCVS_OK) return rc;
         g = Gemm16{};
         g.x = d->q; g.ldx = d->C; g.y = d->att; g.kcache = L.kcache; g.vcache = L.vcache; g.H = d->H; g.M = d->B; g.Tmax = d->Tmax;
@@ -1471,14 +1516,17 @@
         g = Gemm16{};
         g.x = d->att; g.ldx = d->C; g.w = L.proj_w; g.bias = L.proj_b; g.res = d->x; g.y = d->x; g.ldy = d->C; g.M = d->B; g.N = d->C; g.K = d->C; g.epi = 2;
         g.ws_slabs = ws_slabs; g.ws_count = ws_count;
+        g.wt = wt;
         if ((rc = visit(STEP_GEMM, g, "ccvs_gpt_decode_step(proj)")) != CCVS_OK) return rc;
         g = Gemm16{};
         g.x = d->x; g.ldx = d->C; g.w = L.fc_w; g.bias = L.fc_b; g.y = d->h; g.ldy = d->F; g.M = d->B; g.N = d->F; g.K = d->C; g.epi = 1;
         g.ln_s = L.fc_s; g.ln_eps = d->ln_eps;
+        g.wt = wt;
         if ((rc = visit(STEP_GEMM, g, "ccvs_gpt_decode_step(fc)")) != CCVS_OK) return rc;
         g = Gemm16{};
         g.x = d->h; g.ldx = d->F; g.w = L.fc2_w; g.bias = L.fc2_b; g.res = d->x; g.y = d->x; g.ldy = d->C; g.M = d->B; g.N = d->C; g.K = d->F; g.epi = 2;
         g.ws_slabs = ws_slabs; g.ws_count = ws_count;
+        g.wt = wt;
         if ((rc = visit(STEP_GEMM, g, "ccvs_gpt_decode_step(fc2)")) != CCVS_OK) return rc;
     }
     Gemm16 g = step_head_gemm(d);
@@ -1507,7 +1555,7 @@
     const GemmForm tile = step_tile2(d) ? GEMM_FORM_TILE2 : GEMM_FORM_TILE1;
     int n = 0;
     rc = step_phases(d, "ccvs_gpt_decode_prepare", [&](int kind, Gemm16& g, const char* name) -> int {
-        if (n == n_ph || (kind == STEP_GEMM && (gemm16_plan(g) != tile || !gemm_ws_holds(g)))) { ccvs_set_error("ccvs_gpt_decode_prepare: %s does not fit the persistent step's table", name); return CCVS_ERR_ARG; }
+        if (n == n_ph || (kind == STEP_GEMM && (gemm16_plan(g) != tile || !gemm_ws_holds(g) || !gemm_wt_holds(g)))) { ccvs_set_error("ccvs_gpt_decode_prepare: %s does not fit the persistent step's table", name); return CCVS_ERR_ARG; }
         prog[n].kind = kind;
         prog[n++].g = g;
         return CCVS_OK;
@@ -1536,19 +1584,21 @@
     if (w_att > words) words = w_att;
     if (w_pick > words) words = w_pick;
     const size_t smem = words * sizeof(float);
-#define STEP_LAUNCH(Dv, T2v)                                                                                                          \
+#define STEP_LAUNCH_(Dv, T2v, WTv)                                                                                                        \
     do {                                                                                                                              \
         static bool attr_set = false;                                                                                                 \
         if (!attr_set) {                                                                                                              \
-            (void)hipFuncSetAttribute((const void*)gpt_step_kernel<Dv, T2v>, hipFuncAttributeMaxDynamicSharedMemorySize, 160 * 1024); \
+            (void)hipFuncSetAttribute((const void*)gpt_step_kernel<Dv, T2v, WTv>, hipFuncAttributeMaxDynamicSharedMemorySize, 160 * 1024); \
             attr_set = true;                                                                                                          \
         }                                                                                                                             \
-        hipLaunchKernelGGL((gpt_step_kernel<Dv, T2v>), dim3(n_cu), dim3(256), smem, st, a);                                           \
+        hipLaunchKernelGGL((gpt_step_kernel<Dv, T2v, WTv>), dim3(n_cu), dim3(256), smem, st, a);                                      \
     } while (0)
+#define STEP_LAUNCH(Dv, T2v) do { if (d->w_tiled) STEP_LAUNCH_(Dv, T2v, true); else STEP_LAUNCH_(Dv, T2v, false); } while (0)
     if (D == 64) { if (t2) STEP_LAUNCH(64, true); else STEP_LAUNCH(64, false); }
     else if (D == 32) { if (t2) STEP_LAUNCH(32, true); else STEP_LAUNCH(32, false); }
     else { if (t2) STEP_LAUNCH(16, true); else STEP_LAUNCH(16, false); }
 #undef STEP_LAUNCH
+#undef STEP_LAUNCH_
     CCVS_CHECK_LAUNCH("ccvs_gpt_decode_step(persistent)");
     return CCVS_OK;
 }
diff --git a/ccvs_amd/lib.py b/ccvs_amd/lib.py
--- a/ccvs_amd/lib.py
+++ b/ccvs_amd/lib.py
@@ -14,6 +14,7 @@
 ]
 EVAL_EXPORTS = ["ccvs_l1_workspace_bytes", "ccvs_l1_mean", "ccvs_vq_stats_workspace_bytes", "ccvs_vq_stats", "ccvs_code_perplexity"]
 INPUT_EXPORTS = ["ccvs_ingest_u8"]
+GEMM_EXPORTS = ["ccvs_gemm_tiled", "ccvs_gemm_tiled_max_rows"]
 
 
 class ConvDesc(C.Structure):
@@ -55,7 +56,7 @@
         ("noise", C.c_void_p), ("rng", C.c_int32), ("top_k", C.c_int32), ("temperature", C.c_float),
         ("workspace", C.c_void_p), ("state", C.c_void_p), ("groups", C.c_int32),
         ("noise_stream", C.c_void_p),
-        ("persistent", C.c_int32), ("program", C.c_void_p),
+        ("persistent", C.c_int32), ("program", C.c_void_p), ("w_tiled", C.c_int32),
     ]
 
 
@@ -86,6 +87,8 @@
     lib.ccvs_l1_workspace_bytes.argtypes = [C.c_int64]
     lib.ccvs_vq_stats_workspace_bytes.restype = C.c_int64
     lib.ccvs_vq_stats_workspace_bytes.argtypes = [C.c_int64, C.c_int32, C.c_int32]
+    lib.ccvs_gemm_tiled_max_rows.restype = C.c_int32
+    lib.ccvs_gemm_tiled_max_rows.argtypes = []
     lib.ccvs_gpt_program_bytes.restype = C.c_int64
     lib.ccvs_gpt_program_bytes.argtypes = [C.c_int32]
     lib.ccvs_conv_fetch_bytes_per_lane.restype = C.c_int
@@ -115,6 +118,7 @@
         "ccvs_gemm_nt": [vp, i64, vp, vp, vp, vp, i64, i32, i32, i32, i32, vp, vp],
         "ccvs_gemm_ln": [vp, i64, vp, vp, vp, f32, vp, i64, i32, i32, i32, i32, vp],
         "ccvs_gemm_ln_qkv": [vp, i64, vp, vp, vp, f32, vp, vp, vp, i32, i32, i32, i32, i32, vp, i32, vp],
+        "ccvs_gemm_tiled": [vp, i64, vp, vp, vp, vp, f32, vp, i64, i32, i32, i32, i32, vp, vp, i32, i32, vp, i32, vp, vp],
         "ccvs_attention": [vp, i64, i64, vp, vp, vp, i32, i32, i32, i32, vp, i32, i32, vp],
         "ccvs_kv_append": [vp, vp, i64, i64, vp, vp, i32, i32, i32, i32, vp, i32, i32, vp],
         "ccvs_sample_topk": [vp, i64, vp, vp, i64, i32, i32, i32, f32, vp],
diff --git a/ccvs_amd/models/skip_vid_generator/models/mingpt.py b/ccvs_amd/models/skip_vid_generator/models/mingpt.py
--- a/ccvs_amd/models/skip_vid_generator/models/mingpt.py
+++ b/ccvs_amd/models/skip_vid_generator/models/mingpt.py
@@ -65,6 +65,16 @@
             nn.Dropout(config.resid_pdrop),
         )
         self._folded = None
+        self._tiled = None
+
+    def tiled(self):
+        (qw, _, _), (fw, _, _) = self.folded()
+        src = (self.attn.proj.weight, self.mlp[3].weight)
+        key = (self._folded[0],) + tuple((t.data_ptr(), t._version) for t in src)
+        if self._tiled is None or self._tiled[0] != key:
+            self._tiled = (key, dict(qkv_w=ops.tile_weight(qw), proj_w=ops.tile_weight(src[0]), fc_w=ops.tile_weight(fw),
+                                     fc2_w=ops.tile_weight(src[1])))
+        return self._tiled
 
     def folded(self):
         src = (self.ln1.weight, self.ln1.bias, self.attn.query.weight, self.attn.key.weight, self.attn.value.weight,
@@ -134,6 +144,7 @@
         self.noise_streams = None
         import os
         self.persistent_step = os.environ.get("CCVS_DECODE_PERSISTENT", "0") == "1"
+        self.tiled_weights = os.environ.get("CCVS_DECODE_TILED_W", "1") == "1"
 
     @property
     def _graphs(self):
@@ -350,6 +361,13 @@
             hf = self._head_folded = (key, ops.pack_ln_linear(self.head.weight, None, self.ln_f.weight, self.ln_f.bias))
         return hf
 
+    def _head_tiled(self):
+        key, (hw, _, _) = self._head_packed()
+        ht = getattr(self, "_head_tiled_w", None)
+        if ht is None or ht[0] != key:
+            ht = self._head_tiled_w = (key, ops.tile_weight(hw))
+        return ht[1]
+
     def _head(self, x):
         return ops.gemm_ln(x, *self._head_packed()[1], eps=self.ln_f.eps)
 
@@ -432,9 +450,11 @@
         folded = [blk.folded() for blk in self.blocks]
         head_key, (hw, hb, hs) = self._head_packed()
         device_rng = sampler["sample"] and sampler["noise"] == "device"
+        tiled = self.tiled_weights and c["B"] <= ops.gemm_tiled_max_rows()
         host_stream = bool(sampler["sample"] and not device_rng and sampler.get("stream"))
         key = (tuple(blk._folded[0] for blk in self.blocks), head_key, sampler["sample"], sampler["top_k"],
-               sampler["temperature"], device_rng, host_stream, c["frame_pos0"], bool(self.persistent_step))
+               sampler["temperature"], device_rng, host_stream, c["frame_pos0"], bool(self.persistent_step),
+               tuple(blk.tiled()[0] for blk in self.blocks) if tiled else None)
         if c["desc"] is None or c["desc"][0] != key:
             layers = []
             for i, blk in enumerate(self.blocks):
@@ -449,7 +469,8 @@
                 x=c["x"], q=c["q"], att=c["att"], h=c["h"], logits=c["logits"],
                 noise=c["noise"] if (sampler["sample"] and not device_rng and not host_stream) else None, rng=device_rng,
                 noise_stream=c["noise_ptrs"] if host_stream else None,
-                top_k=sampler["top_k"], temperature=sampler["temperature"], state=c["state"], persistent=self.persistent_step)
+                top_k=sampler["top_k"], temperature=sampler["temperature"], state=c["state"], persistent=self.persistent_step,
+                tiled=([blk.tiled()[1] for blk in self.blocks], self._head_tiled()) if tiled else None)
             c["desc"] = (key, desc)
             c["graphs"] = {}
         return c["desc"][1]
diff --git a/ccvs_amd/ops.py b/ccvs_amd/ops.py
--- a/ccvs_amd/ops.py
+++ b/ccvs_amd/ops.py
@@ -629,6 +629,41 @@
     return q
 
 
+def tile_weight(w):
+    w = w.detach()
+    n, k = w.shape
+    assert w.dtype == torch.float32 and k % 16 == 0
+    npad = -(-n // 16) * 16
+    if npad != n:
+        w = torch.cat([w, w[-1:].expand(npad - n, k)], dim=0)
+    return w.reshape(npad // 16, 16, k // 16, 4, 4).permute(0, 2, 3, 1, 4).contiguous().view(-1)
+
+
+def gemm_tiled_max_rows():
+    return int(_lib.load().ccvs_gemm_tiled_max_rows())
+
+
+def gemm_tiled(x, wt, n, bias=None, epilogue=EPI_NONE, residual=None, out=None, ln_s=None, eps=1e-5, kcache=None, vcache=None, pos0=0,
+               pos_dev=None):
+    _need_gpu(x, wt, bias, residual, out, ln_s, kcache, vcache, pos_dev)
+    m, k = x.shape
+    assert x.stride(1) == 1 and wt.is_contiguous() and wt.numel() == -(-n // 16) * 16 * k
+    if out is None:
+        out = torch.empty(m, k if kcache is not None else n, dtype=torch.float32, device=x.device)
+    assert out.stride(1) == 1
+    if residual is not None:
+        assert residual.stride(1) == 1 and residual.stride(0) == out.stride(0)
+    h = tmax = 0
+    if kcache is not None:
+        _, h, tmax, d = kcache.shape
+        assert n == 3 * k and h * d == k and out.shape == (m, k) and out.is_contiguous() and kcache.shape[0] == m
+    ws = _gemm_workspace(x.device) if ln_s is None else None
+    L = _lib.load()
+    _lib.check(L.ccvs_gemm_tiled(_p(x), x.stride(0), _p(wt), _p(bias), _p(residual), _p(ln_s), eps, _p(out), out.stride(0), m, n, k, epilogue,
+                                 _p(kcache), _p(vcache), h, pos0, _p(pos_dev), tmax, _p(ws), _stream()), "ccvs_gemm_tiled")
+    return out
+
+
 def kv_append(k, v, kcache, vcache, pos0, pos_dev=None):
     b, tq, hd = k.shape
     _, h, tmax, d = kcache.shape
@@ -687,7 +722,8 @@
 class GptDecodeStep:
 
     def __init__(self, layers, B, C, H, Tmax, ln_eps, tok_emb, pos_table, pos_off, head, tok, codes, widx, length,
-                 x, q, att, h, logits, noise, top_k, temperature, state, rng=False, groups=1, noise_stream=None, persistent=False):
+                 x, q, att, h, logits, noise, top_k, temperature, state, rng=False, groups=1, noise_stream=None, persistent=False,
+                 tiled=None):
         hw, hb, hs = head
         keep = [tok_emb, pos_table, hw, hb, hs, tok, codes, widx, length, x, q, att, h, logits, noise, state, noise_stream]
         for t in keep:
@@ -707,6 +743,10 @@
                 t = t.detach()
                 _need_gpu(t)
                 assert t.dtype == torch.float32 and t.is_contiguous(), name
+                if tiled is not None and name in tiled[0][i]:
+                    n_k, t = t.shape, tiled[0][i][name]
+                    _need_gpu(t)
+                    assert t.dtype == torch.float32 and t.is_contiguous() and t.numel() == -(-n_k[0] // 16) * 16 * n_k[1], name
                 keep.append(t)
                 setattr(arr[i], name, _p(t))
         F = layers[0]["fc_w"].shape[0]
@@ -718,6 +758,12 @@
         d.layers = arr
         d.tok_emb, d.pos_table, d.pos_off = _p(tok_emb.detach()), _p(pos_table), int(pos_off)
         d.head_w, d.head_b, d.head_s = _p(hw), _p(hb), _p(hs)
+        if tiled is not None:
+            assert all(set(t) == {"qkv_w", "proj_w", "fc_w", "fc2_w"} for t in tiled[0]) and len(tiled[0]) == len(layers)
+            _need_gpu(tiled[1])
+            assert tiled[1].dtype == torch.float32 and tiled[1].is_contiguous() and tiled[1].numel() == -(-hw.shape[0] // 16) * 16 * C
+            keep.append(tiled[1])
+            d.head_w, d.w_tiled = _p(tiled[1]), 1
         d.tok, d.codes, d.codes_sB = _p(tok), _p(codes), codes.stride(0)
         d.widx, d.len = _p(widx), _p(length)
         d.x, d.q, d.att, d.h, d.logits = _p(x), _p(q), _p(att), _p(h), _p(logits)
diff --git a/include/ccvs_hip.h b/include/ccvs_hip.h
--- a/include/ccvs_hip.h
+++ b/include/ccvs_hip.h
@@ -160,6 +160,7 @@
     const float* const* noise_stream;
     int32_t persistent;
     void* program;
+    int32_t w_tiled;
 } ccvs_gpt_decode;
 int ccvs_gpt_decode_step(const ccvs_gpt_decode* d, void* stream);
 int ccvs_gpt_decode_status(const void* workspace, void* stream);
@@ -193,6 +194,7 @@
 
 #include "ccvs_hip_eval.h"
 #include "ccvs_hip_input.h"
+#include "ccvs_hip_gemm.h"
 
 #ifdef __cplusplus
 }
diff --git a/include/ccvs_hip_gemm.h b/include/ccvs_hip_gemm.h
--- /dev/null
+++ b/include/ccvs_hip_gemm.h
@@ -0,0 +1,17 @@
+#ifndef CCVS_HIP_GEMM_H
+#define CCVS_HIP_GEMM_H
+#include <stdint.h>
+#ifdef __cplusplus
+extern "C" {
+#endif
+
+int ccvs_gemm_tiled(const float* x, int64_t ldx, const float* w_tiled, const float* bias, const float* res, const float* w_rowsum,
+                    float eps, float* y, int64_t ldy, int32_t M, int32_t N, int32_t K, int32_t epilogue, float* kcache, float* vcache,
+                    int32_t H, int32_t pos0, const int32_t* pos_dev, int32_t Tmax, void* workspace, void* stream);
+
+int32_t ccvs_gemm_tiled_max_rows(void);
+
+#ifdef __cplusplus
+}
+#endif
+#endif
```

Measured after the change: 209.8 (median of 6 runs). 2.5% higher.
